# DaehwanKimLab/centrifuge

Hardware: AMD Instinct MI355X
Metric: classified reads/sec (whole node) on 100bp synthetic reads vs p_compressed; HBM GB/s achieved (higher is better)
Workload: dtype u64

## Files before the change

### centrifuge_amd/csrc/cf_device.hip

```cpp
#include <hip/hip_runtime.h>
#include <sched.h>
#include <dlfcn.h>

#include <algorithm>
#include <cmath>
#include <chrono>
#include <cstdio>
#include <cstdlib>
#include <cstring>
#include <memory>
#include <mutex>
#include <stdexcept>
#include <string>
#include <vector>

#include "../../include/centrifuge_amd.h"
#include "cf_index.hpp"
#include "cf_kernels.hpp"
#include "cf_scan.hpp"
#include "cf_textio.hpp"
#include "cf_restore.hpp"
#include "cf_plan.hpp"
#include "cf_knobs.hpp"

using namespace cfamd;

namespace {

thread_local std::string g_err;

struct HipError : std::runtime_error {
    using std::runtime_error::runtime_error;
};
struct ArgError : std::runtime_error {
    using std::runtime_error::runtime_error;
};

#define HIP_OK(expr)                                                                              \
    do {                                                                                          \
        hipError_t e_ = (expr);                                                                   \
        if (e_ != hipSuccess)                                                                     \
            throw HipError(std::string(#expr) + ": " + hipGetErrorString(e_));                    \
    } while (0)

static thread_local uint64_t *g_dryBytes = nullptr;
template <typename T>
struct DevBuf {
    T *p = nullptr;
    size_t n = 0;
    DevBuf() = default;
    DevBuf(const DevBuf &) = delete;
    DevBuf &operator=(const DevBuf &) = delete;
    ~DevBuf() { release(); }
    void release() { if (p) (void)hipFree(p); p = nullptr; n = 0; }
    void alloc(size_t count) {
        release();
        if (count == 0) count = 1;
        if (g_dryBytes) { *g_dryBytes += count * sizeof(T); n = count; return; }
        HIP_OK(hipMalloc(reinterpret_cast<void **>(&p), count * sizeof(T)));
        n = count;
    }
    void ensure(size_t count) { if (count > n) alloc(count + count / 8); }
    void upload(const std::vector<T> &v) {
        alloc(v.size());
        if (!v.empty()) HIP_OK(hipMemcpy(p, v.data(), v.size() * sizeof(T), hipMemcpyHostToDevice));
    }
    size_t bytes() const { return n * sizeof(T); }
};

template <int G>
__global__ void __launch_bounds__(256) k_search(DIndex ix, DParams pr, DBatch b) { search_body<G>(ix, pr, b); }

__global__ void __launch_bounds__(256) k_rlen(const uint64_t *off, uint32_t *rlen, uint32_t nReads) { rlen_body(off, rlen, nReads, cf_global_thread()); }
__global__ void __launch_bounds__(256) k_convert(DConvert c) { convert_body(c, cf_global_thread()); }
__global__ void __launch_bounds__(256) k_dense_unpack(DUnpack u) { dense_unpack_body(u, (uint64_t)blockIdx.x * blockDim.x + threadIdx.x); }
__global__ void __launch_bounds__(256) k_pack(DBatch b, uint8_t *recs, uint32_t W) { pack_body(b, recs, W, cf_global_thread()); }

template <int G, int W, bool COUNT>
__global__ void __launch_bounds__(256) __attribute__((amdgpu_waves_per_eu(COUNT ? 1 : W == 4 ? 6 : W == 6 ? 5 : 4, 8))) k_search2(DIndex ix, DParams pr, DBatch b) {
    __shared__ __attribute__((aligned(16))) uint8_t lds[(256 / G) * rec_lds_stride(W) + 256 * 4 * RankTab<G>::WORDS + (256 / G) * 16 * kLazyHits];
    search2_body<G, W, COUNT>(ix, pr, b, lds);
}

template <int W, bool COUNT, int LZ = 0, bool MULTI = false>
__global__ void __launch_bounds__(256) __attribute__((amdgpu_waves_per_eu((W == 4 && LZ == 1) ? 7 : (W == 4 && MULTI) ? 6 : (W == 6 && MULTI) ? 5 : 1, 8))) k_search2_l1(DIndex ix, DParams pr, DBatch b) {
    __shared__ __attribute__((aligned(16))) uint8_t lds[256 * rec_lds_stride(W) + 256 * 16 * (LZ ? LZ : (int)lazy_hits(1, W))];
    search2_body<1, W, COUNT, true, LZ, MULTI>(ix, pr, b, lds);
}
__global__ void __launch_bounds__(256) k_pair_planes(DIndex ix, uint8_t *planes2, uint64_t nGroups) {
    pair_planes_body(ix, planes2, (uint64_t)blockIdx.x * blockDim.x + threadIdx.x, nGroups);
}
__global__ void __launch_bounds__(256) k_occ_planes(DIndex ix, uint8_t *planes, uint64_t nSides) {
    occ_planes_body(ix, planes, (uint64_t)blockIdx.x * blockDim.x + threadIdx.x, nSides);
}
__global__ void __launch_bounds__(256) k_repeat_probe(DIndex ix, uint32_t nSamples, uint32_t depth, uint32_t *hits) {
    const uint32_t i = cf_global_thread();
    bool yes = false;
    if (i < nSamples && ix.len > 2) {
        uint64_t x = 0x9e3779b97f4a7c15ull * (i + 1);
        x ^= x >> 29; x *= 0xbf58476d1ce4e5b9ull; x ^= x >> 32;
        yes = repeat_probe_body(ix, x % (ix.len - 1), depth);
    }
    const uint64_t m = cf_ballot(yes);
    if (m && cf_lane() == (uint32_t)cf_ctz64(m)) (void)cf_atomic_add(hits, (uint32_t)cf_popc64(m));
}

__global__ void __launch_bounds__(256) k_post_fast(DIndex ix, DParams pr, DBatch b) {
    const uint32_t q = cf_global_thread();
    const bool d = q < b.nQueries ? post_fast_body(ix, pr, b, q) : false;
    if (q < b.nQueries && b.postDeferred) b.postDeferred[q] = d ? 1 : 0;
    defer_push(b.slowPost, &b.st->nSlowPost, d, q);
}
template <bool EARLY>
__global__ void __launch_bounds__(256) k_score_fast(DIndex ix, DParams pr, DBatch b) {
    const uint32_t q = cf_global_thread();
    const bool d = q < b.nQueries ? score_fast_body<EARLY>(ix, pr, b, q) : false;
    defer_push(b.slowScore, &b.st->nSlowScore, d, q);
}
__global__ void __launch_bounds__(256) k_list_all(uint32_t *list, uint32_t *counter, uint32_t n) {
    const uint32_t q = cf_global_thread();
    if (q < n) list[q] = q;
    if (q == 0) *counter = n;
}
__global__ void __launch_bounds__(64) __attribute__((amdgpu_waves_per_eu(3, 8))) k_post(DIndex ix, DParams pr, DBatch b, uint32_t capHits) {
    extern __shared__ __attribute__((aligned(16))) uint8_t ldsPost[];
    HitP *scratch = capHits ? reinterpret_cast<HitP *>(ldsPost) + (size_t)cf_local_thread() * capHits : nullptr;
    const uint32_t n = b.st->nSlowPost;
    for (uint32_t i = cf_global_thread(); i < n; i += cf_global_threads()) post_body(ix, pr, b, b.slowPost[i], scratch, capHits);
}
__global__ void __launch_bounds__(64) k_postfix_only(DIndex ix, DParams pr, DBatch b) {
    const uint32_t i = cf_global_thread();
    if (i < b.st->nItems / 2) post_fix(ix, pr, b, b.items[i]);
}
__global__ void k_window(DBatch b, uint32_t qLo, bool keepSlow) { if (cf_global_thread() == 0) row_window_body(b, qLo, keepSlow); }
__global__ void __launch_bounds__(256) k_emit(DParams pr, DBatch b) {
    const uint32_t q = cf_global_thread();
    if (q < b.nQueries) emit_body(pr, b, q);
}
template <int G, bool COUNT>
__global__ void __launch_bounds__(256) k_walk2(DIndex ix, DBatch b) { walk2_body<G, COUNT>(ix, b); }
template <int MODE>
__global__ void __launch_bounds__(256) k_walk_table(DIndex ix, DBatch b) { walk2_body<2, false, MODE>(ix, b); }
template <typename T>
__global__ void __launch_bounds__(256) k_stop_samples(DIndex ix, T *stopVal, uint64_t *stopBits, uint64_t nSamples) {
    for (uint64_t i = (uint64_t)blockIdx.x * blockDim.x + threadIdx.x; i < nSamples; i += (uint64_t)gridDim.x * blockDim.x) {
        const uint64_t pos = trio_at(ix.saPos, i << ix.offRate);
        stopVal[pos] = static_cast<const T *>(ix.offs)[i];
        cf_atomic_or64(&stopBits[pos >> 6], 1ull << (pos & 63));
    }
}
template <typename T>
__global__ void __launch_bounds__(256) k_stop_bounds(DIndex ix, T *stopVal, uint64_t *stopBits) {
    for (uint64_t j = (uint64_t)blockIdx.x * blockDim.x + threadIdx.x; j < ix.nBound; j += (uint64_t)gridDim.x * blockDim.x) {
        const uint64_t pos = trio_at(ix.saPos, ix.boundRow[j]);
        stopVal[pos] = (T)ix.boundRef[j];
        cf_atomic_or64(&stopBits[pos >> 6], 1ull << (pos & 63));
    }
}
template <typename T>
__global__ void k_stop_end(DIndex ix, T *stopVal, uint64_t *stopBits) {
    const uint64_t pos = trio_at(ix.saPos, ix.zOff);
    stopVal[pos] = 0;
    cf_atomic_or64(&stopBits[pos >> 6], 1ull << (pos & 63));
}
template <typename T>
__global__ void __launch_bounds__(256) k_table_by_position(DIndex ix, const T *stopVal, const uint64_t *stopBits, T *table, uint64_t nRows, uint32_t *walkMax) {
    uint32_t gap = 0;
    for (uint64_t row = (uint64_t)blockIdx.x * blockDim.x + threadIdx.x; row < nRows; row += (uint64_t)gridDim.x * blockDim.x) {
        const uint64_t pos = trio_at(ix.saPos, row);
        uint64_t w = pos >> 6;
        uint64_t m = stopBits[w] & (~0ull >> (63 - (pos & 63)));
        while (m == 0 && w > 0) m = stopBits[--w];
        const uint64_t pred = m ? (w << 6) + 63 - (uint64_t)__builtin_clzll(m) : 0;
        table[row] = stopVal[pred];
        const uint32_t g = (uint32_t)(pos - pred);
        gap = g > gap ? g : gap;
    }
    for (int d = 32; d > 0; d >>= 1) { const uint32_t o = __shfl_xor(gap, d, 64); gap = o > gap ? o : gap; }
    if ((threadIdx.x & 63) == 0 && gap) atomicMax(walkMax, gap);
}
template <typename T>
__global__ void __launch_bounds__(256) k_table_spot_check(DIndex ix, const T *table, uint64_t nRows, uint32_t nCheck, uint32_t *bad) {
    const uint32_t i = blockIdx.x * blockDim.x + threadIdx.x;
    if (i >= nCheck) return;
    const uint64_t row = i < 64 ? (i < 32 ? (uint64_t)i : nRows - 1 - (i - 32)) % nRows : (0x9e3779b97f4a7c15ull * (i + 1)) % nRows;
    uint32_t steps = 0;
    const uint32_t want = resolve_plain_row(ix, row, steps);
    if ((uint32_t)table[row] != (sizeof(T) == 2 ? (want & 0xffffu) : want)) atomicAdd(bad, 1u);
}

template <bool COUNT>
__global__ void __launch_bounds__(256) k_walk3(DIndex ix, DBatch b) {
    for (uint64_t i = (uint64_t)blockIdx.x * blockDim.x + threadIdx.x; i < b.st->rowHi - b.st->rowLo; i += (uint64_t)gridDim.x * blockDim.x)
        walk3_body<COUNT>(ix, b, i);
}
template <bool PLANES>
__global__ void __launch_bounds__(256) k_wide_ftab(DIndex ix, uint32_t wideChars, uint64_t *table) {
    __builtin_assume(PLANES ? ix.planes != nullptr : ix.planes == nullptr);
    for (uint64_t t = (uint64_t)blockIdx.x * blockDim.x + threadIdx.x; t < (1ull << (2 * wideChars)); t += (uint64_t)gridDim.x * blockDim.x)
        wide_ftab_body(ix, wideChars, table, t);
}

__global__ void __launch_bounds__(64) k_resolve_slow(DIndex ix, DParams pr, DBatch b) {
    const uint32_t n = b.st->nSlowScore;
    for (uint32_t i = cf_global_thread(); i < n; i += cf_global_threads()) resolve_query_body(ix, pr, b, b.slowScore[i]);
}
__global__ void __launch_bounds__(64) k_score(DIndex ix, DParams pr, DBatch b, uint32_t capRows, uint32_t sparse, uint32_t rowsMin, uint32_t rowsMax) {
    extern __shared__ __attribute__((aligned(16))) uint8_t ldsScore[];
    const uint32_t n = b.st->nSlowScore;
    if (cf_local_thread() % sparse) return;
    const uint32_t me = cf_global_thread() / sparse, all = cf_global_threads() / sparse;
    uint8_t *scratch = capRows ? ldsScore + (size_t)(cf_local_thread() / sparse) * score_scratch_bytes(capRows) : nullptr;
    for (uint32_t i = me; i < n; i += all) score_body(ix, pr, b, b.slowScore[i], scratch, capRows, rowsMin, rowsMax);
}

__global__ void __launch_bounds__(256) k_scatter_nmask(const uint64_t *idx, const uint32_t *mask, uint64_t n, uint64_t nWords, uint32_t *nmask) {
    const uint64_t i = (uint64_t)blockIdx.x * blockDim.x + threadIdx.x;
    if (i < n && idx[i] < nWords) nmask[idx[i]] = mask ? mask[i] : 0u;
}
__global__ void __launch_bounds__(1024) k_count(DBatch b, uint32_t slotBits, bool direct) {
    __shared__ uint32_t slots[3 * kCountSlots];
    count_body(b, slots, blockIdx.x, slotBits, direct);
}
__global__ void __launch_bounds__(256) k_plan(DPlan p) { plan_body(p, cf_global_thread()); }
__global__ void __launch_bounds__(256) k_plan_fill(DPlan p) { plan_fill_body(p, cf_global_thread()); }
__global__ void __launch_bounds__(256) k_rev_words(DPlan p, uint32_t wordsPerRead) { rev_words_body(p, wordsPerRead, (uint64_t)blockIdx.x * blockDim.x + threadIdx.x); }
__global__ void __launch_bounds__(256) k_plan_maxscore(const uint32_t *rlen, const uint8_t *pass, uint32_t nQueries, int paired, uint32_t *maxScore) {
    plan_maxscore_body(rlen, pass, nQueries, paired, maxScore, cf_global_thread());
}
__global__ void __launch_bounds__(256) k_compact(DCompact c) {
    compact_body(c, cf_global_thread());
}
__global__ void __launch_bounds__(256) k_text_count(DTextMark m) { text_count_body(m, (uint64_t)blockIdx.x * blockDim.x + threadIdx.x); }
__global__ void __launch_bounds__(256) k_text_mark(DTextMark m) { text_mark_body(m, (uint64_t)blockIdx.x * blockDim.x + threadIdx.x); }
__global__ void __launch_bounds__(256) k_text_records(DTextRec d) { text_record_body(d, cf_global_thread()); }
__global__ void __launch_bounds__(256) k_text_pack(DTextPack d) { text_pack_body(d, cf_global_thread()); }
__global__ void __launch_bounds__(256) k_fmt_size(DTextFmt f) { fmt_size_body(f, cf_global_thread()); }
__global__ void __launch_bounds__(256) k_fmt_write(DTextFmt f) { fmt_write_body(f, cf_global_thread()); }
template <int G, bool WRITE>
__global__ void __launch_bounds__(256) k_restore(DIndex ix, DRestore r) { restore_body<G, WRITE>(ix, r); }
__global__ void __launch_bounds__(256) k_restore_rank(const uint64_t *sumIn, const uint32_t *nextIn, uint64_t *sumOut, uint32_t *nextOut, uint32_t nElem) {
    restore_rank_body(sumIn, nextIn, sumOut, nextOut, nElem, cf_global_thread());
}
__global__ void __launch_bounds__(256) k_restore_link(uint64_t *sum, uint32_t *next, uint32_t nSeg, uint32_t *maxLen) {
    const uint32_t s = cf_global_thread();
    if (s < nSeg) {
        if (next[s] == kRestoreTerm) next[s] = nSeg;
        const uint64_t len = sum[s];
        uint32_t l32 = len > 0xffffffffull ? 0xffffffffu : (uint32_t)len;
        for (int m = 32; m > 0; m >>= 1) { const uint32_t o = cf_shfl_xor(l32, m); if (o > l32) l32 = o; }
        if (cf_lane() == 0 && l32) cf_atomic_max(maxLen, l32);
    }
    else if (s == nSeg) { sum[s] = 0; next[s] = nSeg; }
}

template <int G>
__global__ void k_debug_rank(DIndex ix, const uint8_t *chars, const uint64_t *rows, uint64_t n, uint64_t *out) {
    const uint64_t i = (uint64_t)cf_global_thread() / G;
    const uint64_t ii = i < n ? i : n - 1;
    uint64_t t, bb; bool two;
    if (ix.sides) rank_pair<G>(ix, chars[ii] & 3, rows[ii], rows[ii], t, bb, two);
    else rank_any<G>(ix, chars[ii] & 3, rows[ii], rows[ii], t, bb, two);
    if (i < n && Grp<G>::sub() == 0) out[i] = t;
}

__global__ void __launch_bounds__(256) k_random_sides(const uint8_t *sides, uint64_t numSides, uint32_t steps,
                                                        uint64_t seed, unsigned long long *sink) {
    const uint32_t grp = cf_global_thread() >> 3, sub = cf_lane() & 7;
    uint64_t x = seed + 0x9e3779b97f4a7c15ull * (grp + 1);
    unsigned long long acc = 0;
    for (uint32_t s = 0; s < steps; s++) {
        x ^= x >> 12; x ^= x << 25; x ^= x >> 27;
        const uint64_t side = (x * 0x2545f4914f6cdd1dull) % numSides;
        const u64x2 v = cf_load16(sides + side * 128 + 16 * sub);
        uint32_t f = (uint32_t)(v.x ^ v.y);
        f += __shfl_xor(f, 1, 64); f += __shfl_xor(f, 2, 64); f += __shfl_xor(f, 4, 64);
        x += f & 1u;
        acc += f;
    }
    if (acc == 0x1234567u) sink[0] = acc;
}

}

struct TablePlanRecord { int K = 0, textRate = -1, planes = 0, resolveRate = -1, pair = 0, dropSides = 0; bool valid = false; };
struct cf_index {
    HostIndex h;
    int device = -1;
    DIndex d{};
    DevBuf<uint8_t> planes;
    float planesMs = 0;
    DevBuf<uint8_t> planes2;
    float planes2Ms = 0;
    DevBuf<uint64_t> wide;
    float wideMs = 0;
    DevBuf<uint32_t> text;
    DevBuf<uint64_t> saPos, isa;
    float textMs = 0;
    DevBuf<uint8_t> sides, offs, dense;
    int denseRate = -1;
    uint32_t walkMaxSeen = 0;
    bool denseByPos = false;
    uint32_t restoreShift = 0, restoreMaxSeg = 0;
    DevBuf<uint32_t> posBucket;
    DevBuf<u64x2> posFrag, posSeq;
    float denseMs = 0;
    DevBuf<uint64_t> ftab, eftab, boundRow, paths;
    DevBuf<RefInfo> refInfo;
    DevBuf<uint32_t> boundRef, boundBits, pathTidx;
    uint64_t deviceBytes = 0, fileBytes = 0, budgetSeen = 0;
    cf_index_options opt{};
    bool planned = false;
    bool planDropSides = false, sidesDropped = false;
    uint64_t droppedBytes = 0;
    bool wantTextRate0 = false;
    double repeatFrac = -1.0;
    uint32_t multiRowsPlan = 0;
    TablePlanRecord plan{};
    int plannedTextRate = -2;
    int numCUs = 256;
    int occSides[3] = {0, 0, 0}, occPlanes[3] = {0, 0, 0};
    int occMulti[3] = {0, 0, 0};
    int occLazy[3] = {0, 0, 0};
};

struct cf_classifier {
    cf_index *ix = nullptr;
    cf_params p{};
    std::vector<uint64_t> hostList, exclList;
    DParams d{};
    DevBuf<uint8_t> refExcluded;
    DevBuf<uint64_t> hostSet;
    DevBuf<unsigned long long> counts;
    DevBuf<uint8_t> fmtStrs, fmtLeaf;
    DevBuf<uint32_t> fmtUidOff, fmtRankOff, fmtTaxOff;
    uint32_t fmtIdxZero = 0;
    bool fmtMade = false;
    std::mutex fmtMu;
};

template <typename T>
struct PinBuf {
    T *p = nullptr;
    size_t n = 0;
    PinBuf() = default;
    PinBuf(const PinBuf &) = delete;
    PinBuf &operator=(const PinBuf &) = delete;
    ~PinBuf() { if (p) (void)hipHostFree(p); }
    void ensure(size_t count) {
        if (count <= n) return;
        if (p) (void)hipHostFree(p);
        p = nullptr; n = 0;
        count += count / 8;
        if (g_dryBytes) { n = count; return; }
        HIP_OK(hipHostMalloc(reinterpret_cast<void **>(&p), count * sizeof(T), hipHostMallocDefault));
        n = count;
    }
};

struct cf_batch {
    cf_classifier *cl = nullptr;
    uint64_t nReads = 0, nQueries = 0, nWords = 0;
    int paired = 0;
    uint32_t maxLenHost = 0;
    uint32_t recWords = 0;
    bool selfRecords = false;
    bool revMade = false;
    uint32_t revDelta = 0;
    bool loaded = false, planned = false, running = false, finished = false, downloaded = false;
    bool fromBytes = false;
    DevBuf<uint8_t> seq, pass, recs;
    DevBuf<uint64_t> bases, woff, off8, hitBase, qBase, rowVal, rowFirst, tileA;
    DevBuf<uint32_t> nmask, rlen, seeds, items, slotOf, hitCap, nhml, rowRef, nOut, score2, maxScore, qRows, tileC, slowPost, slowScore, qflag, itemMeta;
    DevBuf<HitP> hits;
    DevBuf<PlanHit> qplan;
    DevBuf<QHead> qhead;
    DevBuf<uint64_t> o1tax, o1a, o1b;
    DevBuf<uint8_t> dense;
    uint32_t densePending = 0;
    DevBuf<uint8_t> qinfo;
    DevBuf<uint8_t> postDeferred;
    hipEvent_t evPostFast = nullptr, evPost = nullptr;
    int resultFormat = CF_RESULTS_ROWS;
    DevBuf<uint8_t> text, textOut;
    DevBuf<uint32_t> txCnt, txPos, txSeqOff, txIdOff, txIdLen, txSize, txTuples, txTileC;
    DevBuf<uint64_t> txBase, txOutOff, txTileA;
    DevBuf<TextStatus> txSt;
    PinBuf<TextStatus> hTxSt;
    PinBuf<uint64_t> hTxTotal;
    PinBuf<uint8_t> hTextOut;
    PinBuf<uint32_t> hTuples;
    bool fromText = false;
    bool rowsStay = false;
    bool textDone = false;
    uint64_t textBytes = 0, tupleWords = 0;
    DevBuf<uint64_t> nIdx; DevBuf<uint32_t> nMsk;
    const uint32_t *nmaskZeroOf = nullptr;
    uint64_t nSparsePrev = 0, nmaskZeroN = 0;
    DevBuf<HmEntry> hm;
    DevBuf<TcEntry> tc;
    DevBuf<OutRow> out, outCompact;
    DevBuf<OpCounts> ops;
    DevBuf<unsigned long long> cursor;
    DevBuf<BatchStatus> st;
    uint64_t hitsCapLimit = 0, rowsCapLimit = 0;
    DPlan pl{};
    DBatch d{};
    PinBuf<BatchStatus> hSt;
    PinBuf<OpCounts> hOps;
    PinBuf<OutRow> hRows;
    PinBuf<uint32_t> hNOut, hScore2, hMaxScore;
    PinBuf<uint8_t> hQInfo;
    uint64_t rowsSpec = 0;
    uint64_t rowsOut = 0, rowsTotal = 0;
    double rowsPerQuery = 0;
    double plannedPerQuery = 0;
    uint32_t passes = 0;
    float planMs = 0;
    float ms[5] = {0, 0, 0, 0, 0};
    OpCounts lastOps{};
    bool opsValid = false;
    hipStream_t stream = nullptr;
    hipStream_t tail = nullptr;
    hipEvent_t ev[10] = {};
    hipEvent_t evLate = nullptr;
    bool evInit = false;
    ~cf_batch() { if (evInit) { for (auto &e : ev) (void)hipEventDestroy(e); (void)hipEventDestroy(evLate); (void)hipEventDestroy(evPostFast); (void)hipEventDestroy(evPost); } if (tail) (void)hipStreamDestroy(tail); }
};

namespace {

void streamSection(std::FILE *f, uint64_t bytes, uint8_t *dst) {
    constexpr size_t kChunk = 32u << 20;
    uint8_t *stage[2] = {nullptr, nullptr};
    hipStream_t st;
    HIP_OK(hipStreamCreate(&st));
    hipEvent_t done[2];
    for (int i = 0; i < 2; i++) {
        HIP_OK(hipHostMalloc(reinterpret_cast<void **>(&stage[i]), kChunk, hipHostMallocDefault));
        HIP_OK(hipEventCreate(&done[i]));
    }
    uint64_t pos = 0;
    int cur = 0;
    bool used[2] = {false, false};
    try {
        while (pos < bytes) {
            const size_t n = static_cast<size_t>(std::min<uint64_t>(kChunk, bytes - pos));
            if (used[cur]) HIP_OK(hipEventSynchronize(done[cur]));
            if (std::fread(stage[cur], 1, n, f) != n) throw std::runtime_error("short read while streaming an index section");
            HIP_OK(hipMemcpyAsync(dst + pos, stage[cur], n, hipMemcpyHostToDevice, st));
            HIP_OK(hipEventRecord(done[cur], st));
            used[cur] = true;
            pos += n;
            cur ^= 1;
        }
        HIP_OK(hipStreamSynchronize(st));
    } catch (...) {
        for (int i = 0; i < 2; i++) { (void)hipHostFree(stage[i]); (void)hipEventDestroy(done[i]); }
        (void)hipStreamDestroy(st);
        throw;
    }
    for (int i = 0; i < 2; i++) { (void)hipHostFree(stage[i]); (void)hipEventDestroy(done[i]); }
    (void)hipStreamDestroy(st);
}

void uploadIndex(cf_index &ix, const std::string &base) {
    HostIndex &h = ix.h;
    h.load(base, [&](Section s, std::FILE *f, uint64_t bytes) {
        switch (s) {
            case Section::Sides:
                ix.sides.alloc(bytes + 128);
                streamSection(f, bytes, ix.sides.p);
                break;
            case Section::Ftab:
                ix.ftab.alloc(bytes / 8);
                streamSection(f, bytes, reinterpret_cast<uint8_t *>(ix.ftab.p));
                break;
            case Section::Eftab:
                ix.eftab.alloc(bytes / 8);
                streamSection(f, bytes, reinterpret_cast<uint8_t *>(ix.eftab.p));
                break;
            case Section::SaSample:
                ix.offs.alloc(bytes + 8);
                streamSection(f, bytes, ix.offs.p);
                break;
        }
    });
// ... 726 lines not shown
int cf_index_sa_width(const cf_index *ix) { return ix->h.offw ? 4 : 2; }
int cf_index_wide_ftab_chars(const cf_index *ix) { return ix->d.wideChars; }
int cf_index_occ_planes(const cf_index *ix) { return ix->d.planes ? 1 : 0; }
double cf_index_occ_planes_build_ms(const cf_index *ix) { return ix->planesMs; }
int cf_index_text_verify_rate(const cf_index *ix) { return ix->device >= 0 ? ix->d.posRate : -1; }
double cf_index_text_verify_build_ms(const cf_index *ix) { return ix->textMs; }
int cf_index_resolve_rate(const cf_index *ix) { return ix->denseRate >= 0 ? ix->denseRate : ix->h.g.offRate; }
double cf_index_resolve_build_ms(const cf_index *ix) { return ix->denseMs; }
uint32_t cf_index_walk_bound(const cf_index *ix) { return ix->d.posFrag ? ix->d.walkMax : 0u; }
int cf_index_resolve_by_position(const cf_index *ix) { return ix->denseByPos ? 1 : 0; }
const char *cf_index_uid(const cf_index *ix, uint64_t r) { return r < ix->h.uid.size() ? ix->h.uid[r].c_str() : ""; }
uint64_t cf_index_ref_taxid(const cf_index *ix, uint64_t r) { return r < ix->h.uidTid.size() ? ix->h.uidTid[r] : 0; }
uint64_t cf_index_taxon_id(const cf_index *ix, uint64_t i) { return i < ix->h.taxa.size() ? ix->h.taxa[i] : 0; }
const char *cf_format_seqid(const cf_index *ix, uint32_t u, uint64_t t) { return ix->h.formatSeqId(u, t); }
int cf_tax_rank(const cf_index *ix, uint64_t t) { const TaxNode *n = ix->h.findNode(t); return n ? n->rank : 0; }
const char *cf_tax_rank_string(int rank) { return rankString(rank); }
const char *cf_tax_name(const cf_index *ix, uint64_t t) { return ix->h.name(t); }
uint64_t cf_tax_size(const cf_index *ix, uint64_t t) { return ix->h.size(t); }

cf_status cf_params_default(cf_params *p) {
    if (!p) return CF_ERR_ARG;
    std::memset(p, 0, sizeof *p);
    p->khits = 5; p->min_hitlen = 22; p->rank_slot = 0; p->tree_traverse = 1;
    return CF_OK;
}

cf_status cf_classifier_create(cf_index *ix, const cf_params *p, cf_classifier **out) {
    if (!ix || !p || !out || p->khits < 1 || p->min_hitlen < 15 || p->rank_slot < 0 || p->rank_slot > 9) return CF_ERR_ARG;
    *out = nullptr;
    if (ix->device < 0) { g_err = "index was opened host-only"; return CF_ERR_NO_DEVICE; }
    auto cl = std::make_unique<cf_classifier>();
    cf_status st = guard([&] {
        HIP_OK(hipSetDevice(ix->device));
        cl->ix = ix; cl->p = *p;
        cl->hostList.assign(p->host_taxids, p->host_taxids + std::max(0, p->n_host));
        cl->exclList.assign(p->exclude_taxids, p->exclude_taxids + std::max(0, p->n_exclude));
        cl->p.host_taxids = cl->hostList.data(); cl->p.exclude_taxids = cl->exclList.data();
        const ClassifierTables t = makeClassifier(ix->h, cl->p, cl->d);
        if (cl->d.ihits >= 0x7fffffffu) throw ArgError("-k too large");
        if (ix->h.g.len >= (1ull << 40)) throw ArgError("index too large: hit records hold 40-bit rows");
        if (!t.refExcluded.empty()) { cl->refExcluded.upload(t.refExcluded); cl->d.refExcluded = cl->refExcluded.p; }
        if (!t.hostSet.empty()) { cl->hostSet.upload(t.hostSet); cl->d.hostSet = cl->hostSet.p; cl->d.nHostSet = (uint32_t)t.hostSet.size(); }
        cl->counts.alloc(3 * ix->h.taxa.size());
        HIP_OK(hipMemset(cl->counts.p, 0, cl->counts.bytes()));
    });
    if (st == CF_OK) *out = cl.release();
    return st;
}
void cf_classifier_destroy(cf_classifier *c) { delete c; }

uint32_t cf_gen_rand_seed(const uint8_t *seq, const uint8_t *qual, uint64_t len, const char *name, uint64_t nlen,
                          uint32_t seed) {
    uint32_t r = (seed + 101u) * 59u * 61u * 67u * 71u * 73u * 79u * 83u;
    for (uint64_t i = 0; i < len; i++) r ^= (uint32_t)seq[i] << ((i & 15) << 1);
    for (uint64_t i = 0; i < len; i++) r ^= (uint32_t)(qual ? qual[i] : (uint8_t)'I') << ((i & 3) << 3);
    for (uint64_t i = 0; i < nlen; i++) {
        const int p = (int)(signed char)name[i];
        if (p == '/') break;
        r ^= (uint32_t)p << ((i & 3) << 3);
    }
    return r;
}


static void sizeBatch(cf_batch *bt, uint64_t nReads, uint64_t nWords, uint64_t nBases, uint32_t maxLen, int paired) {
    cf_classifier *cl = bt->cl;
    if (paired && (nReads & 1)) throw ArgError("a paired batch needs an even number of reads");
    if (nReads >= 0x7fffffffull) throw ArgError("a batch holds fewer than 2^31 reads");
    if (maxLen > kMaxReadLen) throw ArgError("reads of more than 16,777,213 bases are not supported (24-bit offsets in the hit records)");
    const uint32_t ftc = (uint32_t)std::max(1, cl->ix->h.g.ftabChars);
    bt->nReads = nReads; bt->paired = paired ? 1 : 0; bt->nQueries = paired ? nReads / 2 : nReads; bt->nWords = nWords;
    bt->maxLenHost = maxLen;
    const uint64_t nq = bt->nQueries;
    bt->bases.ensure(nWords + 16); bt->nmask.ensure(nWords + 16);
    bt->rlen.ensure(nReads + 16); bt->seeds.ensure(nReads + 1); bt->woff.ensure(nReads + 1);
    bt->pass.ensure(nReads + 1); bt->hitCap.ensure(nReads + 16);
    bt->slotOf.ensure(nReads + 1); bt->hitBase.ensure(nReads + 1); bt->items.ensure(nReads + 1);
    bt->nhml.ensure(2 * nReads + 1);
    bt->maxScore.ensure(nq + 1); bt->qflag.ensure(nq + 1); bt->qhead.ensure(nq + 1); bt->qRows.ensure(nq + 16); bt->qBase.ensure(nq + 1);
    bt->qplan.ensure((nq + 1) * kInlinePlan); bt->o1tax.ensure((nq + 1) * kFieldRows); bt->o1a.ensure((nq + 1) * kFieldRows); bt->o1b.ensure((nq + 1) * kFieldRows);
    bt->slowPost.ensure(nq + 1); bt->slowScore.ensure(nq + 1);
    if (envInt("CF_EARLY_SCORE", 0)) bt->postDeferred.ensure(nq + 16);
    bt->out.ensure(nq * (uint64_t)cl->d.k + 1); bt->nOut.ensure(nq + 16); bt->score2.ensure(nq + 1); bt->rowFirst.ensure(nq + 1);
    bt->cursor.ensure(4); bt->ops.ensure(1); bt->st.ensure(1);
    bt->tileA.ensure(scan_tiles_for(std::max(nReads, nq)) + 1); bt->tileC.ensure(scan_tiles_for(std::max(nReads, nq)) + 1);
    bt->recWords = searchVersion() != 2 ? 0u : maxLen <= 128 ? 4u : maxLen <= 192 ? 6u : maxLen <= 256 ? 8u : 0u;
    if ((uint64_t)(0.15 * maxLen) + maxLen / (uint64_t)ftc + 3 >= 255) bt->recWords = 0;
    bt->selfRecords = bt->recWords && cl->ix->d.planes && nWords < 0xffffffffull && envInt("CF_SELF_RECORDS", 1);
    if (bt->selfRecords) bt->itemMeta.ensure(8 * nReads + 8);
    bt->revDelta = bt->selfRecords && 2 * nWords + 64 < 0xffffffffull && envInt("CF_REV_WORDS", 1) ? (uint32_t)nWords + 16u : 0u;
    if (bt->revDelta) bt->bases.ensure(2 * (nWords + 16));
    else if (bt->recWords) bt->recs.ensure(2 * nReads * (uint64_t)rec_bytes((int)bt->recWords) + 64);
    uint64_t hitsWant = 2 * ((nBases ? nBases : 32 * nWords) / ftc + 2 * nReads);
    hitsWant += hitsWant / 50 + 4096;
    if (bt->hitsCapLimit) hitsWant = std::min(hitsWant, bt->hitsCapLimit);
    if (bt->hits.n < hitsWant) bt->hits.ensure(hitsWant);
    if (bt->recWords && bt->hits.n > 0xffffffffull) throw ArgError("batch too large: its hit lists need 32-bit offsets, split it");
    uint64_t rowsWant = std::max<uint64_t>(4 * nq, 1u << 16);
    if (bt->plannedPerQuery > 0) rowsWant = std::max<uint64_t>(rowsWant, (uint64_t)((double)nq * bt->plannedPerQuery * 1.15));
    if (const int per = envInt("CF_ROWS_PER_QUERY", 0)) rowsWant = std::max<uint64_t>((uint64_t)per * nq, 1024);
    if (bt->rowsCapLimit) rowsWant = bt->rowsCapLimit;
    if (bt->rowVal.n < rowsWant || bt->rowsCapLimit) { bt->rowVal.ensure(rowsWant); bt->rowRef.ensure(rowsWant); bt->hm.ensure(rowsWant); bt->tc.ensure(rowsWant); }
    bt->outCompact.ensure(nq * (uint64_t)cl->d.k + 1);
    bt->hSt.ensure(1); bt->hOps.ensure(1);
    bt->hNOut.ensure(nq + 1); bt->hScore2.ensure(nq + 1); bt->hMaxScore.ensure(nq + 1);
    if (bt->resultFormat == CF_RESULTS_NARROW) { bt->qinfo.ensure(nq + 16); bt->hQInfo.ensure(nq + 16); }
    bt->rowsSpec = bt->rowsPerQuery > 0 ? (uint64_t)((double)nq * bt->rowsPerQuery * 1.04) + 4096 : nq + nq / 4 + 1024;
    bt->rowsSpec = std::min<uint64_t>(bt->rowsSpec, nq * (uint64_t)cl->d.k);
    bt->hRows.ensure(std::max<uint64_t>(bt->rowsSpec, nq + nq / 4 + 1024));
    if (g_dryBytes) return;
    if (!bt->evInit) { for (auto &e : bt->ev) HIP_OK(hipEventCreate(&e)); HIP_OK(hipEventCreate(&bt->evLate)); HIP_OK(hipEventCreate(&bt->evPostFast)); HIP_OK(hipEventCreate(&bt->evPost)); bt->evInit = true; }
    if (!bt->tail && (envInt("CF_TAIL_STREAM", 0) || envInt("CF_EARLY_SCORE", 0))) HIP_OK(hipStreamCreateWithFlags(&bt->tail, hipStreamNonBlocking));
}

static void bindBatch(cf_batch *bt) {
    cf_classifier *cl = bt->cl;
    DPlan &pl = bt->pl;
    pl.nmask = bt->nmask.p; pl.rlen = bt->rlen.p; pl.woff = bt->woff.p; pl.nReads = (uint32_t)bt->nReads; pl.ftabChars = cl->ix->h.g.ftabChars;
    pl.maxLenAllowed = bt->maxLenHost;
    pl.nWords = bt->nWords;
    pl.pass = bt->pass.p; pl.hitCap = bt->hitCap.p; pl.slotOf = bt->slotOf.p;
    pl.hitBase = bt->hitBase.p; pl.items = bt->items.p; pl.st = bt->st.p;
    pl.itemMeta = bt->selfRecords ? bt->itemMeta.p : nullptr;
    pl.bases = bt->bases.p; pl.revDelta = bt->revDelta;
    pl.hitsCap = bt->hitsCapLimit ? std::min<uint64_t>(bt->hitsCapLimit, bt->hits.n) : bt->hits.n;
    DBatch &d = bt->d;
    d.bases = bt->bases.p; d.nmask = bt->nmask.p; d.rlen = bt->rlen.p; d.woff = bt->woff.p; d.seeds = bt->seeds.p;
    d.pass = bt->pass.p; d.items = bt->items.p; d.slotOf = bt->slotOf.p; d.hitBase = bt->hitBase.p; d.hitCap = bt->hitCap.p;
    d.lazyHits = (uint32_t)(envInt("CF_LAZY_HITS", 1) != 0) | (cl->ix->d.posFrag ? 4u : 0u);
    d.directRefs = (uint32_t)(cl->ix->dense.p && cl->ix->d.walkRate == 0 && envInt("CF_SCORE_FAST", 1) != 0 && envInt("CF_DIRECT_REFS", 1) != 0);
    d.hits = bt->hits.p; d.nhml = bt->nhml.p; d.qflag = bt->qflag.p; d.qhead = bt->qhead.p; d.qplan = bt->qplan.p; d.qplanStride = bt->qplan.n / kInlinePlan; d.qRows = bt->qRows.p; d.qBase = bt->qBase.p;
    d.rowVal = bt->rowVal.p; d.rowRef = bt->rowRef.p; d.hm = bt->hm.p; d.tc = bt->tc.p;
    d.out = bt->out.p; d.nOut = bt->nOut.p; d.score2 = bt->score2.p;
    d.counts = cl->counts.p; d.nTaxa = (uint32_t)cl->ix->h.taxa.size();
    d.nReads = (uint32_t)bt->nReads; d.nQueries = (uint32_t)bt->nQueries; d.paired = bt->paired;
    d.cursor = bt->cursor.p; d.st = bt->st.p; d.ops = bt->ops.p;
    d.slowPost = bt->slowPost.p; d.slowScore = bt->slowScore.p; d.postDeferred = envInt("CF_EARLY_SCORE", 0) ? bt->postDeferred.p : nullptr;
    d.o1tax = bt->o1tax.p; d.o1a = bt->o1a.p; d.o1b = bt->o1b.p; d.oStride = bt->o1tax.n / kFieldRows;
    d.hitsCap = pl.hitsCap;
    d.rowsCap = bt->rowsCapLimit ? std::min<uint64_t>(bt->rowsCapLimit, bt->rowVal.n) : bt->rowVal.n;
    d.recs = bt->recWords && !bt->selfRecords ? bt->recs.p : nullptr; d.recWords = bt->recWords;
    d.itemMeta = bt->selfRecords ? bt->itemMeta.p : nullptr;
}

static void enqueuePlan(cf_batch *bt, hipStream_t st) {
    const uint64_t nReads = bt->nReads;
    const DPlan &pl = bt->pl;
    HIP_OK(hipStreamWaitEvent(st, bt->ev[8], 0));
    if (bt->densePending) {
        const uint32_t L = bt->densePending - 1;
        const DUnpack u{bt->dense.p, bt->bases.p, bt->rlen.p, (uint32_t)nReads, L, bt->revDelta ? bt->bases.p + bt->revDelta : nullptr};
        bt->revMade = bt->revDelta != 0;
        const uint64_t threads = nReads * std::max<uint64_t>(((uint64_t)L + 31) >> 5, 1);
        hipLaunchKernelGGL(k_dense_unpack, dim3((unsigned)((threads + 255) / 256)), dim3(256), 0, st, u);
        bt->densePending = 0;
    }
    HIP_OK(hipEventRecord(bt->ev[5], st));
    HIP_OK(hipMemsetAsync(bt->st.p, 0, sizeof(BatchStatus), st));
    const dim3 gp((unsigned)((nReads + 1 + 255) / 256)), bl(256);
    if (bt->fromBytes && nReads) hipLaunchKernelGGL(k_rlen, gp, bl, 0, st, bt->off8.p, bt->rlen.p, (uint32_t)nReads);
    scan_enqueue<SCAN_WORDS>(bt->rlen.p, nReads, bt->woff.p, nullptr, bt->tileA.p, bt->tileC.p, st);
    if (bt->fromBytes && nReads) {
        DConvert c{bt->seq.p, bt->off8.p, bt->woff.p, bt->bases.p, bt->nmask.p, (uint32_t)nReads};
        hipLaunchKernelGGL(k_convert, dim3((unsigned)((nReads + 255) / 256)), dim3(256), 0, st, c);
    }
    if (bt->fromText && nReads) {
        const DTextPack c{bt->text.p, bt->txSeqOff.p, bt->rlen.p, bt->woff.p, bt->bases.p, bt->nmask.p, (uint32_t)nReads};
        hipLaunchKernelGGL(k_text_pack, dim3((unsigned)((nReads + 255) / 256)), dim3(256), 0, st, c);
    }
    hipLaunchKernelGGL(k_plan, gp, bl, 0, st, pl);
    scan_enqueue<SCAN_HITS>(bt->hitCap.p, nReads, bt->hitBase.p, bt->slotOf.p, bt->tileA.p, bt->tileC.p, st);
    hipLaunchKernelGGL(k_plan_fill, gp, bl, 0, st, pl);
    if (pl.revDelta && nReads && !bt->revMade) {
        const uint64_t threads = nReads * (uint64_t)bt->recWords;
        hipLaunchKernelGGL(k_rev_words, dim3((unsigned)((threads + 255) / 256)), bl, 0, st, pl, bt->recWords);
    }
    if (bt->nQueries) hipLaunchKernelGGL(k_plan_maxscore, dim3((unsigned)((bt->nQueries + 255) / 256)), bl, 0, st, bt->rlen.p, bt->pass.p,
                                         (uint32_t)bt->nQueries, bt->paired, bt->maxScore.p);
    if (bt->recWords && !bt->selfRecords && nReads) {
        const uint64_t threads = 2 * nReads * (uint64_t)bt->recWords;
        hipLaunchKernelGGL(k_pack, dim3((unsigned)((threads + 255) / 256)), bl, 0, st, bt->d, bt->recs.p, bt->recWords);
    }
    HIP_OK(hipEventRecord(bt->ev[6], st));
    bt->planned = true;
}

static dim3 listGrid(const cf_index &ix, uint64_t nq) { return dim3((unsigned)std::max<uint64_t>(1, std::min<uint64_t>((nq + 63) / 64, (uint64_t)ix.numCUs * 32))); }

static bool earlyScoreMode(const cf_batch *bt) {
    static const bool on = envInt("CF_EARLY_SCORE", 0) != 0 && envInt("CF_POST_FAST", 1) != 0 && envInt("CF_SCORE_FAST", 1) != 0 && envInt("CF_TAIL_STREAM", 0) == 0;
    return on && bt->d.directRefs != 0 && bt->tail != nullptr && bt->nQueries != 0;
}

static void enqueuePost(cf_batch *bt, hipStream_t st) {
    cf_classifier *cl = bt->cl;
    cf_index &ix = *cl->ix;
    const DBatch &d = bt->d;
    const uint32_t nq = (uint32_t)bt->nQueries;
    if (!nq) return;
    static const bool fast = envInt("CF_POST_FAST", 1) != 0;
    if (fast) hipLaunchKernelGGL(k_post_fast, dim3((nq + 255) / 256), dim3(256), 0, st, ix.d, cl->d, d);
    else hipLaunchKernelGGL(k_list_all, dim3((nq + 255) / 256), dim3(256), 0, st, bt->slowPost.p, &bt->st.p->nSlowPost, nq);
    if (earlyScoreMode(bt)) {
        HIP_OK(hipEventRecord(bt->evPostFast, st));
        HIP_OK(hipStreamWaitEvent(bt->tail, bt->evPostFast, 0));
        hipLaunchKernelGGL(k_post, listGrid(ix, nq), dim3(64), 0, bt->tail, ix.d, cl->d, d, 0u);
        HIP_OK(hipEventRecord(bt->evPost, bt->tail));
        hipLaunchKernelGGL(k_score_fast<true>, dim3((nq + 255) / 256), dim3(256), 0, st, ix.d, cl->d, d);
        HIP_OK(hipStreamWaitEvent(st, bt->evPost, 0));
        return;
    }
    static const bool postLds = envInt("CF_POST_LDS", 0) != 0;
    const uint32_t capHits = postLds ? (uint32_t)std::min<uint64_t>(60, 2 * ((uint64_t)bt->maxLenHost / (uint64_t)std::max(1, ix.h.g.ftabChars) + 2)) : 0u;
    hipLaunchKernelGGL(k_post, listGrid(ix, nq), dim3(64), (size_t)64 * capHits * sizeof(HitP), st, ix.d, cl->d, d, capHits);
}

static bool enqueueRowPass(cf_batch *bt, uint32_t qLo, hipStream_t st, bool marks, hipStream_t late = nullptr, bool early = false) {
    cf_classifier *cl = bt->cl;
    cf_index &ix = *cl->ix;
    const DBatch &d = bt->d;
    const uint32_t nq = (uint32_t)bt->nQueries;
    static const bool fast = envInt("CF_SCORE_FAST", 1) != 0;
    HIP_OK(hipMemsetAsync(bt->cursor.p + 1, 0, 8, st));
    hipLaunchKernelGGL(k_window, dim3(1), dim3(64), 0, st, d, qLo, early);
    const bool direct = d.directRefs != 0;
    if (nq && !direct) hipLaunchKernelGGL(k_emit, dim3((nq + 255) / 256), dim3(256), 0, st, cl->d, d);
    if (marks) HIP_OK(hipEventRecord(bt->ev[2], st));
    const bool counted = nq && !direct ? launchWalk(cl, bt, st) : true;
    if (marks) HIP_OK(hipEventRecord(bt->ev[3], st));
    if (nq) {
        if (early) {}
        else if (fast) hipLaunchKernelGGL(k_score_fast<false>, dim3((nq + 255) / 256), dim3(256), 0, st, ix.d, cl->d, d);
        else hipLaunchKernelGGL(k_list_all, dim3((nq + 255) / 256), dim3(256), 0, st, bt->slowScore.p, &bt->st.p->nSlowScore, nq);
        if (late && late != st) {
            HIP_OK(hipEventRecord(bt->evLate, st));
            HIP_OK(hipStreamWaitEvent(late, bt->evLate, 0));
            st = late;
        }
        if (direct) hipLaunchKernelGGL(k_resolve_slow, listGrid(ix, nq), dim3(64), 0, st, ix.d, cl->d, d);
        static const uint32_t capRows = (uint32_t)std::clamp(envInt("CF_SCORE_LDS_ROWS", 0), 0, 64), sparse = (uint32_t)std::clamp(envInt("CF_SCORE_LDS_SPARSE", 2), 1, 64);
        hipLaunchKernelGGL(k_score, listGrid(ix, nq), dim3(64), (size_t)(64 / sparse) * score_scratch_bytes(capRows), st, ix.d, cl->d, d, capRows, capRows ? sparse : 1u, 0u, 0xffffffffu);
        static const uint32_t slotBits = (uint32_t)std::clamp(envInt("CF_COUNT_SLOT_BITS", (int)kCountSlotBits), 1, (int)kCountSlotBits);
        hipLaunchKernelGGL(k_count, dim3((nq + kCountChunk - 1) / kCountChunk), dim3(1024), 0, st, d, slotBits, d.nTaxa <= (1u << slotBits));
    }
    if (marks) HIP_OK(hipEventRecord(bt->ev[4], st));
    return counted;
}

static void enqueueCompact(cf_batch *bt, hipStream_t st) {
    const uint32_t nq = (uint32_t)bt->nQueries;
    const dim3 g((nq + 1 + 255) / 256), bl(256);
    scan_enqueue<SCAN_PLAIN>(bt->nOut.p, nq, bt->rowFirst.p, nullptr, bt->tileA.p, bt->tileC.p, st);
    const bool narrow = bt->resultFormat == CF_RESULTS_NARROW;
    const DCompact c{bt->out.p, bt->o1tax.p, bt->o1a.p, bt->o1b.p, bt->d.oStride, bt->nOut.p, bt->rowFirst.p, (uint32_t)bt->cl->d.k, nq, bt->outCompact.p, bt->st.p,
                     narrow ? reinterpret_cast<NarrowRow *>(bt->outCompact.p) : nullptr, bt->qinfo.p, bt->pass.p, bt->paired};
    hipLaunchKernelGGL(k_compact, g, bl, 0, st, c);
}

static void enqueueClassify(cf_batch *bt, hipStream_t st) {
    cf_classifier *cl = bt->cl;
    HIP_OK(hipMemsetAsync(bt->cursor.p, 0, 32, st));
    HIP_OK(hipMemsetAsync(bt->ops.p, 0, sizeof(OpCounts), st));
    static const bool allFast = envInt("CF_POST_FAST", 1) != 0 && envInt("CF_SCORE_FAST", 1) != 0;
    if (!allFast) {
        HIP_OK(hipMemsetAsync(bt->qRows.p, 0, 4 * (bt->nQueries + 1), st));
        HIP_OK(hipMemsetAsync(bt->nOut.p, 0, 4 * (bt->nQueries + 1), st));
    }
    HIP_OK(hipMemsetAsync(&bt->st.p->nSlowPost, 0, 8, st));
    HIP_OK(hipEventRecord(bt->ev[0], st));
    bool counted = true;
    if (bt->nReads) counted = launchSearch(cl, bt, st) && counted;
    HIP_OK(hipEventRecord(bt->ev[1], st));
    static const int tailMode = envInt("CF_TAIL_STREAM", 0);
    hipStream_t ts = bt->tail && tailMode == 1 ? bt->tail : st;
    hipStream_t late = bt->tail && tailMode == 2 ? bt->tail : ts;
    if (ts != st) HIP_OK(hipStreamWaitEvent(ts, bt->ev[1], 0));
    const bool early = earlyScoreMode(bt);
    enqueuePost(bt, ts);
    scan_enqueue<SCAN_PLAIN>(bt->qRows.p, bt->nQueries, bt->qBase.p, nullptr, bt->tileA.p, bt->tileC.p, ts);
    counted = enqueueRowPass(bt, 0, ts, true, late, early) && counted;
    enqueueCompact(bt, late);
    HIP_OK(hipEventRecord(bt->ev[9], late));
    bt->opsValid = counted;
    bt->passes = 1;
    bt->running = true; bt->finished = false; bt->downloaded = false;
    bt->stream = st;
}

static void enqueueDownload(cf_batch *bt, hipStream_t st) {
    const uint64_t nq = bt->nQueries;
    HIP_OK(hipStreamWaitEvent(st, bt->ev[9], 0));
    HIP_OK(hipMemcpyAsync(bt->hSt.p, bt->st.p, sizeof(BatchStatus), hipMemcpyDeviceToHost, st));
    HIP_OK(hipMemcpyAsync(bt->hOps.p, bt->ops.p, sizeof(OpCounts), hipMemcpyDeviceToHost, st));
    if (nq && !bt->rowsStay) {
        const uint64_t spec = std::min<uint64_t>(bt->rowsSpec, nq * (uint64_t)bt->cl->d.k);
        if (bt->resultFormat == CF_RESULTS_NARROW) {
            HIP_OK(hipMemcpyAsync(bt->hQInfo.p, bt->qinfo.p, nq, hipMemcpyDeviceToHost, st));
            HIP_OK(hipMemcpyAsync(bt->hScore2.p, bt->score2.p, nq * 4, hipMemcpyDeviceToHost, st));
            HIP_OK(hipMemcpyAsync(bt->hRows.p, bt->outCompact.p, spec * sizeof(NarrowRow), hipMemcpyDeviceToHost, st));
        } else {
            HIP_OK(hipMemcpyAsync(bt->hNOut.p, bt->nOut.p, nq * 4, hipMemcpyDeviceToHost, st));
            HIP_OK(hipMemcpyAsync(bt->hScore2.p, bt->score2.p, nq * 4, hipMemcpyDeviceToHost, st));
            HIP_OK(hipMemcpyAsync(bt->hMaxScore.p, bt->maxScore.p, nq * 4, hipMemcpyDeviceToHost, st));
            HIP_OK(hipMemcpyAsync(bt->hRows.p, bt->outCompact.p, spec * sizeof(OutRow), hipMemcpyDeviceToHost, st));
        }
    }
    HIP_OK(hipEventRecord(bt->ev[7], st));
    bt->downloaded = true;
}

static void waitBatch(cf_batch *bt) {
    if (!bt->running) throw ArgError("no batch in flight on this slot");
    if (bt->finished) return;
    hipStream_t st = bt->stream;
    if (!bt->downloaded) enqueueDownload(bt, st);
    HIP_OK(hipEventSynchronize(bt->ev[7]));
    HIP_OK(hipGetLastError());
    bool redo = false;
    auto fetchStatus = [&] {
        HIP_OK(hipEventSynchronize(bt->ev[9]));
        HIP_OK(hipMemcpyAsync(bt->hSt.p, bt->st.p, sizeof(BatchStatus), hipMemcpyDeviceToHost, st));
        HIP_OK(hipStreamSynchronize(st));
        HIP_OK(hipGetLastError());
    };
    HIP_OK(hipEventSynchronize(bt->ev[9]));
    auto lapse = [&](float &ms, int a, int b) { if (hipEventElapsedTime(&ms, bt->ev[a], bt->ev[b]) != hipSuccess) { ms = 0; (void)hipGetLastError(); } };
    lapse(bt->planMs, 5, 6);
    lapse(bt->ms[0], 0, 1); lapse(bt->ms[1], 1, 2); lapse(bt->ms[2], 2, 3); lapse(bt->ms[3], 3, 4); lapse(bt->ms[4], 0, 4);
    if (bt->hSt.p->flags & kStLenOverflow) throw ArgError("a read is longer than the max_len the batch was submitted with");
    if (bt->hSt.p->flags & kStWordsOverflow) throw ArgError("the read lengths need more packed words than n_words says were uploaded");
    if (bt->hSt.p->flags & kStHitsOverflow) {
        const uint64_t need = bt->hSt.p->hitsNeed;
        if (bt->recWords && need > 0xffffffffull) throw ArgError("batch too large: its hit lists need 32-bit offsets, split it");
        bt->hitsCapLimit = 0;
        bt->hits.ensure(need + 1);
        bindBatch(bt);
        enqueuePlan(bt, st);
        enqueueClassify(bt, st);
        fetchStatus();
        if (bt->hSt.p->flags & kStHitsOverflow) throw std::logic_error("hit pool still too small after growing it");
        redo = true;
    }
    while (bt->hSt.p->qHi < bt->nQueries) {
        if (bt->hSt.p->qHi == bt->hSt.p->qLo) {
            const uint64_t need = bt->hSt.p->needRows;
            bt->rowsCapLimit = 0;
            bt->rowVal.ensure(need); bt->rowRef.ensure(need); bt->hm.ensure(need); bt->tc.ensure(need);
            bindBatch(bt);
        }
        enqueueRowPass(bt, bt->hSt.p->qHi, st, false);
        bt->passes++;
        bt->opsValid = false;
        fetchStatus();
        redo = true;
    }
    if (redo) {
        enqueueCompact(bt, st);
        HIP_OK(hipEventRecord(bt->ev[9], st));
        enqueueDownload(bt, st);
        HIP_OK(hipEventSynchronize(bt->ev[7]));
        HIP_OK(hipGetLastError());
    }
    bt->rowsOut = bt->hSt.p->rowsOut;
    bt->rowsTotal = bt->hSt.p->rowsTotal;
    if (bt->nQueries) { bt->rowsPerQuery = (double)bt->rowsOut / (double)bt->nQueries; bt->plannedPerQuery = (double)bt->rowsTotal / (double)bt->nQueries; }
    if (bt->rowsOut > bt->rowsSpec && !bt->rowsStay) {
        const uint64_t have = bt->rowsSpec;
        const size_t rb = bt->resultFormat == CF_RESULTS_NARROW ? sizeof(NarrowRow) : sizeof(OutRow);
        if (bt->rowsOut > bt->hRows.n) {
            PinBuf<OutRow> bigger;
            bigger.ensure(bt->rowsOut + bt->rowsOut / 8);
            std::memcpy(bigger.p, bt->hRows.p, have * rb);
            std::swap(bt->hRows.p, bigger.p); std::swap(bt->hRows.n, bigger.n);
        }
        HIP_OK(hipMemcpy(reinterpret_cast<uint8_t *>(bt->hRows.p) + have * rb, reinterpret_cast<const uint8_t *>(bt->outCompact.p) + have * rb, (bt->rowsOut - have) * rb, hipMemcpyDeviceToHost));
    }
    bt->lastOps = *bt->hOps.p;
    bt->lastOps.nRows = bt->rowsTotal;
    bt->finished = true;
}

static void uploadBytes(cf_batch *bt, const uint8_t *seq, const uint64_t *off, const uint32_t *seeds, uint64_t nReads, int paired, hipStream_t st) {
    uint64_t nWords = 0, maxLen = 0;
    for (uint64_t r = 0; r < nReads; r++) {
        if (off[r + 1] < off[r]) throw ArgError("read offsets must be non-decreasing");
        const uint64_t L = off[r + 1] - off[r];
        nWords += (L + 31) >> 5;
        maxLen = std::max(maxLen, L);
    }
    if (maxLen > 0xffffffffull) throw ArgError("a read is longer than 2^32 bases");
    const uint64_t nbases = off[nReads] - off[0];
    if (nbases && !seq) throw ArgError("null sequence buffer");
    sizeBatch(bt, nReads, nWords, nbases, (uint32_t)maxLen, paired);
    bt->seq.ensure(nbases + 16); bt->off8.ensure(nReads + 1);
    bindBatch(bt);
    HIP_OK(hipMemsetAsync(bt->seq.p + nbases, 0, 16, st));
    if (nbases) HIP_OK(hipMemcpyAsync(bt->seq.p, seq + off[0], nbases, hipMemcpyHostToDevice, st));
    if (off[0] == 0) HIP_OK(hipMemcpyAsync(bt->off8.p, off, (nReads + 1) * 8, hipMemcpyHostToDevice, st));
    else {
        std::vector<uint64_t> rel(nReads + 1);
        for (uint64_t r = 0; r <= nReads; r++) rel[r] = off[r] - off[0];
        HIP_OK(hipMemcpy(bt->off8.p, rel.data(), (nReads + 1) * 8, hipMemcpyHostToDevice));
    }
    if (nReads) HIP_OK(hipMemcpyAsync(bt->seeds.p, seeds, nReads * 4, hipMemcpyHostToDevice, st));
    HIP_OK(hipEventRecord(bt->ev[8], st));
    bt->fromBytes = true; bt->fromText = false; bt->densePending = 0; bt->revMade = false; bt->nmaskZeroOf = nullptr;
    bt->loaded = true; bt->planned = false; bt->running = false; bt->finished = false;
}

static void uploadSparseMask(cf_batch *bt, const uint64_t *idx, const uint32_t *mask, uint64_t nNWords, uint64_t nWords, hipStream_t st) {
    if (bt->nmaskZeroOf != bt->nmask.p || bt->nmaskZeroN != bt->nmask.n) {
        HIP_OK(hipMemsetAsync(bt->nmask.p, 0, bt->nmask.bytes(), st));
        bt->nmaskZeroOf = bt->nmask.p; bt->nmaskZeroN = bt->nmask.n; bt->nSparsePrev = 0;
    } else if (bt->nSparsePrev) {
        hipLaunchKernelGGL(k_scatter_nmask, dim3((unsigned)((bt->nSparsePrev + 255) / 256)), dim3(256), 0, st, bt->nIdx.p, nullptr,
                           bt->nSparsePrev, (uint64_t)bt->nmask.n, bt->nmask.p);
        bt->nSparsePrev = 0;
    }
    if (nNWords) {
        bt->nSparsePrev = nNWords;
        bt->nIdx.ensure(nNWords); bt->nMsk.ensure(nNWords);
        HIP_OK(hipMemcpyAsync(bt->nIdx.p, idx, nNWords * 8, hipMemcpyHostToDevice, st));
        HIP_OK(hipMemcpyAsync(bt->nMsk.p, mask, nNWords * 4, hipMemcpyHostToDevice, st));
        hipLaunchKernelGGL(k_scatter_nmask, dim3((unsigned)((nNWords + 255) / 256)), dim3(256), 0, st, bt->nIdx.p, bt->nMsk.p,
                           nNWords, nWords, bt->nmask.p);
    }
}

static void uploadPacked(cf_batch *bt, const cf_packed_reads *in, hipStream_t st) {
    if (in->n_reads && (!in->len || !in->seeds)) throw ArgError("null length / seed array");
    if (in->n_words && !in->bases) throw ArgError("null packed-base array");
    if (!in->nmask && in->n_nwords && (!in->nword_idx || !in->nword_mask)) throw ArgError("null sparse N-mask arrays");
    sizeBatch(bt, in->n_reads, in->n_words, in->n_bases, in->max_len, in->paired);
    bindBatch(bt);
    if (in->n_words) {
        HIP_OK(hipMemcpyAsync(bt->bases.p, in->bases, in->n_words * 8, hipMemcpyHostToDevice, st));
        if (in->nmask) { HIP_OK(hipMemcpyAsync(bt->nmask.p, in->nmask, in->n_words * 4, hipMemcpyHostToDevice, st)); bt->nmaskZeroOf = nullptr; }
        else uploadSparseMask(bt, in->nword_idx, in->nword_mask, in->n_nwords, in->n_words, st);
    }
    if (in->n_reads) {
        HIP_OK(hipMemcpyAsync(bt->rlen.p, in->len, in->n_reads * 4, hipMemcpyHostToDevice, st));
        HIP_OK(hipMemcpyAsync(bt->seeds.p, in->seeds, in->n_reads * 4, hipMemcpyHostToDevice, st));
    }
    HIP_OK(hipEventRecord(bt->ev[8], st));
    bt->fromBytes = false; bt->fromText = false; bt->densePending = 0; bt->revMade = false;
    bt->loaded = true; bt->planned = false; bt->running = false; bt->finished = false;
}

static void uploadDense(cf_batch *bt, const cf_dense_reads *in, hipStream_t st) {
    if (in->n_reads && (!in->bases4 || !in->seeds)) throw ArgError("null dense-base / seed array");
    if (in->n_nwords && (!in->nword_idx || !in->nword_mask)) throw ArgError("null sparse N-mask arrays");
    if (in->read_len > kMaxReadLen) throw ArgError("reads of more than 16,777,213 bases are not supported (24-bit offsets in the hit records)");
    const uint64_t W = ((uint64_t)in->read_len + 31) >> 5, bpr = ((uint64_t)in->read_len + 3) >> 2;
    const uint64_t nWords = in->n_reads * W, nBytes = in->n_reads * bpr;
    sizeBatch(bt, in->n_reads, nWords, in->n_reads * (uint64_t)in->read_len, in->read_len, in->paired);
    bt->dense.ensure(nBytes + 32);
    bindBatch(bt);
    if (in->n_reads) {
        HIP_OK(hipMemcpyAsync(bt->dense.p, in->bases4, nBytes, hipMemcpyHostToDevice, st));
        HIP_OK(hipMemsetAsync(bt->dense.p + nBytes, 0, 32, st));
        HIP_OK(hipMemcpyAsync(bt->seeds.p, in->seeds, in->n_reads * 4, hipMemcpyHostToDevice, st));
        if (nWords) uploadSparseMask(bt, in->nword_idx, in->nword_mask, in->n_nwords, nWords, st);
    }
    bt->densePending = in->n_reads ? in->read_len + 1 : 0; bt->revMade = false;
    HIP_OK(hipEventRecord(bt->ev[8], st));
    bt->fromBytes = false; bt->fromText = false;
    bt->loaded = true; bt->planned = false; bt->running = false; bt->finished = false;
}


static void uploadText(cf_batch *bt, const cf_text_reads *in, hipStream_t st, cf_text_info *info) {
    if (in->format != CF_TEXT_FASTA && in->format != CF_TEXT_FASTQ) throw ArgError("cf_text_reads::format is CF_TEXT_FASTA or CF_TEXT_FASTQ");
    const int nBlocks = in->text2 ? 2 : 1;
    const char *src[2] = {in->text, in->text2};
    const uint64_t nBs[2] = {in->n_bytes, in->text2 ? in->n_bytes2 : 0};
    if ((nBs[0] && !src[0]) || (nBs[1] && !src[1])) throw ArgError("null text block");
    if (nBs[0] + nBs[1] >= 0xffff0000ull) throw ArgError("the text blocks of a batch hold fewer than 2^32 bytes (32-bit places in them)");
    const bool fasta = in->format == CF_TEXT_FASTA;
    uint64_t at[2], pieces[2], pieceAt[2], recCap[2], posCap[2], posAt[2], textBytes = 0, nPieces = 0, posTotal = 0, recMax = 0;
    for (int k = 0; k < nBlocks; k++) {
        at[k] = textBytes; pieces[k] = (nBs[k] + kTextPiece - 1) / kTextPiece; pieceAt[k] = nPieces;
        recCap[k] = nBs[k] / 32 + 1024; posCap[k] = fasta ? recCap[k] : 4 * recCap[k]; posAt[k] = posTotal;
        textBytes += pieces[k] * kTextPiece + kTextPad; nPieces += pieces[k] + 16; posTotal += posCap[k] + 16;
        recMax = std::max(recMax, recCap[k]);
    }
    const uint64_t readCap = recMax * (uint64_t)nBlocks;
    bt->text.ensure(textBytes);
    bt->txCnt.ensure(nPieces + 16); bt->txBase.ensure(nPieces + 16); bt->txPos.ensure(posTotal + 16);
    bt->txTileA.ensure(scan_tiles_for(std::max(pieces[0], pieces[nBlocks - 1])) + 1); bt->txTileC.ensure(scan_tiles_for(std::max(pieces[0], pieces[nBlocks - 1])) + 1);
    bt->rlen.ensure(readCap + 16); bt->seeds.ensure(readCap + 16);
    bt->txSeqOff.ensure(readCap + 16); bt->txIdOff.ensure(readCap + 16); bt->txIdLen.ensure(readCap + 16);
    bt->txSt.ensure(1); bt->hTxSt.ensure(1); bt->hTxTotal.ensure(2);
    *info = cf_text_info{};
    bt->loaded = false; bt->planned = false; bt->running = false; bt->finished = false;
    HIP_OK(hipMemsetAsync(bt->txSt.p, 0, sizeof(TextStatus), st));
    const uint32_t seed0 = (in->global_seed + 101u) * 59u * 61u * 67u * 71u * 73u * 79u * 83u;
    const dim3 bl(256);
    for (int k = 0; k < nBlocks; k++) {
        uint8_t *text = bt->text.p + at[k];
        HIP_OK(hipMemsetAsync(text + nBs[k], 0, pieces[k] * kTextPiece + kTextPad - nBs[k], st));
        if (nBs[k]) HIP_OK(hipMemcpyAsync(text, src[k], nBs[k], hipMemcpyHostToDevice, st));
        uint32_t *cnt = bt->txCnt.p + pieceAt[k], *pos = bt->txPos.p + posAt[k];
        uint64_t *base = bt->txBase.p + pieceAt[k];
        const DTextMark m{text, nBs[k], fasta ? (uint32_t)'>' : (uint32_t)'\n', cnt, base, pos, posCap[k]};
        const dim3 gp((unsigned)std::max<uint64_t>(1, (pieces[k] + 255) / 256));
        if (pieces[k]) hipLaunchKernelGGL(k_text_count, gp, bl, 0, st, m);
        scan_enqueue<SCAN_PLAIN>(cnt, pieces[k], base, nullptr, bt->txTileA.p, bt->txTileC.p, st);
        if (pieces[k]) hipLaunchKernelGGL(k_text_mark, gp, bl, 0, st, m);
        DTextRec d{text, nBs[k], pos, base + pieces[k], posCap[k], (uint32_t)recCap[k], (uint32_t)in->format, seed0,
                   bt->rlen.p, bt->seeds.p, bt->txSeqOff.p, bt->txIdOff.p, bt->txIdLen.p, bt->txSt.p, (uint32_t)at[k], (uint32_t)nBlocks, (uint32_t)k};
        hipLaunchKernelGGL(k_text_records, dim3((unsigned)((recCap[k] + 255) / 256)), bl, 0, st, d);
        HIP_OK(hipMemcpyAsync(bt->hTxTotal.p + k, base + pieces[k], 8, hipMemcpyDeviceToHost, st));
    }
    HIP_OK(hipMemcpyAsync(bt->hTxSt.p, bt->txSt.p, sizeof(TextStatus), hipMemcpyDeviceToHost, st));
    HIP_OK(hipStreamSynchronize(st));
    HIP_OK(hipGetLastError());
    const TextStatus ts = *bt->hTxSt.p;
    uint64_t nRec[2] = {0, 0};
    for (int k = 0; k < nBlocks; k++) nRec[k] = fasta ? bt->hTxTotal.p[k] : bt->hTxTotal.p[k] >> 2;
    if (ts.flags) { info->irregular = ts.flags; return; }
    if (nBlocks == 2 && nRec[0] != nRec[1]) { info->irregular = kTxMateCount; return; }
    uint64_t nq = nRec[0];
    if (in->max_reads && nq > in->max_reads) nq = in->max_reads;
    const uint64_t nReads = nq * (uint64_t)nBlocks;
    sizeBatch(bt, nReads, ts.words(), ts.bases(), ts.maxLen, nBlocks == 2);
    bindBatch(bt);
    HIP_OK(hipEventRecord(bt->ev[8], st));
    bt->fromText = true; bt->fromBytes = false; bt->densePending = 0; bt->revMade = false; bt->nmaskZeroOf = nullptr;
    bt->loaded = true;
    info->n_reads = nReads; info->n_bases = ts.bases(); info->max_len = ts.maxLen;
}

cf_status cf_host_alloc(void **p, size_t bytes) {
    if (!p) return CF_ERR_ARG;
    *p = nullptr;
    if (!haveDevice()) { g_err = "no HIP device visible"; return CF_ERR_NO_DEVICE; }
    return guard([&] { HIP_OK(hipHostMalloc(p, bytes ? bytes : 1, hipHostMallocDefault)); });
}
void cf_host_free(void *p) { if (p) (void)hipHostFree(p); }

cf_status cf_batch_alloc(cf_classifier *cl, uint64_t maxReads, uint64_t maxWords, cf_batch **out) {
    if (!cl || !out) return CF_ERR_ARG;
    *out = nullptr;
    auto bt = std::make_unique<cf_batch>();
    cf_status st = guard([&] {
        HIP_OK(hipSetDevice(cl->ix->device));
        bt->cl = cl;
        const uint64_t per = maxReads ? (32 * maxWords + maxReads - 1) / maxReads : 0;
        sizeBatch(bt.get(), maxReads & ~1ull, maxWords, 0, (uint32_t)std::min<uint64_t>(per, 128), 0);
        bt->nReads = bt->nQueries = bt->nWords = 0;
    });
    if (st == CF_OK) *out = bt.release();
    return st;
}

cf_status cf_slot_estimate_bytes(uint64_t maxReads, uint64_t maxWords, int khits, int ftabChars, int occPlanes, uint64_t *bytes) {
    if (!bytes || khits < 1 || ftabChars < 1) return CF_ERR_ARG;
    *bytes = 0;
    return guard([&] {
        cf_index ix;
        ix.h.g.ftabChars = ftabChars;
        if (occPlanes) ix.d.planes = reinterpret_cast<const uint8_t *>(&ix);
        cf_classifier cl;
        cl.ix = &ix; cl.d.k = (uint32_t)khits;
        uint64_t total = 0;
        g_dryBytes = &total;
        try {
            cf_batch bt;
            bt.cl = &cl;
            const uint64_t per = maxReads ? (32 * maxWords + maxReads - 1) / maxReads : 0;
            sizeBatch(&bt, maxReads & ~1ull, maxWords, 0, (uint32_t)std::min<uint64_t>(per, 128), 0);
            bt.evInit = false;
        } catch (...) { g_dryBytes = nullptr; throw; }
        g_dryBytes = nullptr;
        *bytes = total;
    });
}

cf_status cf_batch_upload_packed_async(cf_batch *bt, const cf_packed_reads *in, void *streamv) {
    if (!bt || !in) return CF_ERR_ARG;
    return guard([&] {
        HIP_OK(hipSetDevice(bt->cl->ix->device));
        if (bt->running && !bt->finished) throw ArgError("the slot still has a batch in flight: cf_batch_wait first");
        uploadPacked(bt, in, static_cast<hipStream_t>(streamv));
    });
}

cf_status cf_batch_upload_dense_async(cf_batch *bt, const cf_dense_reads *in, void *streamv) {
    if (!bt || !in) return CF_ERR_ARG;
    return guard([&] {
        HIP_OK(hipSetDevice(bt->cl->ix->device));
        if (bt->running && !bt->finished) throw ArgError("the slot still has a batch in flight: cf_batch_wait first");
        uploadDense(bt, in, static_cast<hipStream_t>(streamv));
    });
}

cf_status cf_batch_set_result_format(cf_batch *bt, int format) {
    if (!bt || (format != CF_RESULTS_ROWS && format != CF_RESULTS_NARROW)) return CF_ERR_ARG;
    if (format == CF_RESULTS_NARROW && bt->cl->d.k > 63) { g_err = "the narrow result format holds a query's row count in six bits: -k <= 63"; return CF_ERR_ARG; }
    if (bt->running && !bt->finished) { g_err = "the slot still has a batch in flight: cf_batch_wait first"; return CF_ERR_ARG; }
    return guard([&] {
        HIP_OK(hipSetDevice(bt->cl->ix->device));
        if (format != bt->resultFormat) { bt->finished = false; bt->running = false; bt->downloaded = false; }
        bt->resultFormat = format;
        if (format == CF_RESULTS_NARROW) { bt->qinfo.ensure(bt->nOut.n + 16); bt->hQInfo.ensure(bt->nOut.n + 16); }
    });
}

cf_status cf_classify_async(cf_classifier *cl, cf_batch *bt, void *streamv) {
    if (!cl || !bt || bt->cl != cl) return CF_ERR_ARG;
    return guard([&] {
// ... 255 lines not shown
        if (!bt->loaded) throw ArgError("no reads were uploaded into this slot");
        hipStream_t st = static_cast<hipStream_t>(streamv);
        enqueuePlan(bt, st);
        HIP_OK(hipEventSynchronize(bt->ev[6]));
        HIP_OK(hipGetLastError());
        HIP_OK(hipEventElapsedTime(&bt->planMs, bt->ev[5], bt->ev[6]));
    });
}
cf_status cf_batch_plan_ms(const cf_batch *bt, float *ms) {
    if (!bt || !ms) return CF_ERR_ARG;
    *ms = bt->planMs;
    return CF_OK;
}

cf_status cf_classify(cf_classifier *cl, cf_batch *bt, void *streamv) {
    cf_status s = cf_classify_async(cl, bt, streamv);
    if (s == CF_OK) s = cf_batch_download_async(bt, streamv);
    if (s == CF_OK) s = cf_batch_wait(bt, nullptr);
    return s;
}

static void needFinished(const cf_batch *bt) {
    if (!bt->finished) throw ArgError("the batch has not been classified (or waited for)");
    if (bt->resultFormat != CF_RESULTS_ROWS) throw ArgError("the slot's result format is CF_RESULTS_NARROW: cf_batch_wait_narrow / cf_results_narrow_expand");
}

cf_status cf_batch_results(cf_batch *bt, cf_row *rows, uint32_t *nRows, uint32_t *score2) {
    if (!bt || !rows || !nRows || !score2) return CF_ERR_ARG;
    return guard([&] {
        HIP_OK(hipSetDevice(bt->cl->ix->device));
        needFinished(bt);
        const uint32_t k = bt->cl->d.k;
        uint64_t at = 0;
        for (uint64_t q = 0; q < bt->nQueries; q++) {
            const uint32_t n = std::min(bt->hNOut.p[q], k);
            std::memcpy(rows + q * k, bt->hRows.p + at, (size_t)n * sizeof(OutRow));
            at += n;
        }
        std::memcpy(nRows, bt->hNOut.p, bt->nQueries * 4);
        std::memcpy(score2, bt->hScore2.p, bt->nQueries * 4);
    });
}

cf_status cf_batch_max_scores(const cf_batch *bt, uint32_t *out) {
    if (!bt || !out) return CF_ERR_ARG;
    return guard([&] {
        HIP_OK(hipSetDevice(bt->cl->ix->device));
        if (bt->finished && bt->resultFormat == CF_RESULTS_ROWS) std::memcpy(out, bt->hMaxScore.p, bt->nQueries * 4);
        else if (bt->nQueries) {
            if (!bt->planned) throw ArgError("the batch has no plan yet");
            HIP_OK(hipMemcpy(out, bt->maxScore.p, bt->nQueries * 4, hipMemcpyDeviceToHost));
        }
    });
}

cf_status cf_batch_num_rows(cf_batch *bt, uint64_t *total) {
    if (!bt || !total) return CF_ERR_ARG;
    return guard([&] { needFinished(bt); *total = bt->rowsOut; });
}

cf_status cf_batch_results_compact(cf_batch *bt, cf_row *rows, uint64_t rowsCap, uint32_t *nRows, uint32_t *score2) {
    if (!bt || !nRows || !score2 || (!rows && rowsCap)) return CF_ERR_ARG;
    return guard([&] {
        needFinished(bt);
        if (rowsCap < bt->rowsOut) throw ArgError("cf_batch_results_compact: the row buffer is smaller than cf_batch_num_rows");
        std::memcpy(rows, bt->hRows.p, bt->rowsOut * sizeof(OutRow));
        std::memcpy(nRows, bt->hNOut.p, bt->nQueries * 4);
        std::memcpy(score2, bt->hScore2.p, bt->nQueries * 4);
    });
}

cf_status cf_batch_timings(const cf_batch *bt, float ms[5]) {
    if (!bt || !ms) return CF_ERR_ARG;
    std::memcpy(ms, bt->ms, sizeof bt->ms);
    return CF_OK;
}
cf_status cf_batch_opcounts(cf_batch *bt, cf_opcounts *o) {
    if (!bt || !o) return CF_ERR_ARG;
    if (!bt->finished) { g_err = "the batch has not been classified"; return CF_ERR_ARG; }
    if (!bt->opsValid) {
        cf_classifier *cl = bt->cl;
        const cf_status st = guard([&] {
            HIP_OK(hipSetDevice(cl->ix->device));
            HIP_OK(hipMemset(bt->cursor.p, 0, 32));
            HIP_OK(hipMemset(bt->ops.p, 0, sizeof(OpCounts)));
            if (bt->nReads) launchSearch(cl, bt, nullptr, 0, true);
            if (bt->nQueries && !bt->d.directRefs) launchWalk(cl, bt, nullptr, true);
            HIP_OK(hipDeviceSynchronize());
            HIP_OK(hipGetLastError());
            HIP_OK(hipMemcpy(&bt->lastOps, bt->ops.p, sizeof(OpCounts), hipMemcpyDeviceToHost));
            bt->lastOps.nRows = bt->rowsTotal;
            bt->opsValid = true;
        });
        if (st != CF_OK) return st;
    }
    o->n_ftab = bt->lastOps.nFtab; o->n_pair = bt->lastOps.nPair; o->n_pair2 = bt->lastOps.nPair2;
    o->n_single = bt->lastOps.nSingle; o->n_walk = bt->lastOps.nWalk; o->n_rows = bt->lastOps.nRows;
    o->n_ftab_wide = bt->lastOps.nFtabWide; o->n_verify = bt->lastOps.nVerify; o->n_text_loads = bt->lastOps.nTextLoads;
    o->n_pos_hits = bt->lastOps.nPosHits;
    return CF_OK;
}

cf_status cf_counts_reset(cf_classifier *cl) {
    if (!cl) return CF_ERR_ARG;
    return guard([&] { HIP_OK(hipSetDevice(cl->ix->device)); HIP_OK(hipMemset(cl->counts.p, 0, cl->counts.bytes())); });
}
cf_status cf_counts_get(cf_classifier *cl, uint64_t *nReads, uint64_t *nUnique) {
    if (!cl || !nReads || !nUnique) return CF_ERR_ARG;
    return guard([&] {
        const size_t n = cl->ix->h.taxa.size();
        HIP_OK(hipSetDevice(cl->ix->device));
        HIP_OK(hipMemcpy(nReads, cl->counts.p, n * 8, hipMemcpyDeviceToHost));
        HIP_OK(hipMemcpy(nUnique, cl->counts.p + n, n * 8, hipMemcpyDeviceToHost));
    });
}
cf_status cf_counts_get_single(cf_classifier *cl, uint64_t *nSingle) {
    if (!cl || !nSingle) return CF_ERR_ARG;
    return guard([&] {
        const size_t n = cl->ix->h.taxa.size();
        HIP_OK(hipSetDevice(cl->ix->device));
        HIP_OK(hipMemcpy(nSingle, cl->counts.p + 2 * n, n * 8, hipMemcpyDeviceToHost));
    });
}
void *cf_counts_device(cf_classifier *cl) { return cl ? cl->counts.p : nullptr; }

extern "C++" {
namespace {
struct Rccl {
    int (*allReduce)(const void *, void *, size_t, int, int, void *, hipStream_t) = nullptr;
    int (*commInitAll)(void **, int, const int *) = nullptr;
    int (*commDestroy)(void *) = nullptr;
    int (*groupStart)() = nullptr;
    int (*groupEnd)() = nullptr;
    bool ok = false;
};
const Rccl &rccl() {
    static const Rccl r = [] {
        Rccl x;
        void *h = dlopen("librccl.so.1", RTLD_LAZY | RTLD_LOCAL);
        if (!h) h = dlopen("librccl.so", RTLD_LAZY | RTLD_LOCAL);
        if (!h) return x;
        x.allReduce = reinterpret_cast<decltype(x.allReduce)>(dlsym(h, "ncclAllReduce"));
        x.commInitAll = reinterpret_cast<decltype(x.commInitAll)>(dlsym(h, "ncclCommInitAll"));
        x.commDestroy = reinterpret_cast<decltype(x.commDestroy)>(dlsym(h, "ncclCommDestroy"));
        x.groupStart = reinterpret_cast<decltype(x.groupStart)>(dlsym(h, "ncclGroupStart"));
        x.groupEnd = reinterpret_cast<decltype(x.groupEnd)>(dlsym(h, "ncclGroupEnd"));
        x.ok = x.allReduce && x.commInitAll && x.commDestroy && x.groupStart && x.groupEnd;
        return x;
    }();
    return r;
}
}
}

cf_status cf_counts_allreduce(cf_classifier *cl, void *comm, void *streamv) {
    if (!cl || !comm) return CF_ERR_ARG;
    if (!rccl().ok) { g_err = "librccl.so.1 could not be loaded"; return CF_ERR_HIP; }
    return guard([&] {
        HIP_OK(hipSetDevice(cl->ix->device));
        constexpr int kNcclUint64 = 5, kNcclSum = 0;
        const int rc = rccl().allReduce(cl->counts.p, cl->counts.p, 3 * cl->ix->h.taxa.size(), kNcclUint64, kNcclSum, comm,
                                        static_cast<hipStream_t>(streamv));
        if (rc != 0) throw HipError("ncclAllReduce failed with ncclResult_t " + std::to_string(rc));
    });
}

cf_status cf_comm_init_all(int n, const int *devices, void **comms) {
    if (n < 1 || !devices || !comms) return CF_ERR_ARG;
    if (!rccl().ok) { g_err = "librccl.so.1 could not be loaded"; return CF_ERR_HIP; }
    return guard([&] {
        if (envInt("CF_TEST_FAIL_COMM", 0)) throw HipError("ncclCommInitAll failed with ncclResult_t 2 (CF_TEST_FAIL_COMM)");
        const int rc = rccl().commInitAll(comms, n, devices);
        if (rc != 0) throw HipError("ncclCommInitAll failed with ncclResult_t " + std::to_string(rc));
// ... 4 lines not shown
cf_status cf_counts_allreduce_group(cf_classifier *const *cls, void *const *comms, int n) {
    if (n < 1 || !cls || !comms) return CF_ERR_ARG;
    if (!rccl().ok) { g_err = "librccl.so.1 could not be loaded"; return CF_ERR_HIP; }
    return guard([&] {
        if (rccl().groupStart() != 0) throw HipError("ncclGroupStart failed");
        cf_status st = CF_OK;
        for (int i = 0; i < n && st == CF_OK; i++) st = cf_counts_allreduce(cls[i], comms[i], nullptr);
        const int rc = rccl().groupEnd();
        if (st != CF_OK) throw HipError(g_err);
        if (rc != 0) throw HipError("ncclGroupEnd failed with ncclResult_t " + std::to_string(rc));
        for (int i = 0; i < n; i++) { HIP_OK(hipSetDevice(cls[i]->ix->device)); HIP_OK(hipStreamSynchronize(nullptr)); }
    });
}

cf_status cf_stream_create(int device, void **stream) {
    if (!stream) return CF_ERR_ARG;
    *stream = nullptr;
    if (!haveDevice()) { g_err = "no HIP device visible"; return CF_ERR_NO_DEVICE; }
    return guard([&] {
        HIP_OK(hipSetDevice(device));
        hipStream_t s;
        HIP_OK(hipStreamCreateWithFlags(&s, hipStreamNonBlocking));
        *stream = s;
    });
}
void cf_stream_destroy(void *stream) { if (stream) (void)hipStreamDestroy(static_cast<hipStream_t>(stream)); }
int cf_device_count(void) { int n = 0; return hipGetDeviceCount(&n) == hipSuccess ? n : 0; }

int cf_device_numa_node(int device) {
    char bdf[64] = {0};
    if (device < 0 || device >= cf_device_count()) return -1;
    if (hipDeviceGetPCIBusId(bdf, (int)sizeof bdf - 1, device) != hipSuccess) { (void)hipGetLastError(); return -1; }
    for (char *c = bdf; *c; c++) *c = (char)std::tolower((unsigned char)*c);
    std::FILE *f = std::fopen((std::string("/sys/bus/pci/devices/") + bdf + "/numa_node").c_str(), "r");
    if (!f) return -1;
    int node = -1;
    if (std::fscanf(f, "%d", &node) != 1) node = -1;
    std::fclose(f);
    return node;
}

cf_status cf_thread_bind_near_device(int device, int *nodeOut) {
    if (nodeOut) *nodeOut = -1;
    const int node = cf_device_numa_node(device);
    if (node < 0) return CF_OK;
    std::FILE *f = std::fopen(("/sys/devices/system/node/node" + std::to_string(node) + "/cpulist").c_str(), "r");
    if (!f) return CF_OK;
    char buf[4096] = {0};
    const size_t got = std::fread(buf, 1, sizeof buf - 1, f);
    std::fclose(f);
    buf[got] = 0;
    cpu_set_t have, want;
    CPU_ZERO(&have); CPU_ZERO(&want);
    if (sched_getaffinity(0, sizeof have, &have) != 0) return CF_OK;
    int nWant = 0;
    for (const char *p = buf; *p;) {
        char *e = nullptr;
        const long lo = std::strtol(p, &e, 10);
        if (e == p) break;
        long hi = lo;
        p = e;
        if (*p == '-') { hi = std::strtol(p + 1, &e, 10); p = e; }
        for (long c = lo; c <= hi && c < CPU_SETSIZE; c++) if (c >= 0 && CPU_ISSET((int)c, &have)) { CPU_SET((int)c, &want); nWant++; }
        while (*p == ',' || *p == '\n' || *p == ' ') p++;
    }
    if (nWant == 0) return CF_OK;
    if (sched_setaffinity(0, sizeof want, &want) != 0) return CF_OK;
    if (nodeOut) *nodeOut = node;
    return CF_OK;
}

cf_status cf_debug_search(cf_classifier *cl, const uint8_t *seq, uint64_t len, cf_hit *hf, cf_hit *hr,
                          uint32_t maxHits, uint32_t nhits[2]) {
    if (!cl || !seq || !hf || !hr || !nhits) return CF_ERR_ARG;
    nhits[0] = nhits[1] = 0;
    const uint64_t off[2] = {0, len};
    const uint32_t seed = 0;
    cf_batch *bt = nullptr;
    cf_status st = cf_batch_create(cl, seq, off, &seed, 1, 0, &bt);
    if (st != CF_OK) return st;
    std::unique_ptr<cf_batch> own(bt);
    return guard([&] {
        BatchStatus hs{};
        HIP_OK(hipMemcpy(&hs, bt->st.p, sizeof hs, hipMemcpyDeviceToHost));
        if (hs.nItems == 0) return;
        HIP_OK(hipMemset(bt->cursor.p, 0, 32));
        HIP_OK(hipMemset(bt->ops.p, 0, sizeof(OpCounts)));
        bt->d.lazyHits = 0;
        launchSearch(cl, bt, nullptr, 1);
        hipLaunchKernelGGL(k_postfix_only, dim3(1), dim3(64), 0, 0, cl->ix->d, cl->d, bt->d);
        HIP_OK(hipDeviceSynchronize());
        HIP_OK(hipGetLastError());
        uint32_t n[2], cap = 0;
        HIP_OK(hipMemcpy(n, bt->nhml.p, 8, hipMemcpyDeviceToHost));
        n[0] &= 0x7fffffffu; n[1] &= 0x7fffffffu;
        HIP_OK(hipMemcpy(&cap, bt->hitCap.p, 4, hipMemcpyDeviceToHost));
        std::vector<HitP> all(2 * (size_t)cap);
        HIP_OK(hipMemcpy(all.data(), bt->hits.p, all.size() * sizeof(HitP), hipMemcpyDeviceToHost));
        cf_hit *o[2] = {hf, hr};
        for (int f = 0; f < 2; f++) {
            nhits[f] = n[f];
            for (uint32_t i = 0; i < n[f] && i < maxHits; i++) {
                const HitP &p = all[f * cap + i];
                const uint64_t top = p.w0 & kHit40, size = p.w1 & kHit40;
                const bool dummy = top == kHit40 && size == 0;
                const uint32_t bw = (uint32_t)(p.w1 >> 40);
                o[f][i].top = dummy ? kNone64 : top; o[f][i].bot = dummy ? kNone64 : top + size;
                o[f][i].bwoff = bw == kHit24 ? kNone32 : bw; o[f][i].len = (uint32_t)(p.w0 >> 40);
            }
        }
    });
}

cf_status cf_debug_resolve(cf_index *ix, const uint64_t *rows, uint64_t n, uint32_t *refs) {
    if (!ix || !rows || !refs) return CF_ERR_ARG;
    if (ix->device < 0) return CF_ERR_NO_DEVICE;
    return guard([&] {
        HIP_OK(hipSetDevice(ix->device));
        DevBuf<uint64_t> r; DevBuf<uint32_t> o; DevBuf<unsigned long long> cur; DevBuf<BatchStatus> st;
        r.upload(std::vector<uint64_t>(rows, rows + n)); o.alloc(n); cur.alloc(4); st.alloc(1);
        HIP_OK(hipMemset(cur.p, 0, 32));
        BatchStatus hs{};
        hs.rowLo = 0; hs.rowHi = n;
        HIP_OK(hipMemcpy(st.p, &hs, sizeof hs, hipMemcpyHostToDevice));
        DBatch d{};
        d.rowVal = r.p; d.rowRef = o.p; d.cursor = cur.p; d.st = st.p;
        hipLaunchKernelGGL((k_walk2<2, false>), dim3(persistentBlocks(*ix, n, 4, 2)), dim3(256), 0, 0, ix->d, d);
        HIP_OK(hipDeviceSynchronize());
        HIP_OK(hipGetLastError());
        HIP_OK(hipMemcpy(refs, o.p, n * 4, hipMemcpyDeviceToHost));
    });
}

cf_status cf_debug_scan(int device, int mode, const uint32_t *in, uint64_t n, uint64_t *sums, uint32_t *counts) {
    if ((!in && n) || !sums || mode < 0 || mode > 2 || (mode == 2 && !counts)) return CF_ERR_ARG;
    if (!haveDevice()) return CF_ERR_NO_DEVICE;
    return guard([&] {
        HIP_OK(hipSetDevice(device));
        DevBuf<uint32_t> din, dc, tc; DevBuf<uint64_t> da, ta;
        din.alloc(n + 16); da.alloc(n + 1); dc.alloc(n + 1); ta.alloc(scan_tiles_for(n) + 1); tc.alloc(scan_tiles_for(n) + 1);
        if (n) HIP_OK(hipMemcpy(din.p, in, n * 4, hipMemcpyHostToDevice));
        if (mode == SCAN_WORDS) scan_enqueue<SCAN_WORDS>(din.p, n, da.p, dc.p, ta.p, tc.p, nullptr);
        else if (mode == SCAN_PLAIN) scan_enqueue<SCAN_PLAIN>(din.p, n, da.p, dc.p, ta.p, tc.p, nullptr);
        else scan_enqueue<SCAN_HITS>(din.p, n, da.p, dc.p, ta.p, tc.p, nullptr);
        HIP_OK(hipDeviceSynchronize());
        HIP_OK(hipGetLastError());
        HIP_OK(hipMemcpy(sums, da.p, (n + 1) * 8, hipMemcpyDeviceToHost));
        if (mode == SCAN_HITS) HIP_OK(hipMemcpy(counts, dc.p, (n + 1) * 4, hipMemcpyDeviceToHost));
    });
}

static cf_status debugRank(cf_index *ix, const uint8_t *chars, const uint64_t *rows, uint64_t n, uint64_t *out, int g) {
    if (!ix || !chars || !rows || !out || n == 0) return CF_ERR_ARG;
    if (ix->device < 0) return CF_ERR_NO_DEVICE;
    return guard([&] {
        HIP_OK(hipSetDevice(ix->device));
        DevBuf<uint8_t> c; DevBuf<uint64_t> r, o;
        c.upload(std::vector<uint8_t>(chars, chars + n)); r.upload(std::vector<uint64_t>(rows, rows + n)); o.alloc(n);
        const uint64_t threads = n * g;
        if (g == 8) hipLaunchKernelGGL(k_debug_rank<8>, dim3((int)((threads + 255) / 256)), dim3(256), 0, 0, ix->d, c.p, r.p, n, o.p);
        else hipLaunchKernelGGL(k_debug_rank<1>, dim3((int)((threads + 255) / 256)), dim3(256), 0, 0, ix->d, c.p, r.p, n, o.p);
        HIP_OK(hipDeviceSynchronize());
        HIP_OK(hipGetLastError());
        HIP_OK(hipMemcpy(out, o.p, n * 8, hipMemcpyDeviceToHost));
    });
}
cf_status cf_debug_rank(cf_index *ix, const uint8_t *chars, const uint64_t *rows, uint64_t n, uint64_t *out) {
    return debugRank(ix, chars, rows, n, out, 8);
}
cf_status cf_debug_rank1(cf_index *ix, const uint8_t *chars, const uint64_t *rows, uint64_t n, uint64_t *out) {
// ... 47 lines not shown
```

### centrifuge_amd/csrc/cf_kernels.hpp

```cpp
#pragma once
#include "cf_platform.hpp"

namespace cfamd {

constexpr uint32_t kNone32 = 0xffffffffu;
constexpr uint64_t kNone64 = ~0ull;
constexpr uint32_t kSideChars = 384;
constexpr int kSearchChunk = CF_WAVE;

struct RefInfo { uint64_t tax; uint32_t tidx, pid; };
static_assert(sizeof(RefInfo) == 16, "RefInfo layout");
struct DIndex {
    const uint8_t *sides;
    const uint64_t *ftab, *eftab;
    uint64_t fchr0, fchr1, fchr2, fchr3;
    uint64_t len, zOff, zSide;
    uint32_t zIn;
    int32_t ftabChars, offRate, offw;
    const void *offs;
    const uint8_t *planes;
    const uint8_t *planes2;
    const uint64_t *wide;
    int32_t wideChars;
    const uint64_t *text;
// ... 384 lines not shown
CF_DEV int strand_char(const DBatch &b, uint64_t wbase, uint32_t L, bool fw, uint32_t j, ReadWin &win) {
    const uint32_t pos = fw ? j : L - 1 - j;
    const uint64_t wi = wbase + (pos >> 5);
    if (wi != win.idx) { win.w = b.bases[wi]; win.m = b.nmask[wi]; win.idx = wi; }
    const uint32_t sh = pos & 31;
    if ((win.m >> sh) & 1u) return 4;
    const int c = (int)((win.w >> (2 * sh)) & 3);
    return fw ? c : (c ^ 3);
}

CF_DEV uint64_t load8_any(const uint8_t *base, uint64_t off) {
    const uint64_t a = off & ~7ull;
    const uint32_t sh = (uint32_t)(off & 7) * 8;
    const uint64_t lo = cf_load8(base + a);
    if (sh == 0) return lo;
    const uint64_t hi = cf_load8(base + a + 8);
    return (lo >> sh) | (hi << (64 - sh));
}
CF_DEV uint64_t nonzero_bytes(uint64_t t) { t |= t >> 4; t |= t >> 2; t |= t >> 1; return t & 0x0101010101010101ull; }
CF_DEV uint64_t bswap64(uint64_t v) {
    v = ((v & 0x00ff00ff00ff00ffull) << 8) | ((v >> 8) & 0x00ff00ff00ff00ffull);
    v = ((v & 0x0000ffff0000ffffull) << 16) | ((v >> 16) & 0x0000ffff0000ffffull);
    return (v << 32) | (v >> 32);
}

CF_DEV void squeeze8(uint64_t x, uint32_t &c16, uint32_t &n8) {
    const uint64_t isN = nonzero_bytes(x & 0xfcfcfcfcfcfcfcfcull);
    uint64_t c = x & 0x0303030303030303ull & ~(isN * 3);
    c = (c | (c >> 6)) & 0x000f000f000f000full;
    c = (c | (c >> 12)) & 0x000000ff000000ffull;
    c = (c | (c >> 24)) & 0xffffull;
    c16 = (uint32_t)c;
    n8 = (uint32_t)((isN * 0x0102040810204080ull) >> 56);
}
CF_DEV uint64_t spread_pairs(uint32_t m) {
    uint64_t x = m;
    x = (x | (x << 16)) & 0x0000ffff0000ffffull;
    x = (x | (x << 8)) & 0x00ff00ff00ff00ffull;
    x = (x | (x << 4)) & 0x0f0f0f0f0f0f0f0full;
    x = (x | (x << 2)) & 0x3333333333333333ull;
    x = (x | (x << 1)) & 0x5555555555555555ull;
    return x * 3;
}
CF_DEV uint64_t pair_reverse(uint64_t x) {
    x = cf_brev64(x);
    return ((x >> 1) & 0x5555555555555555ull) | ((x & 0x5555555555555555ull) << 1);
}

struct DConvert {
    const uint8_t *seq;
    const uint64_t *off;
    const uint64_t *woff;
    uint64_t *bases;
    uint32_t *nmask;
    uint32_t nReads;
};
CF_DEV void convert_body(const DConvert &c, uint32_t r) {
    if (r >= c.nReads) return;
    const uint64_t o = c.off[r], L = c.off[r + 1] - o, wo = c.woff[r];
    for (uint64_t k = 0; 32 * k < L; k++) {
        uint64_t w = 0;
        uint32_t m = 0;
#pragma unroll
        for (uint32_t g = 0; g < 4; g++) {
            const uint64_t j0 = 32 * k + 8 * g;
            if (j0 >= L) break;
            uint64_t x = load8_any(c.seq, o + j0);
            if (L - j0 < 8) x &= (1ull << (8 * (L - j0))) - 1;
            uint32_t c16, n8;
            squeeze8(x, c16, n8);
            w |= (uint64_t)c16 << (16 * g);
            m |= n8 << (8 * g);
        }
        c.bases[wo + k] = w;
        c.nmask[wo + k] = m;
    }
}
struct DUnpack {
    const uint8_t *dense;
    uint64_t *bases;
    uint32_t *rlen;
    uint32_t nReads, readLen;
    uint64_t *rev;
};
CF_DEV void dense_unpack_body(const DUnpack &u, uint64_t t) {
    const uint32_t W = (u.readLen + 31) >> 5, bpr = (u.readLen + 3) >> 2;
    if (W == 0) { if (t < u.nReads) u.rlen[t] = 0; return; }
    const uint64_t r = t / W;
    const uint32_t k = (uint32_t)(t - r * W);
    if (r >= u.nReads) return;
    uint64_t w = load8_any(u.dense, r * bpr + 8ull * k);
    const uint32_t have = u.readLen - 32 * k;
    if (have < 32) w &= (1ull << (2 * have)) - 1;
    u.bases[r * W + k] = w;
    if (k == 0) u.rlen[r] = u.readLen;
    if (u.rev) {
        const uint32_t L = u.readLen;
        const int32_t s0 = (int32_t)(L - 1 - 32u * k) - 31;
        uint64_t x;
        if (s0 >= 0) {
            const uint64_t at = r * bpr + ((uint32_t)s0 >> 2);
            const uint32_t sh = 2u * ((uint32_t)s0 & 3u);
            x = load8_any(u.dense, at) >> sh;
            if (sh) x |= (load8_any(u.dense, at + 8) & 0xffull) << (64 - sh);
        } else x = load8_any(u.dense, r * bpr) << (2 * (uint32_t)(-s0));
        uint64_t rv = pair_reverse(x);
        if (have < 32) rv &= (1ull << (2 * have)) - 1;
        u.rev[r * W + k] = rv;
    }
}

CF_DEV void rlen_body(const uint64_t *off, uint32_t *rlen, uint32_t nReads, uint32_t r) {
    if (r >= nReads) return;
    const uint64_t l = off[r + 1] - off[r];
    rlen[r] = l > 0xffffffffull ? 0xffffffffu : (uint32_t)l;
}

struct DPlan {
    const uint32_t *nmask;
    const uint32_t *rlen;
    const uint64_t *woff;
    uint32_t nReads;
    int32_t ftabChars;
    uint32_t maxLenAllowed;
    uint64_t nWords;
    uint8_t *pass;
    uint32_t *hitCap;
    uint32_t *slotOf;
    uint64_t *hitBase;
    uint32_t *items;
    uint32_t *itemMeta;
    uint64_t *bases;
    uint32_t revDelta;
    BatchStatus *st;
    uint64_t hitsCap;
};

CF_DEV void plan_body(const DPlan &p, uint32_t r) {
    if (r < p.nReads) {
        const uint64_t L = p.rlen[r], wo = p.woff[r];
        uint32_t nN = 0;
        const bool inside = wo + ((L + 31) >> 5) <= p.nWords;
        if (!inside) cf_atomic_or(&p.st->flags, kStWordsOverflow);
        for (uint64_t k = 0; inside && 32 * k < L; k++) {
            uint32_t m = p.nmask[wo + k];
            if (L - 32 * k < 32) m &= (1u << (L - 32 * k)) - 1u;
            nN += (uint32_t)cf_popc32(m);
        }
        const uint64_t maxns = (uint64_t)(0.0 + (double)0.15f * (double)L);
        bool ok = inside && L >= 2 && nN <= maxns;
        if (ok && L > p.maxLenAllowed) { cf_atomic_or(&p.st->flags, kStLenOverflow); ok = false; }
        const uint32_t cap = ok ? (uint32_t)(nN + (L - nN) / (uint64_t)p.ftabChars + 2) : 0u;
        p.pass[r] = ok ? 1 : 0;
        p.hitCap[r] = cap;
    }
}

CF_DEV uint64_t rev_word(const uint64_t *rw, uint32_t L, uint32_t k) {
    const uint32_t have = L - 32u * k;
    const int32_t s0 = (int32_t)(L - 1 - 32u * k) - 31;
    uint64_t x;
    if (s0 >= 0) {
        const uint32_t wi = (uint32_t)s0 >> 5, sh = (uint32_t)s0 & 31;
        x = rw[wi] >> (2 * sh);
        if (sh) x |= rw[wi + 1] << (64 - 2 * sh);
    } else x = rw[0] << (2 * (uint32_t)(-s0));
    uint64_t w = pair_reverse(x);
    if (have < 32) w &= (1ull << (2 * have)) - 1;
    return w;
}

constexpr uint32_t kItemHasN = 0x80000000u;
constexpr uint32_t kItemPre = 0x40000000u;
CF_DEV void plan_fill_body(const DPlan &p, uint32_t r) {
    if (r > p.nReads) return;
    if (r == p.nReads) {
        const uint64_t need = p.hitBase[r];
        p.st->hitsNeed = need;
        if (need > p.hitsCap) { cf_atomic_or(&p.st->flags, kStHitsOverflow); p.st->nItems = 0; }
        else p.st->nItems = 2u * p.slotOf[r];
        return;
    }
    const uint32_t slot = p.slotOf[r];
    if (p.pass[r]) {
        p.items[slot] = r;
        if (p.itemMeta) {
            const uint32_t wo = (uint32_t)p.woff[r], L = p.rlen[r], hb = (uint32_t)p.hitBase[r];
            uint32_t any = 0;
            for (uint32_t k = 0; 32 * k < L; k++) {
                uint32_t mk = p.nmask[p.woff[r] + k];
                if (L - 32 * k < 32) mk &= (1u << (L - 32 * k)) - 1u;
                any |= mk;
            }
            const bool pre = p.revDelta && !any;
            const uint32_t Lf = L | (any ? kItemHasN : 0u) | (pre ? kItemPre : 0u);
            uint32_t *m = p.itemMeta + 8 * (size_t)slot;
            m[0] = pre ? wo + p.revDelta : wo; m[1] = Lf; m[2] = hb; m[3] = r;
            m[4] = wo; m[5] = Lf; m[6] = hb + p.hitCap[r]; m[7] = r;
        }
    } else p.slotOf[r] = kNone32;
}

CF_DEV void rev_words_body(const DPlan &p, uint32_t wordsPerRead, uint64_t t) {
    const uint64_t r = t / wordsPerRead;
    const uint32_t k = (uint32_t)(t - r * wordsPerRead);
    if (r >= p.nReads || !p.revDelta || !p.pass[r]) return;
    const uint32_t L = p.rlen[r];
    if (32u * k >= L) return;
    const uint64_t wo = p.woff[r];
    p.bases[wo + p.revDelta + k] = rev_word(p.bases + wo, L, k);
}

constexpr uint32_t kMaxScoreNever = 0xffffffffu;
CF_DEV void plan_maxscore_body(const uint32_t *rlen, const uint8_t *pass, uint32_t nQueries, int paired, uint32_t *maxScore, uint32_t q) {
    if (q >= nQueries) return;
    const uint32_t r0 = paired ? 2 * q : q;
    const uint64_t L0 = rlen[r0];
    const uint64_t s0 = L0 > 15 ? (L0 - 15) * (L0 - 15) : 0u;
    const bool p0 = pass[r0] != 0;
    uint64_t v = p0 ? s0 : 0u;
    if (paired) {
        const uint64_t L1 = rlen[r0 + 1];
        const uint64_t s1 = L1 > 15 ? (L1 - 15) * (L1 - 15) : 0u;
        const bool p1 = pass[r0 + 1] != 0;
        v = (p0 && p1) ? s0 + s1 : p0 ? s0 : p1 ? s1 : 0u;
    }
    maxScore[q] = v >= 0xffffffffull ? kMaxScoreNever : (uint32_t)v;
}

struct DCompact {
    const OutRow *out;
    const uint64_t *o1tax, *o1a, *o1b;
    uint64_t oStride;
    const uint32_t *nOut;
    const uint64_t *rowFirst;
    uint32_t k, nQueries;
    OutRow *dst;
    BatchStatus *st;
// ... 1245 lines not shown
    else if (p1) { nm = 1; rds[0] = r0 + 1; firstMate = 1; }
    else nm = 0;
    const uint64_t k = pr.k, m = pr.m;
    uint64_t maxG = k;
    uint32_t rowsTotal = 0;
    uint32_t tsBase = 0;
    bool tsWide = false;
    for (int rdi = 0; rdi < nm; rdi++) {
        const uint32_t rd = rds[rdi], slot = b.slotOf[rd];
        HitP *const pool[2] = {b.hits + b.hitBase[rd], b.hits + b.hitBase[rd] + b.hitCap[rd]};
        HitP *hs[2] = {pool[0], pool[1]};
        const uint32_t hm0 = b.nhml[2 * slot], hm1 = b.nhml[2 * slot + 1];
        const uint32_t n[2] = {nhml_n(hm0), nhml_n(hm1)};
        const bool long0 = nhml_long(hm0), long1 = nhml_long(hm1);
        if (!long0 && !long1) continue;
        const uint32_t need = (long0 ? n[0] : 0u) + (long1 ? n[1] : 0u);
        const bool staged = scratch != nullptr && need <= scratchCap;
        if (staged) {
            hs[0] = scratch; hs[1] = scratch + (long0 ? n[0] : 0u);
            if (long0) hits_copy(hs[0], pool[0], n[0]);
            if (long1) hits_copy(hs[1], pool[1], n[1]);
        }
        if (long0 && long1) post_fix(ix, pr, b, rd, hs, n);
        else post_trim(hs[long0 ? 0 : 1], n[long0 ? 0 : 1]);
        uint64_t tot[2] = {0, 0}, mx[2] = {0, 0};
        for (int f = 0; f < 2; f++) if (f == 0 ? long0 : long1) for (uint32_t i = 0; i < n[f]; i++) {
            const uint64_t len = hp_len(hs[f][i]);
            if (len < m) continue;
            tot[f] += (len - 15) * (len - 15);
            if (len > mx[f]) mx[f] = len;
        }
        int lo, hi;
        if (tot[0] != tot[1]) { lo = tot[0] > tot[1] ? 0 : 1; hi = lo + 1; }
        else if (mx[0] != mx[1]) { lo = mx[0] > mx[1] ? 0 : 1; hi = lo + 1; }
        else { lo = 0; hi = 2; }
        qi.lo[rdi] = (uint8_t)lo; qi.hi[rdi] = (uint8_t)hi;
        for (int f = lo; f < hi; f++) {
            HitP *h = hs[f];
            for (uint32_t i = 0; i < n[f]; i++)
                if (hp_len(h[i]) >= m && hp_size(h[i]) > maxG) maxG = hp_size(h[i]);
            if (maxG > k) maxG += k;
            qi.maxG[rdi][f] = maxG > 0xffffffffull ? 0xffffffffu : (uint32_t)maxG;
            std_sort_hits(h, (int)n[f]);
            uint64_t cnt = 0;
            uint32_t i = 0;
            for (; i < n[f]; i++) {
                const uint64_t len = hp_len(h[i]), size = hp_size(h[i]);
                const uint64_t nelt = plan_nelt(len, size, maxG, m, pr.ihits);
                if (nelt == 0) continue;
                if (nPlanned < kInlinePlan) {
                    PlanHit ph;
                    ph.top = hp_row(h[i]); ph.nelt = (uint32_t)nelt; ph.meta = plan_meta((uint32_t)len, rdi, f, tsBase + i);
                    if (tsBase + i > kPlanTsMax || len > 0xffffu) tsWide = true;
                    b.qplan[(uint64_t)nPlanned * b.qplanStride + q] = ph;
                }
                nPlanned++;
                rowsTotal += (uint32_t)nelt;
                cnt += nelt;
                if (cnt >= maxG) { i++; qi.brk[rdi] |= (uint8_t)(1u << f); break; }
            }
            qi.nProc[rdi][f] = i;
            tsBase += i - ((qi.brk[rdi] >> f) & 1u);
            if (staged) hits_copy(pool[f], h, n[f]);
        }
    }
    const uint32_t nPlan = (nPlanned <= kInlinePlan && !tsWide) ? nPlanned : kPlanNotInline;
    b.qflag[q] = qf_make(nPlan, isPaired, firstMate, (uint32_t)nm);
    if (nPlan == kPlanNotInline) b.qhead[q] = qi;
    b.qRows[q] = rowsTotal;
}

CF_DEV void defer_push(uint32_t *list, uint32_t *counter, bool defer, uint32_t q) {
    const uint64_t mask = cf_ballot(defer);
    if (!mask) return;
    const uint32_t lane = cf_lane();
    const int leader = cf_ctz64(mask);
    uint32_t base = 0;
    if ((int)lane == leader) base = cf_atomic_add(counter, (uint32_t)cf_popc64(mask));
    base = cf_shfl(base, leader);
    if (defer) list[base + (uint32_t)cf_popc64(mask & ((1ull << lane) - 1))] = q;
}

constexpr int kPostFastHits = 8;
CF_DEV bool post_fast_body(const DIndex &ix, const DParams &pr, const DBatch &b, uint32_t q) {
    (void)ix;
    if (b.st->flags & kStHitsOverflow) { b.qRows[q] = 0; return false; }
    uint32_t fOf0 = 2, fOf1 = 2, np0 = 0, np1 = 0, brk0 = 0, brk1 = 0;
    uint8_t isPaired = 0, firstMate = 0;
    const uint32_t r0 = b.paired ? 2 * q : q;
    const bool p0 = b.pass[r0] != 0, p1 = b.paired ? b.pass[r0 + 1] != 0 : false;
    uint32_t rd0 = r0;
    int nm;
    if (b.paired && p0 && p1) { nm = 2; isPaired = 1; }
    else if (p0) nm = 1;
    else if (p1) { nm = 1; rd0 = r0 + 1; firstMate = 1; }
    else nm = 0;
    const uint64_t k = pr.k, m = pr.m;
    uint64_t maxG = k;
    uint32_t rowsTotal = 0, tsBase = 0, nPlanned = 0;
    PlanHit pl0{0, 0, 0}, pl1{0, 0, 0}, pl2{0, 0, 0}, pl3{0, 0, 0};
    static_assert(kInlinePlan == 4, "four plan slots below");
    bool defer = false;
    for (int rdi = 0; rdi < nm && !defer; rdi++) {
        const uint32_t rd = rd0 + (uint32_t)rdi, slot = b.slotOf[rd];
        const uint32_t hm0 = b.nhml[2 * slot], hm1 = b.nhml[2 * slot + 1];
        const bool long0 = nhml_long(hm0), long1 = nhml_long(hm1);
        if (!long0 && !long1) continue;
        if (long0 && long1) { defer = true; break; }
        const int f = long0 ? 0 : 1;
        const uint32_t n = nhml_n(f ? hm1 : hm0);
        if (n > (uint32_t)kPostFastHits) { defer = true; break; }
        const uint8_t *hp = reinterpret_cast<const uint8_t *>(b.hits + b.hitBase[rd] + (f ? b.hitCap[rd] : 0u));
        uint64_t w0[kPostFastHits], w1[kPostFastHits];
#pragma unroll
        for (int i = 0; i < kPostFastHits; i++) {
            u64x2 v{0, 0};
            if ((uint32_t)i < n) v = cf_load16(hp + 16 * i);
            w0[i] = v.x; w1[i] = v.y;
        }
        bool apart = true;
        uint64_t mg = maxG;
#pragma unroll
        for (int i = 0; i < kPostFastHits; i++) {
            if ((uint32_t)i >= n) continue;
            const HitP hi{w0[i], w1[i]};
            const uint64_t len = hp_len(hi), size = hp_size(hi);
            if (len >= m && size > mg) mg = size;
            if (i + 1 < kPostFastHits && (uint32_t)(i + 1) < n) {
                const HitP hj{w0[i + 1], w1[i + 1]};
                const uint64_t bi = hp_bwoff(hi), bj = hp_bwoff(hj);
                if (bi >= bj || bi + len > bj) apart = false;
            }
        }
        if (!apart) { defer = true; break; }
        maxG = mg;
        if (maxG > k) maxG += k;
        uint32_t rank[kPostFastHits];
#pragma unroll
        for (int i = 0; i < kPostFastHits; i++) rank[i] = 0;
#pragma unroll
        for (int i = 0; i < kPostFastHits; i++) {
#pragma unroll
            for (int j = i + 1; j < kPostFastHits; j++) {
                if ((uint32_t)j < n) {
                    const bool jFirst = hit_less(HitP{w0[j], w1[j]}, HitP{w0[i], w1[i]});
                    rank[i] += jFirst ? 1u : 0u;
                    rank[j] += jFirst ? 0u : 1u;
                }
            }
        }
        uint64_t cnt = 0;
        uint32_t visited = n;
        bool stopped = false, brk = false;
#pragma unroll
        for (int r = 0; r < kPostFastHits; r++) {
            if ((uint32_t)r >= n || stopped) continue;
            uint64_t c0 = 0, c1 = 0;
#pragma unroll
            for (int i = 0; i < kPostFastHits; i++) if ((uint32_t)i < n && rank[i] == (uint32_t)r) { c0 = w0[i]; c1 = w1[i]; }
            const HitP c{c0, c1};
            const uint64_t len = hp_len(c), size = hp_size(c);
            uint64_t nelt = 0;
            if (!(len <= m || size == 0)) {
                nelt = size < maxG ? size : maxG;
                if (nelt > pr.ihits) nelt = 0;
            }
            if (nelt == 0) continue;
            const PlanHit ph{hp_row(c), (uint32_t)nelt, plan_meta((uint32_t)len, rdi, f, tsBase + (uint32_t)r)};
            if (tsBase + (uint32_t)r > kPlanTsMax || len > 0xffffu) defer = true;
            if (nPlanned == 0) pl0 = ph; else if (nPlanned == 1) pl1 = ph; else if (nPlanned == 2) pl2 = ph; else if (nPlanned == 3) pl3 = ph;
            nPlanned++;
            rowsTotal += (uint32_t)nelt;
            cnt += nelt;
            if (cnt >= maxG) { visited = (uint32_t)r + 1; brk = true; stopped = true; }
        }
        if (rdi == 0) { fOf0 = (uint32_t)f; np0 = visited; brk0 = brk ? 1u : 0u; }
        else { fOf1 = (uint32_t)f; np1 = visited; brk1 = brk ? 1u : 0u; }
        tsBase += visited - (brk ? 1u : 0u);
    }
    if (defer || nPlanned > kInlinePlan) return true;
    (void)np0; (void)np1; (void)brk0; (void)brk1; (void)fOf0; (void)fOf1;
    b.qflag[q] = qf_make(nPlanned, isPaired, firstMate, (uint32_t)nm);
    if (nPlanned > 0) b.qplan[q] = pl0;
    if (nPlanned > 1) b.qplan[b.qplanStride + q] = pl1;
    if (nPlanned > 2) b.qplan[2 * b.qplanStride + q] = pl2;
    if (nPlanned > 3) b.qplan[3 * b.qplanStride + q] = pl3;
    b.qRows[q] = rowsTotal;
    return false;
}

CF_DEV void row_window_body(const DBatch &b, uint32_t qLo, bool keepSlow = false) {
    BatchStatus &st = *b.st;
    const uint32_t nq = b.nQueries;
    st.rowsTotal = b.qBase[nq];
    st.needRows = 0;
    if (!keepSlow) st.nSlowScore = 0;
    if (st.flags & kStHitsOverflow) { st.qLo = st.qHi = 0; st.rowLo = st.rowHi = 0; return; }
    if (qLo > nq) qLo = nq;
    const uint64_t rowLo = b.qBase[qLo];
    uint32_t lo = qLo, hi = nq;
    while (lo < hi) {
        const uint32_t md = lo + (hi - lo + 1) / 2;
        if (b.qBase[md] - rowLo <= b.rowsCap) lo = md; else hi = md - 1;
    }
    if (lo == qLo && qLo < nq) st.needRows = b.qBase[qLo + 1] - rowLo;
    st.qLo = qLo; st.qHi = lo;
    st.rowLo = rowLo; st.rowHi = b.qBase[lo];
}

template <typename Put>
CF_DEV void for_each_planned_row(const DParams &pr, const DBatch &b, uint32_t q, Put put) {
    if (q < b.st->qLo || q >= b.st->qHi) return;
    const uint32_t nRows = b.qRows[q];
    if (nRows == 0) return;
    const uint32_t qf = b.qflag[q], nPlan = qf_nplan(qf);
    const uint64_t base = b.qBase[q] - b.st->rowLo;
    uint32_t rowoff = 0;
    if (nPlan != kPlanNotInline) {
#pragma unroll
        for (uint32_t j = 0; j < kInlinePlan; j++) {
            if (j >= nPlan) continue;
            const PlanHit ph = b.qplan[(uint64_t)j * b.qplanStride + q];
            for (uint32_t e = 0; e < ph.nelt; e++) put(base + rowoff + e, ph.top + e);
            rowoff += ph.nelt;
        }
        return;
    }
    const QHead *qp = &b.qhead[q];
    const uint32_t r0 = (b.paired ? 2 * q : q) + qf_first(qf);
    const int nMates = qf_nmates(qf);
    for (int rdi = 0; rdi < nMates; rdi++) {
        const uint32_t rd = r0 + rdi;
        const int lo = qp->lo[rdi], hi = qp->hi[rdi];
        for (int f = lo; f < hi; f++) {
            const HitP *h = b.hits + b.hitBase[rd] + (f ? b.hitCap[rd] : 0u);
            const uint32_t np = qp->nProc[rdi][f];
            const uint64_t mg = qp->maxG[rdi][f];
            for (uint32_t i = 0; i < np; i++) {
                const HitP hp = h[i];
                const uint32_t ne = plan_nelt(hp_len(hp), hp_size(hp), mg, pr.m, pr.ihits);
                for (uint32_t e = 0; e < ne; e++) put(base + rowoff + e, hp_row(hp) + e);
                rowoff += ne;
            }
        }
    }
}
CF_DEV void emit_body(const DParams &pr, const DBatch &b, uint32_t q) {
    for_each_planned_row(pr, b, q, [&](uint64_t at, uint64_t row) { b.rowVal[at] = row; });
}

CF_DEV bool try_offset(const DIndex &ix, uint64_t row, uint32_t &ref) {
    if (row == ix.zOff) { ref = 0; return true; }
    if ((row & ((1ull << ix.offRate) - 1)) == 0) {
        const uint64_t e = row >> ix.offRate;
        ref = ix.offw ? static_cast<const uint32_t *>(ix.offs)[e] : static_cast<const uint16_t *>(ix.offs)[e];
        return true;
    }
    if (ix.lastBoundary > 0 && row <= ix.lastBoundary) {
        const uint64_t blk = row >> ix.boundShift;
        if ((ix.boundBits[blk >> 5] >> (blk & 31)) & 1u) {
            uint32_t lo = 0, hi = ix.nBound;
            while (lo < hi) { const uint32_t md = (lo + hi) >> 1; if (ix.boundRow[md] < row) lo = md + 1; else hi = md; }
            if (lo < ix.nBound && ix.boundRow[lo] == row) {
                ref = ix.offw ? ix.boundRef[lo] : (ix.boundRef[lo] & 0xffffu);
                return true;
            }
        }
    }
    return false;
}
// ... 168 lines not shown
    uint32_t steps = 0;
    b.rowRef[i] = resolve_row(ix, b.rowVal[i], steps);
    if (COUNT && steps) cf_atomic_add(&b.ops->nWalk, (unsigned long long)steps);
}
CF_DEV void resolve_query_body(const DIndex &ix, const DParams &pr, const DBatch &b, uint32_t q) {
    for_each_planned_row(pr, b, q, [&](uint64_t at, uint64_t row) { uint32_t steps = 0; b.rowRef[at] = resolve_row(ix, row, steps); });
}

CF_DEV bool host_has(const DParams &pr, uint64_t tid) {
    uint32_t lo = 0, hi = pr.nHostSet;
    while (lo < hi) { const uint32_t md = (lo + hi) >> 1; if (pr.hostSet[md] < tid) lo = md + 1; else hi = md; }
    return lo < pr.nHostSet && pr.hostSet[lo] == tid;
}

CF_DEV uint32_t lcg_next(uint32_t &last) {
    last = 1664525u * last + 1013904223u;
    uint32_t ret = last >> 16;
    last = 1664525u * last + 1013904223u;
    return ret ^ last;
}

CF_DEV uint32_t path_len(const HmEntry &e) { return e.pid == kNone32 ? 0u : 10u; }
CF_DEV uint64_t path_at(const DIndex &ix, const HmEntry &e, uint32_t slot) { return ix.paths[(uint64_t)e.pid * 10 + slot]; }
CF_DEV uint32_t path_tidx_at(const DIndex &ix, const HmEntry &e, uint32_t slot) { return ix.pathTidx[(uint64_t)e.pid * 10 + slot]; }

CF_DEV void ref_taxon_of(const DIndex &ix, const DParams &pr, const RefInfo &ri, uint64_t &tax, uint32_t &tidx, uint32_t &pid, uint32_t &rank) {
    tax = ri.tax; tidx = ri.tidx; pid = ri.pid;
    const uint32_t plen = pid == kNone32 ? 0u : 10u;
    rank = pr.rankSlot;
    if (rank > 0) {
        for (; rank < plen; rank++) {
            const uint64_t t = ix.paths[(uint64_t)pid * 10 + rank];
            if (t != 0) { tax = t; tidx = ix.pathTidx[(uint64_t)pid * 10 + rank]; break; }
        }
    }
}
CF_DEV void ref_taxon(const DIndex &ix, const DParams &pr, uint32_t ref, uint64_t &tax, uint32_t &tidx, uint32_t &pid, uint32_t &rank) {
    ref_taxon_of(ix, pr, ix.refInfo[ref], tax, tidx, pid, rank);
}

constexpr uint32_t kCountSlotBits = 12, kCountSlots = 1u << kCountSlotBits, kCountChunk = 32768, kCountProbes = 8, kCountEmpty = 0xffffffffu;
CF_DEV void count_body(const DBatch &b, uint32_t *lds, uint32_t chunk, uint32_t slotBits, bool direct) {
    const uint32_t t = cf_local_thread(), nt = cf_block_threads();
    const uint32_t nSlots = 1u << slotBits;
    uint32_t *keys = lds, *cnt = lds + nSlots, *unq = lds + 2 * nSlots;
    for (uint32_t i = t; i < nSlots; i += nt) { keys[i] = kCountEmpty; cnt[i] = 0; unq[i] = 0; }
    cf_block_sync();
    const uint32_t q0 = chunk * kCountChunk, qLo = b.st->qLo, qHi = b.st->qHi;
    for (uint32_t i = t; i < kCountChunk; i += nt) {
        const uint32_t q = q0 + i;
        if (q < qLo || q >= qHi) continue;
        const uint32_t no = b.nOut[q];
        if (no > kFieldRows) continue;
        const bool one = no <= 1;
#pragma unroll
        for (uint32_t j = 0; j < kFieldRows; j++) {
            if (j >= (no ? no : 1u)) continue;
            const uint32_t tidx = no ? (uint32_t)(b.o1b[j * b.oStride + q] >> 32) : 0u;
            if (tidx >= b.nTaxa) continue;
            const uint32_t h = direct ? tidx : (tidx * 0x9e3779b1u) >> (32u - slotBits);
            bool placed = false;
            for (uint32_t pr = 0; pr < kCountProbes && !placed; pr++) {
                const uint32_t s = (h + pr) & (nSlots - 1);
                uint32_t k = keys[s];
                if (k == kCountEmpty) k = cf_atomic_cas(&keys[s], kCountEmpty, tidx);
                if (k == kCountEmpty || k == tidx) { cf_atomic_add(&cnt[s], 1u); if (one) cf_atomic_add(&unq[s], 1u); placed = true; }
            }
            if (!placed) {
                cf_atomic_add(&b.counts[tidx], 1ull);
                if (one) cf_atomic_add(&b.counts[b.nTaxa + tidx], 1ull);
            }
        }
    }
    cf_block_sync();
    for (uint32_t i = t; i < nSlots; i += nt) {
        const uint32_t k = keys[i], n = cnt[i], u = unq[i];
        if (k == kCountEmpty || n == 0) continue;
        cf_atomic_add(&b.counts[k], (unsigned long long)n);
        if (u) cf_atomic_add(&b.counts[b.nTaxa + k], (unsigned long long)u);
    }
}

constexpr uint32_t kScoreFastRows = 8, kFastEntries = 4;
template <bool EARLY = false>
CF_DEV bool score_fast_body(const DIndex &ix, const DParams &pr, const DBatch &b, uint32_t q) {
    if (EARLY) {
        if (b.postDeferred[q] || (b.st->flags & kStHitsOverflow)) { b.nOut[q] = 0; b.score2[q] = 0; return !(b.st->flags & kStHitsOverflow); }
    } else if (q < b.st->qLo || q >= b.st->qHi) {
        if (b.st->qLo == 0) b.nOut[q] = 0;
        return false;
    }
    const uint32_t qf = b.qflag[q], nPlan = qf_nplan(qf), nRows = b.qRows[q];
    if (nPlan == kPlanNotInline || nRows > kScoreFastRows) { if (EARLY) { b.nOut[q] = 0; b.score2[q] = 0; } return true; }
    const uint64_t base = EARLY ? 0 : b.qBase[q] - b.st->rowLo;
    uint64_t eTax[kFastEntries];
    uint32_t eRef[kFastEntries], eTidx[kFastEntries], eTs[kFastEntries], eSc[kFastEntries][4], eHl[kFastEntries][4];
#pragma unroll
    for (uint32_t z = 0; z < kFastEntries; z++) {
        eTax[z] = 0; eRef[z] = 0; eTidx[z] = 0; eTs[z] = 0;
#pragma unroll
        for (int c = 0; c < 4; c++) { eSc[z][c] = 0; eHl[z][c] = 0; }
    }
    uint64_t pTop[kInlinePlan];
    uint32_t pNelt[kInlinePlan], pMeta[kInlinePlan];
#pragma unroll
    for (uint32_t j = 0; j < kInlinePlan; j++) {
        PlanHit ph{0, 0, 0};
        if (j < nPlan) ph = b.qplan[(uint64_t)j * b.qplanStride + q];
        pTop[j] = ph.top; pNelt[j] = ph.nelt; pMeta[j] = ph.meta;
    }
    static_assert(kInlinePlan == 4, "three thresholds below");
    const uint32_t c1 = pNelt[0], c2 = c1 + pNelt[1], c3 = c2 + pNelt[2];
    uint32_t total = c3 + pNelt[3];
    if (total > kScoreFastRows) total = kScoreFastRows;
    constexpr uint32_t kGather = 4;
    uint32_t nh = 0;
    for (uint32_t s0 = 0; s0 < total; s0 += kGather) {
        uint64_t rowv[kGather];
        uint32_t rmeta[kGather], ref[kGather];
#pragma unroll
        for (uint32_t i = 0; i < kGather; i++) {
            const uint32_t s = s0 + i;
            const bool g1 = s >= c1, g2 = s >= c2, g3 = s >= c3;
            rowv[i] = (g3 ? pTop[3] : g2 ? pTop[2] : g1 ? pTop[1] : pTop[0]) + (s - (g3 ? c3 : g2 ? c2 : g1 ? c1 : 0u));
            rmeta[i] = g3 ? pMeta[3] : g2 ? pMeta[2] : g1 ? pMeta[1] : pMeta[0];
            ref[i] = 0xffffffffu;
        }
        bool act[kGather], isPos[kGather];
#pragma unroll
        for (uint32_t i = 0; i < kGather; i++) { act[i] = s0 + i < total; isPos[i] = act[i] && (rowv[i] & kRowIsPos) != 0; }
        if (b.directRefs) {
            uint32_t tref[kGather];
            if (ix.offw) {
#pragma unroll
                for (uint32_t i = 0; i < kGather; i++) tref[i] = static_cast<const uint32_t *>(ix.walkOffs)[act[i] && !isPos[i] ? rowv[i] : 0ull];
            } else {
#pragma unroll
                for (uint32_t i = 0; i < kGather; i++) tref[i] = static_cast<const uint16_t *>(ix.walkOffs)[act[i] && !isPos[i] ? rowv[i] : 0ull];
            }
            if (ix.posFrag) {
                uint64_t lh[kGather];
#pragma unroll
                for (uint32_t i = 0; i < kGather; i++)
                    lh[i] = cf_load8(reinterpret_cast<const uint8_t *>(ix.posBucket + (isPos[i] ? (rowv[i] & ~kRowIsPos) >> ix.posShift : 0ull)));
                uint32_t lo[kGather], hi[kGather];
                bool narrow = false;
#pragma unroll
                for (uint32_t i = 0; i < kGather; i++) {
                    lo[i] = isPos[i] ? (uint32_t)lh[i] : 0u;
                    hi[i] = isPos[i] ? (uint32_t)(lh[i] >> 32) + 1 : 0u;
                    if (hi[i] > ix.nPosFrag) hi[i] = ix.nPosFrag;
                    narrow = narrow || hi[i] - lo[i] > 1;
                }
                while (narrow) {
                    uint64_t fx[kGather];
#pragma unroll
                    for (uint32_t i = 0; i < kGather; i++) fx[i] = ix.posFrag[hi[i] - lo[i] > 1 ? (lo[i] + hi[i]) >> 1 : 0u].x;
                    narrow = false;
#pragma unroll
                    for (uint32_t i = 0; i < kGather; i++) {
                        if (hi[i] - lo[i] > 1) { const uint32_t md = (lo[i] + hi[i]) >> 1; if (fx[i] <= (rowv[i] & ~kRowIsPos)) lo[i] = md; else hi[i] = md; }
                        narrow = narrow || hi[i] - lo[i] > 1;
                    }
                }
                uint32_t sq[kGather];
#pragma unroll
                for (uint32_t i = 0; i < kGather; i++) sq[i] = (uint32_t)ix.posFrag[lo[i]].y;
                u64x2 span[kGather];
#pragma unroll
                for (uint32_t i = 0; i < kGather; i++) span[i] = ix.posSeq[isPos[i] ? sq[i] : 0u];
                bool leave = false;
#pragma unroll
                for (uint32_t i = 0; i < kGather; i++) {
                    const uint64_t pos = rowv[i] & ~kRowIsPos;
                    if (isPos[i] && !(pos >= span[i].x + ix.walkMax && pos + 12 <= span[i].y)) leave = true;
                    if (isPos[i]) tref[i] = sq[i];
                }
                if (leave) { if (EARLY) { b.nOut[q] = 0; b.score2[q] = 0; } return true; }
            }
#pragma unroll
            for (uint32_t i = 0; i < kGather; i++) if (act[i]) ref[i] = tref[i];
        } else {
#pragma unroll
            for (uint32_t i = 0; i < kGather; i++) { const uint32_t v = b.rowRef[act[i] ? base + s0 + i : 0ull]; if (act[i]) ref[i] = v; }
        }
        RefInfo ri[kGather];
        uint8_t rex[kGather];
#pragma unroll
        for (uint32_t i = 0; i < kGather; i++) ri[i] = ix.refInfo[ref[i] < ix.nRef ? ref[i] : 0u];
#pragma unroll
        for (uint32_t i = 0; i < kGather; i++) rex[i] = pr.refExcluded ? pr.refExcluded[ref[i] < ix.nRef ? ref[i] : 0u] : (uint8_t)0;
#pragma unroll
        for (uint32_t i = 0; i < kGather; i++) {
            if (s0 + i >= total) continue;
            if (ref[i] >= ix.nRef) continue;
            if (rex[i]) continue;
            const uint32_t len = pm_len(rmeta[i]), ts = pm_ts(rmeta[i]);
            const uint32_t col = 2u * (uint32_t)pm_rdi(rmeta[i]) + (uint32_t)pm_f(rmeta[i]);
            const uint32_t sc = (len - 15) * (len - 15);
            uint64_t tax; uint32_t tidx, pid, rank;
            ref_taxon_of(ix, pr, ri[i], tax, tidx, pid, rank);
            uint32_t at = kFastEntries;
#pragma unroll
            for (uint32_t z = 0; z < kFastEntries; z++)
                if (z < nh && at == kFastEntries && (pr.rankSlot == 0 ? eRef[z] == ref[i] : eTax[z] == tax)) at = z;
            bool add = true;
            if (at == kFastEntries) {
                if (nh == kFastEntries) { if (EARLY) { b.nOut[q] = 0; b.score2[q] = 0; } return true; }
                at = nh++;
#pragma unroll
                for (uint32_t z = 0; z < kFastEntries; z++) if (z == at) { eTax[z] = tax; eRef[z] = ref[i]; eTidx[z] = tidx; eTs[z] = ts; }
            } else {
#pragma unroll
                for (uint32_t z = 0; z < kFastEntries; z++) if (z == at) { add = eTs[z] != ts; eTs[z] = ts; }
            }
            if (add) {
#pragma unroll
                for (uint32_t z = 0; z < kFastEntries; z++) {
#pragma unroll
                    for (uint32_t c = 0; c < 4; c++) if (z == at && c == col) { eSc[z][c] += sc; eHl[z][c] += len; }
                }
            }
        }
    }
    if (nh > pr.k) { if (EARLY) { b.nOut[q] = 0; b.score2[q] = 0; } return true; }
    const bool paired = qf_paired(qf);
    uint32_t score[kFastEntries], hitLen[kFastEntries];
#pragma unroll
    for (uint32_t z = 0; z < kFastEntries; z++) {
        score[z] = eSc[z][0] > eSc[z][1] ? eSc[z][0] : eSc[z][1];
        hitLen[z] = eHl[z][0] > eHl[z][1] ? eHl[z][0] : eHl[z][1];
        if (paired) { score[z] += eSc[z][2] > eSc[z][3] ? eSc[z][2] : eSc[z][3]; hitLen[z] += eHl[z][2] > eHl[z][3] ? eHl[z][2] : eHl[z][3]; }
    }
    bool onlyHost = false;
    if (pr.nHostSet) {
        uint32_t best = 0;
#pragma unroll
        for (uint32_t z = 0; z < kFastEntries; z++) {
            if (z >= nh) continue;
            if (score[z] > best) { best = score[z]; onlyHost = host_has(pr, eTax[z]); }
            else if (score[z] == best) onlyHost = onlyHost || host_has(pr, eTax[z]);
        }
    }
    uint32_t res[kFastEntries], rs[kFastEntries], nres = 0;
#pragma unroll
    for (uint32_t z = 0; z < kFastEntries; z++) { res[z] = 0; rs[z] = 0; }
#pragma unroll
    for (uint32_t z = 0; z < kFastEntries; z++) {
        if (z >= nh) continue;
        if (onlyHost && !host_has(pr, eTax[z])) continue;
#pragma unroll
        for (uint32_t i = 0; i < kFastEntries; i++) if (i == nres) { res[i] = z; rs[i] = score[z]; }
        nres++;
    }
    const uint32_t r0 = b.paired ? 2 * q : q;
    if (nres == 0) {
        b.nOut[q] = 0; b.score2[q] = 0;
        return false;
    }
    uint32_t score2 = 0;
    {
        uint32_t bst = 0, sec = 0; bool hb = false, hs = false;
#pragma unroll
        for (uint32_t i = 0; i < kFastEntries; i++) {
            if (i >= nres) continue;
            const uint32_t v = rs[i];
            if (!hb || v > bst) { sec = bst; hs = hb; bst = v; hb = true; }
            else if (!hs || v > sec) { sec = v; hs = true; }
        }
        score2 = hs ? sec : 0;
    }
    uint32_t pos[kFastEntries], ps[kFastEntries];
#pragma unroll
    for (uint32_t p = 0; p < kFastEntries; p++) { pos[p] = 0; ps[p] = 0; }
#pragma unroll
    for (uint32_t i = 0; i < kFastEntries; i++) {
        if (i >= nres) continue;
        uint32_t place = 0;
#pragma unroll
        for (uint32_t j = 0; j < kFastEntries; j++) if (j < nres && j != i && (rs[j] > rs[i] || (rs[j] == rs[i] && j > i))) place++;
#pragma unroll
        for (uint32_t p = 0; p < kFastEntries; p++) if (p == place) { pos[p] = i; ps[p] = rs[i]; }
    }
    if (nres > 1) {
        uint32_t rnd = b.seeds[r0];
        if (paired) rnd ^= b.seeds[r0 + 1];
        uint32_t streak = 0;
#pragma unroll
        for (uint32_t i = 1; i <= kFastEntries; i++) {
            if (i > nres) continue;
            bool tie = false;
#pragma unroll
            for (uint32_t p = 1; p < kFastEntries; p++) if (p == i && i < nres) tie = ps[p] == ps[p - 1];
            if (tie) { if (streak == 0) streak = 1; streak++; }
            else {
                if (streak > 1) {
                    const uint32_t begin = i - streak;
#pragma unroll
                    for (uint32_t z = 0; z + 1 < kFastEntries; z++) {
                        if (z < begin || z + 1 >= begin + streak) continue;
                        const uint32_t left = streak - (z - begin);
                        const uint32_t r = lcg_next(rnd) % left;
#pragma unroll
                        for (uint32_t t = 1; t < kFastEntries; t++)
                            if (r == t && z + t < kFastEntries) { const uint32_t x = pos[z]; pos[z] = pos[z + t < kFastEntries ? z + t : z]; pos[z + t < kFastEntries ? z + t : z] = x; }
                    }
                }
                streak = 0;
            }
        }
    }
    uint32_t num = nres < pr.k ? nres : pr.k;
#pragma unroll
    for (uint32_t i = 0; i + 1 < kFastEntries; i++) if (i + 1 < num && ps[i] != ps[i + 1]) num = i + 1;
#pragma unroll
    for (uint32_t i = 0; i < kFastEntries; i++) {
        if (i >= num) continue;
        uint32_t z = 0;
#pragma unroll
        for (uint32_t p = 0; p < kFastEntries; p++) if (p == i) z = pos[p];
        uint32_t en = 0;
#pragma unroll
        for (uint32_t y = 0; y < kFastEntries; y++) if (y == z) en = res[y];
        uint64_t tax = 0; uint32_t ref = 0, tidx = 0, sco = 0, hle = 0;
#pragma unroll
        for (uint32_t y = 0; y < kFastEntries; y++) if (y == en) { tax = eTax[y]; ref = eRef[y]; tidx = eTidx[y]; sco = score[y]; hle = hitLen[y]; }
        static_assert(kFastEntries <= kFieldRows, "every row of the common-case kernel goes out by field");
        b.o1tax[i * b.oStride + q] = tax; b.o1a[i * b.oStride + q] = (uint64_t)ref | ((uint64_t)sco << 32); b.o1b[i * b.oStride + q] = (uint64_t)hle | ((uint64_t)tidx << 32);
    }
    b.nOut[q] = num; b.score2[q] = score2;
    return false;
}

constexpr uint32_t score_scratch_bytes(uint32_t rows) { return rows * (uint32_t)(sizeof(HmEntry) + sizeof(TcEntry) + sizeof(uint32_t)); }
CF_DEV void score_body(const DIndex &ix, const DParams &pr, const DBatch &b, uint32_t q, uint8_t *scratch = nullptr, uint32_t scratchRows = 0,
                       uint32_t rowsMin = 0, uint32_t rowsMax = 0xffffffffu) {
    if (q < b.st->qLo || q >= b.st->qHi) return;
    if (b.qRows[q] < rowsMin || b.qRows[q] > rowsMax) return;
    const uint32_t qf = b.qflag[q], nPlanQ = qf_nplan(qf);
    const bool qPaired = qf_paired(qf);
    const uint32_t k = pr.k;
    OutRow *out = b.out + (uint64_t)q * k;
    const uint64_t base = b.qBase[q] - b.st->rowLo;
    HmEntry *hm = b.hm + base;
    TcEntry *tc = b.tc + base;
    uint32_t *refBase = b.rowRef + base;
    {
        const uint32_t rowsQ = b.qRows[q];
        if (scratch != nullptr && rowsQ <= scratchRows) {
            hm = reinterpret_cast<HmEntry *>(scratch);
            tc = reinterpret_cast<TcEntry *>(scratch + sizeof(HmEntry) * scratchRows);
            uint32_t *lr = reinterpret_cast<uint32_t *>(scratch + (sizeof(HmEntry) + sizeof(TcEntry)) * scratchRows);
            uint32_t i = 0;
            for (; i + 4 <= rowsQ; i += 4) { const uint32_t a = refBase[i], c1 = refBase[i + 1], c2 = refBase[i + 2], c3 = refBase[i + 3]; lr[i] = a; lr[i + 1] = c1; lr[i + 2] = c2; lr[i + 3] = c3; }
            for (; i < rowsQ; i++) lr[i] = refBase[i];
            refBase = lr;
        }
    }
    uint32_t nh = 0;
    const uint32_t r0 = (b.paired ? 2 * q : q);
    uint32_t rowoff = 0;
    auto addHit = [&](uint32_t ne, uint32_t len, int rdi, int f, uint32_t ts) {
        uint32_t *refs = refBase + rowoff;
        rowoff += ne;
        uint32_t nid = 0;
        for (uint32_t e = 0; e < ne; e++) {
            const uint32_t ref = refs[e];
            bool found = false;
            for (uint32_t z = 0; z < nid && !found; z++) found = refs[z] == ref;
            if (!found) refs[nid++] = ref;
        }
        const uint32_t sc = (len - 15) * (len - 15);
        for (uint32_t z = 0; z < nid; z++) {
            const uint32_t ref = refs[z];
            if (ref >= ix.nRef) continue;
            if (pr.refExcluded && pr.refExcluded[ref]) continue;
            uint64_t tax; uint32_t tidx, pid, rank;
            ref_taxon(ix, pr, ref, tax, tidx, pid, rank);
            uint32_t idx = 0;
            for (; idx < nh; idx++) {
                const bool same = rank == 0 ? (hm[idx].uniqueID == ref) : (hm[idx].taxID == tax);
                if (same) {
                    if (hm[idx].ts != ts) { hm[idx].sc[rdi][f] += sc; hm[idx].hl[rdi][f] += len; hm[idx].ts = ts; }
                    break;
                }
            }
            if (idx >= nh) {
                HmEntry e;
                e.taxID = tax; e.uniqueID = ref; e.pid = pid; e.tidx = tidx;
                e.sc[0][0] = e.sc[0][1] = e.sc[1][0] = e.sc[1][1] = 0;
                e.hl[0][0] = e.hl[0][1] = e.hl[1][0] = e.hl[1][1] = 0;
                e.sc[rdi][f] = sc; e.hl[rdi][f] = len;
                e.ts = ts; e.score = 0; e.hitLen = 0; e.rank = (uint8_t)rank;
                for (int z2 = 0; z2 < 7; z2++) e.pad[z2] = 0;
                hm[nh++] = e;
            }
        }
    };
    if (nPlanQ != kPlanNotInline) {
        for (uint32_t j = 0; j < nPlanQ; j++) {
            const PlanHit ph = b.qplan[(uint64_t)j * b.qplanStride + q];
            addHit(ph.nelt, pm_len(ph.meta), pm_rdi(ph.meta), pm_f(ph.meta), pm_ts(ph.meta));
        }
    } else {
        const QHead *qp = &b.qhead[q];
        uint32_t ts = 0;
        for (int rdi = 0; rdi < qf_nmates(qf); rdi++) {
            const uint32_t rd = r0 + qf_first(qf) + rdi;
            for (int f = qp->lo[rdi]; f < qp->hi[rdi]; f++) {
                const HitP *h = b.hits + b.hitBase[rd] + (f ? b.hitCap[rd] : 0u);
                const uint32_t np = qp->nProc[rdi][f];
                const uint64_t mg = qp->maxG[rdi][f];
                for (uint32_t i = 0; i < np; i++, ts++) {
                    const HitP hp = h[i];
// ... 150 lines not shown
```

### centrifuge_amd/csrc/cf_scan.hpp

```cpp
#pragma once
#include <hip/hip_runtime.h>

#include <cstdint>

namespace cfamd {

enum : int { SCAN_WORDS = 0, SCAN_PLAIN = 1, SCAN_HITS = 2 };
constexpr int kScanBlock = 256, kScanPer = 16, kScanTile = kScanBlock * kScanPer;

template <int MODE>
__device__ __forceinline__ uint64_t scan_value(uint32_t x) {
    return MODE == SCAN_WORDS ? (((uint64_t)x + 31) >> 5) : MODE == SCAN_HITS ? 2ull * x : (uint64_t)x;
}

__device__ __forceinline__ void scan_load(const uint32_t *in, uint64_t n, uint64_t first, uint32_t (&x)[kScanPer]) {
    if (first + kScanPer <= n) {
        const uint4 *p = reinterpret_cast<const uint4 *>(in + first);
#pragma unroll
        for (int i = 0; i < kScanPer / 4; i++) { const uint4 v = p[i]; x[4 * i] = v.x; x[4 * i + 1] = v.y; x[4 * i + 2] = v.z; x[4 * i + 3] = v.w; }
    } else {
#pragma unroll
        for (int i = 0; i < kScanPer; i++) x[i] = first + i < n ? in[first + i] : 0u;
    }
}

__device__ __forceinline__ void scan_block_reduce(uint64_t &a, uint32_t &c, uint64_t *ldsA, uint32_t *ldsC) {
#pragma unroll
    for (int m = 32; m > 0; m >>= 1) { a += __shfl_xor(a, m, 64); c += __shfl_xor(c, m, 64); }
    const int w = threadIdx.x >> 6;
    if ((threadIdx.x & 63) == 0) { ldsA[w] = a; ldsC[w] = c; }
    __syncthreads();
    a = 0; c = 0;
#pragma unroll
    for (int i = 0; i < kScanBlock / 64; i++) { a += ldsA[i]; c += ldsC[i]; }
}

template <int MODE>
__global__ void __launch_bounds__(kScanBlock) k_scan_sums(const uint32_t *in, uint64_t n, uint64_t *tileA, uint32_t *tileC) {
    __shared__ uint64_t ldsA[kScanBlock / 64];
    __shared__ uint32_t ldsC[kScanBlock / 64];
    uint32_t x[kScanPer];
    scan_load(in, n, (uint64_t)blockIdx.x * kScanTile + (uint64_t)threadIdx.x * kScanPer, x);
    uint64_t a = 0;
    uint32_t c = 0;
#pragma unroll
    for (int i = 0; i < kScanPer; i++) { a += scan_value<MODE>(x[i]); if (MODE == SCAN_HITS) c += x[i] != 0; }
    scan_block_reduce(a, c, ldsA, ldsC);
    if (threadIdx.x == 0) { tileA[blockIdx.x] = a; if (MODE == SCAN_HITS) tileC[blockIdx.x] = c; }
}

__global__ void __launch_bounds__(kScanBlock) k_scan_tiles(uint64_t *tileA, uint32_t *tileC, uint32_t nTiles, bool withC) {
    __shared__ uint64_t sA[kScanBlock];
    __shared__ uint32_t sC[kScanBlock];
    uint64_t carryA = 0;
    uint32_t carryC = 0;
    for (uint32_t base = 0; base < nTiles; base += kScanBlock) {
        const uint32_t i = base + threadIdx.x;
        const uint64_t a = i < nTiles ? tileA[i] : 0;
        const uint32_t c = (withC && i < nTiles) ? tileC[i] : 0;
        sA[threadIdx.x] = a; sC[threadIdx.x] = c;
        __syncthreads();
        for (int d = 1; d < kScanBlock; d <<= 1) {
            const uint64_t ta = threadIdx.x >= (unsigned)d ? sA[threadIdx.x - d] : 0;
            const uint32_t tc = threadIdx.x >= (unsigned)d ? sC[threadIdx.x - d] : 0;
            __syncthreads();
            sA[threadIdx.x] += ta; sC[threadIdx.x] += tc;
            __syncthreads();
        }
        if (i < nTiles) { tileA[i] = carryA + sA[threadIdx.x] - a; if (withC) tileC[i] = carryC + sC[threadIdx.x] - c; }
        carryA += sA[kScanBlock - 1]; carryC += sC[kScanBlock - 1];
        __syncthreads();
    }
}

template <int MODE>
__global__ void __launch_bounds__(kScanBlock) k_scan_write(const uint32_t *in, uint64_t n, const uint64_t *tileA, const uint32_t *tileC,
                                                            uint64_t *outA, uint32_t *outC) {
    __shared__ uint64_t ldsA[kScanBlock / 64];
    __shared__ uint32_t ldsC[kScanBlock / 64];
    const uint64_t first = (uint64_t)blockIdx.x * kScanTile + (uint64_t)threadIdx.x * kScanPer;
    uint32_t x[kScanPer];
    scan_load(in, n, first, x);
    uint64_t a = 0;
    uint32_t c = 0;
#pragma unroll
    for (int i = 0; i < kScanPer; i++) { a += scan_value<MODE>(x[i]); if (MODE == SCAN_HITS) c += x[i] != 0; }
    uint64_t ia = a;
    uint32_t ic = c;
    const int lane = threadIdx.x & 63, w = threadIdx.x >> 6;
#pragma unroll
    for (int d = 1; d < 64; d <<= 1) {
        const uint64_t ta = __shfl_up(ia, d, 64);
        const uint32_t tc = __shfl_up(ic, d, 64);
        if (lane >= d) { ia += ta; ic += tc; }
    }
    if (lane == 63) { ldsA[w] = ia; ldsC[w] = ic; }
    __syncthreads();
    uint64_t offA = tileA[blockIdx.x] + ia - a;
    uint32_t offC = (MODE == SCAN_HITS ? tileC[blockIdx.x] : 0u) + ic - c;
    for (int i = 0; i < w; i++) { offA += ldsA[i]; offC += ldsC[i]; }
#pragma unroll
    for (int i = 0; i < kScanPer; i++) {
        const uint64_t idx = first + i;
        if (idx <= n) { outA[idx] = offA; if (MODE == SCAN_HITS) outC[idx] = offC; }
        offA += scan_value<MODE>(x[i]);
        if (MODE == SCAN_HITS) offC += x[i] != 0;
    }
}

inline uint32_t scan_tiles_for(uint64_t n) { return (uint32_t)((n + 1 + kScanTile - 1) / kScanTile); }

template <int MODE>
inline void scan_enqueue(const uint32_t *in, uint64_t n, uint64_t *outA, uint32_t *outC, uint64_t *tileA, uint32_t *tileC, hipStream_t st) {
    const uint32_t tiles = scan_tiles_for(n);
    hipLaunchKernelGGL((k_scan_sums<MODE>), dim3(tiles), dim3(kScanBlock), 0, st, in, n, tileA, tileC);
    hipLaunchKernelGGL(k_scan_tiles, dim3(1), dim3(kScanBlock), 0, st, tileA, tileC, tiles, MODE == SCAN_HITS);
    hipLaunchKernelGGL((k_scan_write<MODE>), dim3(tiles), dim3(kScanBlock), 0, st, in, n, (const uint64_t *)tileA, (const uint32_t *)tileC, outA, outC);
}

}
```

Baseline: 1.431 billion.

## Fuse post/score fast paths, plan scan sums, and control-block memsets

Adds a combined post+score fast kernel so queries resolved in the post fast path are scored in the same pass, and only leftovers go to the slow lists. It also fuses the hit-cap tile sums into k_plan, folds the maxscore kernel into plan_fill, and skips the word-offset scan when dense unpack already produced it. Status, cursor and op counters now share one control buffer so several memsets become one, and the row window is computed inside a fused scan-tiles kernel. The aim is fewer kernel launches and fewer global passes per batch. The cost is larger, more complex kernels and more places where subtle ordering or clearing bugs could appear.

```diff
diff --git a/centrifuge_amd/csrc/cf_device.hip b/centrifuge_amd/csrc/cf_device.hip
--- a/centrifuge_amd/csrc/cf_device.hip
+++ b/centrifuge_amd/csrc/cf_device.hip
@@ -4,6 +4,7 @@
 
 #include <algorithm>
 #include <cmath>
+#include <cstddef>
 #include <chrono>
 #include <cstdio>
 #include <cstdlib>
@@ -117,6 +118,21 @@
     const bool d = q < b.nQueries ? score_fast_body<EARLY>(ix, pr, b, q) : false;
     defer_push(b.slowScore, &b.st->nSlowScore, d, q);
 }
+__global__ void __launch_bounds__(256) k_post_score_fast(DIndex ix, DParams pr, DBatch b) {
+    const uint32_t q = cf_global_thread();
+    const uint32_t left = q < b.nQueries ? post_score_fast_body(ix, pr, b, q) : 0u;
+    defer_push(b.slowPost, &b.st->nSlowPost, (left & kLeftPost) != 0, q);
+    defer_push(b.slowScore, &b.st->nSlowScore, (left & kLeftScore) != 0, q);
+}
+__global__ void __launch_bounds__(64) k_score_fast_listed(DIndex ix, DParams pr, DBatch b) {
+    const uint32_t n = b.st->nSlowPost;
+    for (uint32_t i0 = blockIdx.x * 64u; i0 < n; i0 += gridDim.x * 64u) {
+        const uint32_t i = i0 + threadIdx.x;
+        const uint32_t q = i < n ? b.slowPost[i] : 0u;
+        const bool d = i < n ? score_fast_listed_body(ix, pr, b, q) : false;
+        defer_push(b.slowScore, &b.st->nSlowScore, d, q);
+    }
+}
 __global__ void __launch_bounds__(256) k_list_all(uint32_t *list, uint32_t *counter, uint32_t n) {
     const uint32_t q = cf_global_thread();
     if (q < n) list[q] = q;
@@ -133,6 +149,51 @@
     if (i < b.st->nItems / 2) post_fix(ix, pr, b, b.items[i]);
 }
 __global__ void k_window(DBatch b, uint32_t qLo, bool keepSlow) { if (cf_global_thread() == 0) row_window_body(b, qLo, keepSlow); }
+__global__ void __launch_bounds__(kScanBlock) k_scan_tiles_window(uint64_t *tileA, uint32_t nTiles, DBatch b, bool keepSlow) {
+    __shared__ uint64_t part[kScanBlock];
+    __shared__ uint32_t tileAt;
+    const uint64_t total = scan_tiles_body(tileA, nullptr, nTiles, false);
+    BatchStatus &st = *b.st;
+    const uint32_t nq = b.nQueries;
+    const bool overflow = (st.flags & kStHitsOverflow) != 0;
+    const bool fits = total <= b.rowsCap;
+    if (!overflow && !fits) {
+        __syncthreads();
+        if (threadIdx.x == 0) {
+            uint32_t lo = 0, hi = nTiles - 1;
+            while (lo < hi) { const uint32_t md = lo + (hi - lo + 1) / 2; if (tileA[md] <= b.rowsCap) lo = md; else hi = md - 1; }
+            tileAt = lo;
+        }
+        __syncthreads();
+        uint32_t x[kScanPer];
+        scan_load(b.qRows, nq, (uint64_t)tileAt * kScanTile + (uint64_t)threadIdx.x * kScanPer, x);
+        uint64_t a = 0;
+#pragma unroll
+        for (int i = 0; i < kScanPer; i++) a += x[i];
+        part[threadIdx.x] = a;
+        __syncthreads();
+    }
+    if (threadIdx.x != 0) return;
+    st.rowsTotal = total;
+    st.needRows = 0;
+    if (!keepSlow) st.nSlowScore = 0;
+    if (overflow) { st.qLo = st.qHi = 0; st.rowLo = st.rowHi = 0; return; }
+    uint32_t qHi = nq;
+    uint64_t rowHi = total;
+    if (!fits) {
+        uint64_t off = tileA[tileAt];
+        uint32_t j = 0;
+        while (j < (uint32_t)kScanBlock && off + part[j] <= b.rowsCap) off += part[j++];
+        uint64_t qq = (uint64_t)tileAt * kScanTile + (uint64_t)j * kScanPer;
+        if (j < (uint32_t)kScanBlock)
+            for (int i = 0; i < kScanPer && qq < nq && off + b.qRows[qq] <= b.rowsCap; i++) off += b.qRows[qq++];
+        qHi = qq < nq ? (uint32_t)qq : nq;
+        rowHi = off;
+        if (qHi == 0 && nq > 0) st.needRows = b.qRows[0];
+    }
+    st.qLo = 0; st.qHi = qHi;
+    st.rowLo = 0; st.rowHi = rowHi;
+}
 __global__ void __launch_bounds__(256) k_emit(DParams pr, DBatch b) {
     const uint32_t q = cf_global_thread();
     if (q < b.nQueries) emit_body(pr, b, q);
@@ -222,12 +283,24 @@
     __shared__ uint32_t slots[3 * kCountSlots];
     count_body(b, slots, blockIdx.x, slotBits, direct);
 }
-__global__ void __launch_bounds__(256) k_plan(DPlan p) { plan_body(p, cf_global_thread()); }
-__global__ void __launch_bounds__(256) k_plan_fill(DPlan p) { plan_fill_body(p, cf_global_thread()); }
+__global__ void __launch_bounds__(kScanBlock) k_plan(DPlan p, uint64_t *tileA, uint32_t *tileC) {
+    __shared__ uint64_t ldsA[kScanBlock / 64];
+    __shared__ uint32_t ldsC[kScanBlock / 64];
+    uint64_t a = 0;
+    uint32_t c = 0;
+    for (int i = 0; i < kScanPer; i++) {
+        const uint64_t r = (uint64_t)blockIdx.x * kScanTile + (uint64_t)i * kScanBlock + threadIdx.x;
+        const uint32_t cap = r < p.nReads ? plan_body(p, (uint32_t)r) : 0u;
+        a += 2ull * cap; c += cap != 0;
+    }
+    scan_block_reduce(a, c, ldsA, ldsC);
+    if (threadIdx.x == 0) { tileA[blockIdx.x] = a; tileC[blockIdx.x] = c; }
+}
+__global__ void __launch_bounds__(256) k_plan_fill(DPlan p, uint32_t nQueries, int paired, uint32_t *maxScore) {
+    plan_fill_body(p, cf_global_thread());
+    plan_maxscore_body(p.rlen, p.pass, nQueries, paired, maxScore, cf_global_thread());
+}
 __global__ void __launch_bounds__(256) k_rev_words(DPlan p, uint32_t wordsPerRead) { rev_words_body(p, wordsPerRead, (uint64_t)blockIdx.x * blockDim.x + threadIdx.x); }
-__global__ void __launch_bounds__(256) k_plan_maxscore(const uint32_t *rlen, const uint8_t *pass, uint32_t nQueries, int paired, uint32_t *maxScore) {
-    plan_maxscore_body(rlen, pass, nQueries, paired, maxScore, cf_global_thread());
-}
 __global__ void __launch_bounds__(256) k_compact(DCompact c) {
     compact_body(c, cf_global_thread());
 }
@@ -357,6 +430,8 @@
         n = count;
     }
 };
+
+constexpr size_t kCtlStatus = (sizeof(BatchStatus) + 15) / 16 * 16;
 
 struct cf_batch {
     cf_classifier *cl = nullptr;
@@ -400,9 +475,12 @@
     DevBuf<HmEntry> hm;
     DevBuf<TcEntry> tc;
     DevBuf<OutRow> out, outCompact;
-    DevBuf<OpCounts> ops;
-    DevBuf<unsigned long long> cursor;
-    DevBuf<BatchStatus> st;
+    DevBuf<uint8_t> ctl;
+    BatchStatus *st = nullptr;
+    unsigned long long *cursor = nullptr;
+    OpCounts *ops = nullptr;
+    bool woffMade = false;
+    bool fusedPass = false;
     uint64_t hitsCapLimit = 0, rowsCapLimit = 0;
     DPlan pl{};
     DBatch d{};
@@ -1295,7 +1373,17 @@
     bt->slowPost.ensure(nq + 1); bt->slowScore.ensure(nq + 1);
     if (envInt("CF_EARLY_SCORE", 0)) bt->postDeferred.ensure(nq + 16);
     bt->out.ensure(nq * (uint64_t)cl->d.k + 1); bt->nOut.ensure(nq + 16); bt->score2.ensure(nq + 1); bt->rowFirst.ensure(nq + 1);
-    bt->cursor.ensure(4); bt->ops.ensure(1); bt->st.ensure(1);
+    static_assert(kCtlStatus % 16 == 0 && offsetof(BatchStatus, nSlowPost) % 16 == 0 && (kCtlStatus - offsetof(BatchStatus, nSlowPost) + 32 + sizeof(OpCounts)) % 16 == 0, "whole 16-byte pieces");
+    static_assert(offsetof(BatchStatus, nSlowScore) + 4 == sizeof(BatchStatus) && offsetof(BatchStatus, nSlowPost) + 8 == sizeof(BatchStatus) && sizeof(BatchStatus) % 8 == 0,
+                  "nSlowPost, nSlowScore end the status block: enqueueClassify clears from there on");
+    if (!bt->ctl.n) {
+        bt->ctl.alloc(kCtlStatus + 32 + sizeof(OpCounts));
+        if (bt->ctl.p) {
+            bt->st = reinterpret_cast<BatchStatus *>(bt->ctl.p);
+            bt->cursor = reinterpret_cast<unsigned long long *>(bt->ctl.p + kCtlStatus);
+            bt->ops = reinterpret_cast<OpCounts *>(bt->ctl.p + kCtlStatus + 32);
+        }
+    }
     bt->tileA.ensure(scan_tiles_for(std::max(nReads, nq)) + 1); bt->tileC.ensure(scan_tiles_for(std::max(nReads, nq)) + 1);
     bt->recWords = searchVersion() != 2 ? 0u : maxLen <= 128 ? 4u : maxLen <= 192 ? 6u : maxLen <= 256 ? 8u : 0u;
     if ((uint64_t)(0.15 * maxLen) + maxLen / (uint64_t)ftc + 3 >= 255) bt->recWords = 0;
@@ -1333,7 +1421,7 @@
     pl.maxLenAllowed = bt->maxLenHost;
     pl.nWords = bt->nWords;
     pl.pass = bt->pass.p; pl.hitCap = bt->hitCap.p; pl.slotOf = bt->slotOf.p;
-    pl.hitBase = bt->hitBase.p; pl.items = bt->items.p; pl.st = bt->st.p;
+    pl.hitBase = bt->hitBase.p; pl.items = bt->items.p; pl.st = bt->st;
     pl.itemMeta = bt->selfRecords ? bt->itemMeta.p : nullptr;
     pl.bases = bt->bases.p; pl.revDelta = bt->revDelta;
     pl.hitsCap = bt->hitsCapLimit ? std::min<uint64_t>(bt->hitsCapLimit, bt->hits.n) : bt->hits.n;
@@ -1347,7 +1435,7 @@
     d.out = bt->out.p; d.nOut = bt->nOut.p; d.score2 = bt->score2.p;
     d.counts = cl->counts.p; d.nTaxa = (uint32_t)cl->ix->h.taxa.size();
     d.nReads = (uint32_t)bt->nReads; d.nQueries = (uint32_t)bt->nQueries; d.paired = bt->paired;
-    d.cursor = bt->cursor.p; d.st = bt->st.p; d.ops = bt->ops.p;
+    d.cursor = bt->cursor; d.st = bt->st; d.ops = bt->ops;
     d.slowPost = bt->slowPost.p; d.slowScore = bt->slowScore.p; d.postDeferred = envInt("CF_EARLY_SCORE", 0) ? bt->postDeferred.p : nullptr;
     d.o1tax = bt->o1tax.p; d.o1a = bt->o1a.p; d.o1b = bt->o1b.p; d.oStride = bt->o1tax.n / kFieldRows;
     d.hitsCap = pl.hitsCap;
@@ -1362,17 +1450,18 @@
     HIP_OK(hipStreamWaitEvent(st, bt->ev[8], 0));
     if (bt->densePending) {
         const uint32_t L = bt->densePending - 1;
-        const DUnpack u{bt->dense.p, bt->bases.p, bt->rlen.p, (uint32_t)nReads, L, bt->revDelta ? bt->bases.p + bt->revDelta : nullptr};
+        const DUnpack u{bt->dense.p, bt->bases.p, bt->rlen.p, (uint32_t)nReads, L, bt->revDelta ? bt->bases.p + bt->revDelta : nullptr, bt->woff.p};
         bt->revMade = bt->revDelta != 0;
+        bt->woffMade = nReads != 0;
         const uint64_t threads = nReads * std::max<uint64_t>(((uint64_t)L + 31) >> 5, 1);
         hipLaunchKernelGGL(k_dense_unpack, dim3((unsigned)((threads + 255) / 256)), dim3(256), 0, st, u);
         bt->densePending = 0;
     }
     HIP_OK(hipEventRecord(bt->ev[5], st));
-    HIP_OK(hipMemsetAsync(bt->st.p, 0, sizeof(BatchStatus), st));
+    HIP_OK(hipMemsetAsync(bt->st, 0, kCtlStatus, st));
     const dim3 gp((unsigned)((nReads + 1 + 255) / 256)), bl(256);
     if (bt->fromBytes && nReads) hipLaunchKernelGGL(k_rlen, gp, bl, 0, st, bt->off8.p, bt->rlen.p, (uint32_t)nReads);
-    scan_enqueue<SCAN_WORDS>(bt->rlen.p, nReads, bt->woff.p, nullptr, bt->tileA.p, bt->tileC.p, st);
+    if (!bt->woffMade) scan_enqueue<SCAN_WORDS>(bt->rlen.p, nReads, bt->woff.p, nullptr, bt->tileA.p, bt->tileC.p, st);
     if (bt->fromBytes && nReads) {
         DConvert c{bt->seq.p, bt->off8.p, bt->woff.p, bt->bases.p, bt->nmask.p, (uint32_t)nReads};
         hipLaunchKernelGGL(k_convert, dim3((unsigned)((nReads + 255) / 256)), dim3(256), 0, st, c);
@@ -1381,15 +1470,13 @@
         const DTextPack c{bt->text.p, bt->txSeqOff.p, bt->rlen.p, bt->woff.p, bt->bases.p, bt->nmask.p, (uint32_t)nReads};
         hipLaunchKernelGGL(k_text_pack, dim3((unsigned)((nReads + 255) / 256)), dim3(256), 0, st, c);
     }
-    hipLaunchKernelGGL(k_plan, gp, bl, 0, st, pl);
-    scan_enqueue<SCAN_HITS>(bt->hitCap.p, nReads, bt->hitBase.p, bt->slotOf.p, bt->tileA.p, bt->tileC.p, st);
-    hipLaunchKernelGGL(k_plan_fill, gp, bl, 0, st, pl);
+    hipLaunchKernelGGL(k_plan, dim3(scan_tiles_for(nReads)), dim3(kScanBlock), 0, st, pl, bt->tileA.p, bt->tileC.p);
+    scan_enqueue<SCAN_HITS>(bt->hitCap.p, nReads, bt->hitBase.p, bt->slotOf.p, bt->tileA.p, bt->tileC.p, st, true);
+    hipLaunchKernelGGL(k_plan_fill, gp, bl, 0, st, pl, (uint32_t)bt->nQueries, bt->paired, bt->maxScore.p);
     if (pl.revDelta && nReads && !bt->revMade) {
         const uint64_t threads = nReads * (uint64_t)bt->recWords;
         hipLaunchKernelGGL(k_rev_words, dim3((unsigned)((threads + 255) / 256)), bl, 0, st, pl, bt->recWords);
     }
-    if (bt->nQueries) hipLaunchKernelGGL(k_plan_maxscore, dim3((unsigned)((bt->nQueries + 255) / 256)), bl, 0, st, bt->rlen.p, bt->pass.p,
-                                         (uint32_t)bt->nQueries, bt->paired, bt->maxScore.p);
     if (bt->recWords && !bt->selfRecords && nReads) {
         const uint64_t threads = 2 * nReads * (uint64_t)bt->recWords;
         hipLaunchKernelGGL(k_pack, dim3((unsigned)((threads + 255) / 256)), bl, 0, st, bt->d, bt->recs.p, bt->recWords);
@@ -1403,6 +1490,12 @@
 static bool earlyScoreMode(const cf_batch *bt) {
     static const bool on = envInt("CF_EARLY_SCORE", 0) != 0 && envInt("CF_POST_FAST", 1) != 0 && envInt("CF_SCORE_FAST", 1) != 0 && envInt("CF_TAIL_STREAM", 0) == 0;
     return on && bt->d.directRefs != 0 && bt->tail != nullptr && bt->nQueries != 0;
+}
+
+static bool fusedPostScore(const cf_batch *bt) {
+    static const bool on = envInt("CF_FUSE_POST_SCORE", 1) != 0 && envInt("CF_POST_FAST", 1) != 0 && envInt("CF_SCORE_FAST", 1) != 0 && envInt("CF_EARLY_SCORE", 0) == 0 &&
+                           envInt("CF_TAIL_STREAM", 0) == 0;
+    return on && bt->d.directRefs != 0 && bt->nQueries != 0;
 }
 
 static void enqueuePost(cf_batch *bt, hipStream_t st) {
@@ -1412,8 +1505,9 @@
     const uint32_t nq = (uint32_t)bt->nQueries;
     if (!nq) return;
     static const bool fast = envInt("CF_POST_FAST", 1) != 0;
-    if (fast) hipLaunchKernelGGL(k_post_fast, dim3((nq + 255) / 256), dim3(256), 0, st, ix.d, cl->d, d);
-    else hipLaunchKernelGGL(k_list_all, dim3((nq + 255) / 256), dim3(256), 0, st, bt->slowPost.p, &bt->st.p->nSlowPost, nq);
+    if (fusedPostScore(bt)) hipLaunchKernelGGL(k_post_score_fast, dim3((nq + 255) / 256), dim3(256), 0, st, ix.d, cl->d, d);
+    else if (fast) hipLaunchKernelGGL(k_post_fast, dim3((nq + 255) / 256), dim3(256), 0, st, ix.d, cl->d, d);
+    else hipLaunchKernelGGL(k_list_all, dim3((nq + 255) / 256), dim3(256), 0, st, bt->slowPost.p, &bt->st->nSlowPost, nq);
     if (earlyScoreMode(bt)) {
         HIP_OK(hipEventRecord(bt->evPostFast, st));
         HIP_OK(hipStreamWaitEvent(bt->tail, bt->evPostFast, 0));
@@ -1426,6 +1520,7 @@
     static const bool postLds = envInt("CF_POST_LDS", 0) != 0;
     const uint32_t capHits = postLds ? (uint32_t)std::min<uint64_t>(60, 2 * ((uint64_t)bt->maxLenHost / (uint64_t)std::max(1, ix.h.g.ftabChars) + 2)) : 0u;
     hipLaunchKernelGGL(k_post, listGrid(ix, nq), dim3(64), (size_t)64 * capHits * sizeof(HitP), st, ix.d, cl->d, d, capHits);
+    if (fusedPostScore(bt)) hipLaunchKernelGGL(k_score_fast_listed, listGrid(ix, nq), dim3(64), 0, st, ix.d, cl->d, d);
 }
 
 static bool enqueueRowPass(cf_batch *bt, uint32_t qLo, hipStream_t st, bool marks, hipStream_t late = nullptr, bool early = false) {
@@ -1434,8 +1529,10 @@
     const DBatch &d = bt->d;
     const uint32_t nq = (uint32_t)bt->nQueries;
     static const bool fast = envInt("CF_SCORE_FAST", 1) != 0;
-    HIP_OK(hipMemsetAsync(bt->cursor.p + 1, 0, 8, st));
-    hipLaunchKernelGGL(k_window, dim3(1), dim3(64), 0, st, d, qLo, early);
+    if (!marks) {
+        HIP_OK(hipMemsetAsync(bt->cursor + 1, 0, 8, st));
+        hipLaunchKernelGGL(k_window, dim3(1), dim3(64), 0, st, d, qLo, early);
+    }
     const bool direct = d.directRefs != 0;
     if (nq && !direct) hipLaunchKernelGGL(k_emit, dim3((nq + 255) / 256), dim3(256), 0, st, cl->d, d);
     if (marks) HIP_OK(hipEventRecord(bt->ev[2], st));
@@ -1444,7 +1541,7 @@
     if (nq) {
         if (early) {}
         else if (fast) hipLaunchKernelGGL(k_score_fast<false>, dim3((nq + 255) / 256), dim3(256), 0, st, ix.d, cl->d, d);
-        else hipLaunchKernelGGL(k_list_all, dim3((nq + 255) / 256), dim3(256), 0, st, bt->slowScore.p, &bt->st.p->nSlowScore, nq);
+        else hipLaunchKernelGGL(k_list_all, dim3((nq + 255) / 256), dim3(256), 0, st, bt->slowScore.p, &bt->st->nSlowScore, nq);
         if (late && late != st) {
             HIP_OK(hipEventRecord(bt->evLate, st));
             HIP_OK(hipStreamWaitEvent(late, bt->evLate, 0));
@@ -1465,21 +1562,19 @@
     const dim3 g((nq + 1 + 255) / 256), bl(256);
     scan_enqueue<SCAN_PLAIN>(bt->nOut.p, nq, bt->rowFirst.p, nullptr, bt->tileA.p, bt->tileC.p, st);
     const bool narrow = bt->resultFormat == CF_RESULTS_NARROW;
-    const DCompact c{bt->out.p, bt->o1tax.p, bt->o1a.p, bt->o1b.p, bt->d.oStride, bt->nOut.p, bt->rowFirst.p, (uint32_t)bt->cl->d.k, nq, bt->outCompact.p, bt->st.p,
+    const DCompact c{bt->out.p, bt->o1tax.p, bt->o1a.p, bt->o1b.p, bt->d.oStride, bt->nOut.p, bt->rowFirst.p, (uint32_t)bt->cl->d.k, nq, bt->outCompact.p, bt->st,
                      narrow ? reinterpret_cast<NarrowRow *>(bt->outCompact.p) : nullptr, bt->qinfo.p, bt->pass.p, bt->paired};
     hipLaunchKernelGGL(k_compact, g, bl, 0, st, c);
 }
 
 static void enqueueClassify(cf_batch *bt, hipStream_t st) {
     cf_classifier *cl = bt->cl;
-    HIP_OK(hipMemsetAsync(bt->cursor.p, 0, 32, st));
-    HIP_OK(hipMemsetAsync(bt->ops.p, 0, sizeof(OpCounts), st));
+    HIP_OK(hipMemsetAsync(&bt->st->nSlowPost, 0, kCtlStatus - offsetof(BatchStatus, nSlowPost) + 32 + sizeof(OpCounts), st));
     static const bool allFast = envInt("CF_POST_FAST", 1) != 0 && envInt("CF_SCORE_FAST", 1) != 0;
     if (!allFast) {
         HIP_OK(hipMemsetAsync(bt->qRows.p, 0, 4 * (bt->nQueries + 1), st));
         HIP_OK(hipMemsetAsync(bt->nOut.p, 0, 4 * (bt->nQueries + 1), st));
     }
-    HIP_OK(hipMemsetAsync(&bt->st.p->nSlowPost, 0, 8, st));
     HIP_OK(hipEventRecord(bt->ev[0], st));
     bool counted = true;
     if (bt->nReads) counted = launchSearch(cl, bt, st) && counted;
@@ -1488,9 +1583,16 @@
     hipStream_t ts = bt->tail && tailMode == 1 ? bt->tail : st;
     hipStream_t late = bt->tail && tailMode == 2 ? bt->tail : ts;
     if (ts != st) HIP_OK(hipStreamWaitEvent(ts, bt->ev[1], 0));
-    const bool early = earlyScoreMode(bt);
+    bt->fusedPass = fusedPostScore(bt);
+    const bool early = earlyScoreMode(bt) || bt->fusedPass;
     enqueuePost(bt, ts);
-    scan_enqueue<SCAN_PLAIN>(bt->qRows.p, bt->nQueries, bt->qBase.p, nullptr, bt->tileA.p, bt->tileC.p, ts);
+    {
+        const uint32_t tiles = scan_tiles_for(bt->nQueries);
+        hipLaunchKernelGGL((k_scan_sums<SCAN_PLAIN>), dim3(tiles), dim3(kScanBlock), 0, ts, (const uint32_t *)bt->qRows.p, (uint64_t)bt->nQueries, bt->tileA.p, bt->tileC.p);
+        hipLaunchKernelGGL(k_scan_tiles_window, dim3(1), dim3(kScanBlock), 0, ts, bt->tileA.p, tiles, bt->d, early);
+        hipLaunchKernelGGL((k_scan_write<SCAN_PLAIN>), dim3(tiles), dim3(kScanBlock), 0, ts, (const uint32_t *)bt->qRows.p, (uint64_t)bt->nQueries, (const uint64_t *)bt->tileA.p,
+                           (const uint32_t *)bt->tileC.p, bt->qBase.p, (uint32_t *)nullptr);
+    }
     counted = enqueueRowPass(bt, 0, ts, true, late, early) && counted;
     enqueueCompact(bt, late);
     HIP_OK(hipEventRecord(bt->ev[9], late));
@@ -1503,8 +1605,8 @@
 static void enqueueDownload(cf_batch *bt, hipStream_t st) {
     const uint64_t nq = bt->nQueries;
     HIP_OK(hipStreamWaitEvent(st, bt->ev[9], 0));
-    HIP_OK(hipMemcpyAsync(bt->hSt.p, bt->st.p, sizeof(BatchStatus), hipMemcpyDeviceToHost, st));
-    HIP_OK(hipMemcpyAsync(bt->hOps.p, bt->ops.p, sizeof(OpCounts), hipMemcpyDeviceToHost, st));
+    HIP_OK(hipMemcpyAsync(bt->hSt.p, bt->st, sizeof(BatchStatus), hipMemcpyDeviceToHost, st));
+    HIP_OK(hipMemcpyAsync(bt->hOps.p, bt->ops, sizeof(OpCounts), hipMemcpyDeviceToHost, st));
     if (nq && !bt->rowsStay) {
         const uint64_t spec = std::min<uint64_t>(bt->rowsSpec, nq * (uint64_t)bt->cl->d.k);
         if (bt->resultFormat == CF_RESULTS_NARROW) {
@@ -1532,7 +1634,7 @@
     bool redo = false;
     auto fetchStatus = [&] {
         HIP_OK(hipEventSynchronize(bt->ev[9]));
-        HIP_OK(hipMemcpyAsync(bt->hSt.p, bt->st.p, sizeof(BatchStatus), hipMemcpyDeviceToHost, st));
+        HIP_OK(hipMemcpyAsync(bt->hSt.p, bt->st, sizeof(BatchStatus), hipMemcpyDeviceToHost, st));
         HIP_OK(hipStreamSynchronize(st));
         HIP_OK(hipGetLastError());
     };
@@ -1561,7 +1663,7 @@
             bt->rowVal.ensure(need); bt->rowRef.ensure(need); bt->hm.ensure(need); bt->tc.ensure(need);
             bindBatch(bt);
         }
-        enqueueRowPass(bt, bt->hSt.p->qHi, st, false);
+        enqueueRowPass(bt, bt->hSt.p->qHi, st, false, nullptr, bt->fusedPass);
         bt->passes++;
         bt->opsValid = false;
         fetchStatus();
@@ -1617,7 +1719,7 @@
     }
     if (nReads) HIP_OK(hipMemcpyAsync(bt->seeds.p, seeds, nReads * 4, hipMemcpyHostToDevice, st));
     HIP_OK(hipEventRecord(bt->ev[8], st));
-    bt->fromBytes = true; bt->fromText = false; bt->densePending = 0; bt->revMade = false; bt->nmaskZeroOf = nullptr;
+    bt->fromBytes = true; bt->fromText = false; bt->densePending = 0; bt->revMade = false; bt->woffMade = false; bt->nmaskZeroOf = nullptr;
     bt->loaded = true; bt->planned = false; bt->running = false; bt->finished = false;
 }
 
@@ -1656,7 +1758,7 @@
         HIP_OK(hipMemcpyAsync(bt->seeds.p, in->seeds, in->n_reads * 4, hipMemcpyHostToDevice, st));
     }
     HIP_OK(hipEventRecord(bt->ev[8], st));
-    bt->fromBytes = false; bt->fromText = false; bt->densePending = 0; bt->revMade = false;
+    bt->fromBytes = false; bt->fromText = false; bt->densePending = 0; bt->revMade = false; bt->woffMade = false;
     bt->loaded = true; bt->planned = false; bt->running = false; bt->finished = false;
 }
 
@@ -1675,7 +1777,7 @@
         HIP_OK(hipMemcpyAsync(bt->seeds.p, in->seeds, in->n_reads * 4, hipMemcpyHostToDevice, st));
         if (nWords) uploadSparseMask(bt, in->nword_idx, in->nword_mask, in->n_nwords, nWords, st);
     }
-    bt->densePending = in->n_reads ? in->read_len + 1 : 0; bt->revMade = false;
+    bt->densePending = in->n_reads ? in->read_len + 1 : 0; bt->revMade = false; bt->woffMade = false;
     HIP_OK(hipEventRecord(bt->ev[8], st));
     bt->fromBytes = false; bt->fromText = false;
     bt->loaded = true; bt->planned = false; bt->running = false; bt->finished = false;
@@ -1739,7 +1841,7 @@
     sizeBatch(bt, nReads, ts.words(), ts.bases(), ts.maxLen, nBlocks == 2);
     bindBatch(bt);
     HIP_OK(hipEventRecord(bt->ev[8], st));
-    bt->fromText = true; bt->fromBytes = false; bt->densePending = 0; bt->revMade = false; bt->nmaskZeroOf = nullptr;
+    bt->fromText = true; bt->fromBytes = false; bt->densePending = 0; bt->revMade = false; bt->woffMade = false; bt->nmaskZeroOf = nullptr;
     bt->loaded = true;
     info->n_reads = nReads; info->n_bases = ts.bases(); info->max_len = ts.maxLen;
 }
@@ -2161,13 +2263,13 @@
         cf_classifier *cl = bt->cl;
         const cf_status st = guard([&] {
             HIP_OK(hipSetDevice(cl->ix->device));
-            HIP_OK(hipMemset(bt->cursor.p, 0, 32));
-            HIP_OK(hipMemset(bt->ops.p, 0, sizeof(OpCounts)));
+            HIP_OK(hipMemset(bt->cursor, 0, 32));
+            HIP_OK(hipMemset(bt->ops, 0, sizeof(OpCounts)));
             if (bt->nReads) launchSearch(cl, bt, nullptr, 0, true);
             if (bt->nQueries && !bt->d.directRefs) launchWalk(cl, bt, nullptr, true);
             HIP_OK(hipDeviceSynchronize());
             HIP_OK(hipGetLastError());
-            HIP_OK(hipMemcpy(&bt->lastOps, bt->ops.p, sizeof(OpCounts), hipMemcpyDeviceToHost));
+            HIP_OK(hipMemcpy(&bt->lastOps, bt->ops, sizeof(OpCounts), hipMemcpyDeviceToHost));
             bt->lastOps.nRows = bt->rowsTotal;
             bt->opsValid = true;
         });
@@ -2338,10 +2440,10 @@
     std::unique_ptr<cf_batch> own(bt);
     return guard([&] {
         BatchStatus hs{};
-        HIP_OK(hipMemcpy(&hs, bt->st.p, sizeof hs, hipMemcpyDeviceToHost));
+        HIP_OK(hipMemcpy(&hs, bt->st, sizeof hs, hipMemcpyDeviceToHost));
         if (hs.nItems == 0) return;
-        HIP_OK(hipMemset(bt->cursor.p, 0, 32));
-        HIP_OK(hipMemset(bt->ops.p, 0, sizeof(OpCounts)));
+        HIP_OK(hipMemset(bt->cursor, 0, 32));
+        HIP_OK(hipMemset(bt->ops, 0, sizeof(OpCounts)));
         bt->d.lazyHits = 0;
         launchSearch(cl, bt, nullptr, 1);
         hipLaunchKernelGGL(k_postfix_only, dim3(1), dim3(64), 0, 0, cl->ix->d, cl->d, bt->d);
diff --git a/centrifuge_amd/csrc/cf_kernels.hpp b/centrifuge_amd/csrc/cf_kernels.hpp
--- a/centrifuge_amd/csrc/cf_kernels.hpp
+++ b/centrifuge_amd/csrc/cf_kernels.hpp
@@ -490,13 +490,18 @@
     uint32_t *rlen;
     uint32_t nReads, readLen;
     uint64_t *rev;
+    uint64_t *woff;
 };
 CF_DEV void dense_unpack_body(const DUnpack &u, uint64_t t) {
     const uint32_t W = (u.readLen + 31) >> 5, bpr = (u.readLen + 3) >> 2;
-    if (W == 0) { if (t < u.nReads) u.rlen[t] = 0; return; }
+    if (W == 0) {
+        if (t < u.nReads) { u.rlen[t] = 0; if (u.woff) { u.woff[t] = 0; if (t == 0) u.woff[u.nReads] = 0; } }
+        return;
+    }
     const uint64_t r = t / W;
     const uint32_t k = (uint32_t)(t - r * W);
     if (r >= u.nReads) return;
+    if (u.woff && k == 0) { u.woff[r] = r * W; if (r + 1 == u.nReads) u.woff[r + 1] = (r + 1) * W; }
     uint64_t w = load8_any(u.dense, r * bpr + 8ull * k);
     const uint32_t have = u.readLen - 32 * k;
     if (have < 32) w &= (1ull << (2 * have)) - 1;
@@ -544,7 +549,8 @@
     uint64_t hitsCap;
 };
 
-CF_DEV void plan_body(const DPlan &p, uint32_t r) {
+CF_DEV uint32_t plan_body(const DPlan &p, uint32_t r) {
+    uint32_t capOut = 0;
     if (r < p.nReads) {
         const uint64_t L = p.rlen[r], wo = p.woff[r];
         uint32_t nN = 0;
@@ -561,7 +567,9 @@
         const uint32_t cap = ok ? (uint32_t)(nN + (L - nN) / (uint64_t)p.ftabChars + 2) : 0u;
         p.pass[r] = ok ? 1 : 0;
         p.hitCap[r] = cap;
-    }
+        capOut = cap;
+    }
+    return capOut;
 }
 
 CF_DEV uint64_t rev_word(const uint64_t *rw, uint32_t L, uint32_t k) {
@@ -1973,9 +1981,11 @@
 }
 
 constexpr int kPostFastHits = 8;
-CF_DEV bool post_fast_body(const DIndex &ix, const DParams &pr, const DBatch &b, uint32_t q) {
-    (void)ix;
-    if (b.st->flags & kStHitsOverflow) { b.qRows[q] = 0; return false; }
+struct FastPlan {
+    PlanHit pl0, pl1, pl2, pl3;
+    uint32_t nPlanned, rowsTotal, qf;
+};
+CF_DEV bool post_fast_plan(const DParams &pr, const DBatch &b, uint32_t q, FastPlan &fp) {
     uint32_t fOf0 = 2, fOf1 = 2, np0 = 0, np1 = 0, brk0 = 0, brk1 = 0;
     uint8_t isPaired = 0, firstMate = 0;
     const uint32_t r0 = b.paired ? 2 * q : q;
@@ -2071,12 +2081,24 @@
     }
     if (defer || nPlanned > kInlinePlan) return true;
     (void)np0; (void)np1; (void)brk0; (void)brk1; (void)fOf0; (void)fOf1;
-    b.qflag[q] = qf_make(nPlanned, isPaired, firstMate, (uint32_t)nm);
-    if (nPlanned > 0) b.qplan[q] = pl0;
-    if (nPlanned > 1) b.qplan[b.qplanStride + q] = pl1;
-    if (nPlanned > 2) b.qplan[2 * b.qplanStride + q] = pl2;
-    if (nPlanned > 3) b.qplan[3 * b.qplanStride + q] = pl3;
-    b.qRows[q] = rowsTotal;
+    fp.pl0 = pl0; fp.pl1 = pl1; fp.pl2 = pl2; fp.pl3 = pl3;
+    fp.nPlanned = nPlanned; fp.rowsTotal = rowsTotal; fp.qf = qf_make(nPlanned, isPaired, firstMate, (uint32_t)nm);
+    return false;
+}
+CF_DEV void post_fast_store(const DBatch &b, uint32_t q, const FastPlan &fp) {
+    b.qflag[q] = fp.qf;
+    if (fp.nPlanned > 0) b.qplan[q] = fp.pl0;
+    if (fp.nPlanned > 1) b.qplan[b.qplanStride + q] = fp.pl1;
+    if (fp.nPlanned > 2) b.qplan[2 * b.qplanStride + q] = fp.pl2;
+    if (fp.nPlanned > 3) b.qplan[3 * b.qplanStride + q] = fp.pl3;
+}
+CF_DEV bool post_fast_body(const DIndex &ix, const DParams &pr, const DBatch &b, uint32_t q) {
+    (void)ix;
+    if (b.st->flags & kStHitsOverflow) { b.qRows[q] = 0; return false; }
+    FastPlan fp;
+    if (post_fast_plan(pr, b, q, fp)) return true;
+    post_fast_store(b, q, fp);
+    b.qRows[q] = fp.rowsTotal;
     return false;
 }
 
@@ -2411,17 +2433,9 @@
 }
 
 constexpr uint32_t kScoreFastRows = 8, kFastEntries = 4;
-template <bool EARLY = false>
-CF_DEV bool score_fast_body(const DIndex &ix, const DParams &pr, const DBatch &b, uint32_t q) {
-    if (EARLY) {
-        if (b.postDeferred[q] || (b.st->flags & kStHitsOverflow)) { b.nOut[q] = 0; b.score2[q] = 0; return !(b.st->flags & kStHitsOverflow); }
-    } else if (q < b.st->qLo || q >= b.st->qHi) {
-        if (b.st->qLo == 0) b.nOut[q] = 0;
-        return false;
-    }
-    const uint32_t qf = b.qflag[q], nPlan = qf_nplan(qf), nRows = b.qRows[q];
-    if (nPlan == kPlanNotInline || nRows > kScoreFastRows) { if (EARLY) { b.nOut[q] = 0; b.score2[q] = 0; } return true; }
-    const uint64_t base = EARLY ? 0 : b.qBase[q] - b.st->rowLo;
+template <bool DIRECT_ONLY = false>
+CF_DEV bool score_fast_plan(const DIndex &ix, const DParams &pr, const DBatch &b, uint32_t q, const FastPlan &fp, uint64_t base) {
+    const bool paired = qf_paired(fp.qf);
     uint64_t eTax[kFastEntries];
     uint32_t eRef[kFastEntries], eTidx[kFastEntries], eTs[kFastEntries], eSc[kFastEntries][4], eHl[kFastEntries][4];
 #pragma unroll
@@ -2430,17 +2444,9 @@
 #pragma unroll
         for (int c = 0; c < 4; c++) { eSc[z][c] = 0; eHl[z][c] = 0; }
     }
-    uint64_t pTop[kInlinePlan];
-    uint32_t pNelt[kInlinePlan], pMeta[kInlinePlan];
-#pragma unroll
-    for (uint32_t j = 0; j < kInlinePlan; j++) {
-        PlanHit ph{0, 0, 0};
-        if (j < nPlan) ph = b.qplan[(uint64_t)j * b.qplanStride + q];
-        pTop[j] = ph.top; pNelt[j] = ph.nelt; pMeta[j] = ph.meta;
-    }
     static_assert(kInlinePlan == 4, "three thresholds below");
-    const uint32_t c1 = pNelt[0], c2 = c1 + pNelt[1], c3 = c2 + pNelt[2];
-    uint32_t total = c3 + pNelt[3];
+    const uint32_t c1 = fp.pl0.nelt, c2 = c1 + fp.pl1.nelt, c3 = c2 + fp.pl2.nelt;
+    uint32_t total = c3 + fp.pl3.nelt;
     if (total > kScoreFastRows) total = kScoreFastRows;
     constexpr uint32_t kGather = 4;
     uint32_t nh = 0;
@@ -2451,14 +2457,14 @@
         for (uint32_t i = 0; i < kGather; i++) {
             const uint32_t s = s0 + i;
             const bool g1 = s >= c1, g2 = s >= c2, g3 = s >= c3;
-            rowv[i] = (g3 ? pTop[3] : g2 ? pTop[2] : g1 ? pTop[1] : pTop[0]) + (s - (g3 ? c3 : g2 ? c2 : g1 ? c1 : 0u));
-            rmeta[i] = g3 ? pMeta[3] : g2 ? pMeta[2] : g1 ? pMeta[1] : pMeta[0];
+            rowv[i] = (g3 ? fp.pl3.top : g2 ? fp.pl2.top : g1 ? fp.pl1.top : fp.pl0.top) + (s - (g3 ? c3 : g2 ? c2 : g1 ? c1 : 0u));
+            rmeta[i] = g3 ? fp.pl3.meta : g2 ? fp.pl2.meta : g1 ? fp.pl1.meta : fp.pl0.meta;
             ref[i] = 0xffffffffu;
         }
         bool act[kGather], isPos[kGather];
 #pragma unroll
         for (uint32_t i = 0; i < kGather; i++) { act[i] = s0 + i < total; isPos[i] = act[i] && (rowv[i] & kRowIsPos) != 0; }
-        if (b.directRefs) {
+        if (DIRECT_ONLY || b.directRefs) {
             uint32_t tref[kGather];
             if (ix.offw) {
 #pragma unroll
@@ -2505,7 +2511,7 @@
                     if (isPos[i] && !(pos >= span[i].x + ix.walkMax && pos + 12 <= span[i].y)) leave = true;
                     if (isPos[i]) tref[i] = sq[i];
                 }
-                if (leave) { if (EARLY) { b.nOut[q] = 0; b.score2[q] = 0; } return true; }
+                if (leave) return true;
             }
 #pragma unroll
             for (uint32_t i = 0; i < kGather; i++) if (act[i]) ref[i] = tref[i];
@@ -2535,7 +2541,7 @@
                 if (z < nh && at == kFastEntries && (pr.rankSlot == 0 ? eRef[z] == ref[i] : eTax[z] == tax)) at = z;
             bool add = true;
             if (at == kFastEntries) {
-                if (nh == kFastEntries) { if (EARLY) { b.nOut[q] = 0; b.score2[q] = 0; } return true; }
+                if (nh == kFastEntries) return true;
                 at = nh++;
 #pragma unroll
                 for (uint32_t z = 0; z < kFastEntries; z++) if (z == at) { eTax[z] = tax; eRef[z] = ref[i]; eTidx[z] = tidx; eTs[z] = ts; }
@@ -2552,8 +2558,7 @@
             }
         }
     }
-    if (nh > pr.k) { if (EARLY) { b.nOut[q] = 0; b.score2[q] = 0; } return true; }
-    const bool paired = qf_paired(qf);
+    if (nh > pr.k) return true;
     uint32_t score[kFastEntries], hitLen[kFastEntries];
 #pragma unroll
     for (uint32_t z = 0; z < kFastEntries; z++) {
@@ -2659,6 +2664,51 @@
     }
     b.nOut[q] = num; b.score2[q] = score2;
     return false;
+}
+
+CF_DEV bool fast_plan_load(const DBatch &b, uint32_t q, FastPlan &fp) {
+    const uint32_t qf = b.qflag[q], nPlan = qf_nplan(qf), nRows = b.qRows[q];
+    if (nPlan == kPlanNotInline || nRows > kScoreFastRows) return false;
+    fp = FastPlan{{0, 0, 0}, {0, 0, 0}, {0, 0, 0}, {0, 0, 0}, nPlan, nRows, qf};
+    static_assert(kInlinePlan == 4, "four plan slots");
+    if (nPlan > 0) fp.pl0 = b.qplan[q];
+    if (nPlan > 1) fp.pl1 = b.qplan[b.qplanStride + q];
+    if (nPlan > 2) fp.pl2 = b.qplan[2 * b.qplanStride + q];
+    if (nPlan > 3) fp.pl3 = b.qplan[3 * b.qplanStride + q];
+    return true;
+}
+template <bool EARLY = false>
+CF_DEV bool score_fast_body(const DIndex &ix, const DParams &pr, const DBatch &b, uint32_t q) {
+    if (EARLY) {
+        if (b.postDeferred[q] || (b.st->flags & kStHitsOverflow)) { b.nOut[q] = 0; b.score2[q] = 0; return !(b.st->flags & kStHitsOverflow); }
+    } else if (q < b.st->qLo || q >= b.st->qHi) {
+        if (b.st->qLo == 0) b.nOut[q] = 0;
+        return false;
+    }
+    FastPlan fp;
+    bool leave = !fast_plan_load(b, q, fp);
+    if (!leave) leave = score_fast_plan(ix, pr, b, q, fp, EARLY ? 0 : b.qBase[q] - b.st->rowLo);
+    if (leave && EARLY) { b.nOut[q] = 0; b.score2[q] = 0; }
+    return leave;
+}
+CF_DEV bool score_fast_listed_body(const DIndex &ix, const DParams &pr, const DBatch &b, uint32_t q) {
+    FastPlan fp;
+    if (!fast_plan_load(b, q, fp)) return true;
+    return score_fast_plan<true>(ix, pr, b, q, fp, 0);
+}
+
+constexpr uint32_t kLeftPost = 1u, kLeftScore = 2u;
+CF_DEV uint32_t post_score_fast_body(const DIndex &ix, const DParams &pr, const DBatch &b, uint32_t q) {
+    if (b.st->flags & kStHitsOverflow) { b.qRows[q] = 0; b.nOut[q] = 0; b.score2[q] = 0; return 0; }
+    FastPlan fp;
+    if (post_fast_plan(pr, b, q, fp)) { b.nOut[q] = 0; b.score2[q] = 0; return kLeftPost; }
+    b.qRows[q] = fp.rowsTotal;
+    bool leave = fp.rowsTotal > kScoreFastRows;
+    if (!leave) leave = score_fast_plan<true>(ix, pr, b, q, fp, 0);
+    if (!leave) return 0;
+    post_fast_store(b, q, fp);
+    b.nOut[q] = 0; b.score2[q] = 0;
+    return kLeftScore;
 }
 
 constexpr uint32_t score_scratch_bytes(uint32_t rows) { return rows * (uint32_t)(sizeof(HmEntry) + sizeof(TcEntry) + sizeof(uint32_t)); }
diff --git a/centrifuge_amd/csrc/cf_scan.hpp b/centrifuge_amd/csrc/cf_scan.hpp
--- a/centrifuge_amd/csrc/cf_scan.hpp
+++ b/centrifuge_amd/csrc/cf_scan.hpp
@@ -49,7 +49,7 @@
     if (threadIdx.x == 0) { tileA[blockIdx.x] = a; if (MODE == SCAN_HITS) tileC[blockIdx.x] = c; }
 }
 
-__global__ void __launch_bounds__(kScanBlock) k_scan_tiles(uint64_t *tileA, uint32_t *tileC, uint32_t nTiles, bool withC) {
+__device__ __forceinline__ uint64_t scan_tiles_body(uint64_t *tileA, uint32_t *tileC, uint32_t nTiles, bool withC) {
     __shared__ uint64_t sA[kScanBlock];
     __shared__ uint32_t sC[kScanBlock];
     uint64_t carryA = 0;
@@ -71,6 +71,10 @@
         carryA += sA[kScanBlock - 1]; carryC += sC[kScanBlock - 1];
         __syncthreads();
     }
+    return carryA;
+}
+__global__ void __launch_bounds__(kScanBlock) k_scan_tiles(uint64_t *tileA, uint32_t *tileC, uint32_t nTiles, bool withC) {
+    (void)scan_tiles_body(tileA, tileC, nTiles, withC);
 }
 
 template <int MODE>
@@ -111,9 +115,9 @@
 inline uint32_t scan_tiles_for(uint64_t n) { return (uint32_t)((n + 1 + kScanTile - 1) / kScanTile); }
 
 template <int MODE>
-inline void scan_enqueue(const uint32_t *in, uint64_t n, uint64_t *outA, uint32_t *outC, uint64_t *tileA, uint32_t *tileC, hipStream_t st) {
+inline void scan_enqueue(const uint32_t *in, uint64_t n, uint64_t *outA, uint32_t *outC, uint64_t *tileA, uint32_t *tileC, hipStream_t st, bool haveSums = false) {
     const uint32_t tiles = scan_tiles_for(n);
-    hipLaunchKernelGGL((k_scan_sums<MODE>), dim3(tiles), dim3(kScanBlock), 0, st, in, n, tileA, tileC);
+    if (!haveSums) hipLaunchKernelGGL((k_scan_sums<MODE>), dim3(tiles), dim3(kScanBlock), 0, st, in, n, tileA, tileC);
     hipLaunchKernelGGL(k_scan_tiles, dim3(1), dim3(kScanBlock), 0, st, tileA, tileC, tiles, MODE == SCAN_HITS);
     hipLaunchKernelGGL((k_scan_write<MODE>), dim3(tiles), dim3(kScanBlock), 0, st, in, n, (const uint64_t *)tileA, (const uint32_t *)tileC, outA, outC);
 }
```

After: 1.482 billion (median of 6 runs). 1.04x the previous value.
